# konrad-kaminski/ratelimit

Measured on AMD Instinct MI355X. Metric: rate-limit decisions/sec (whole node) at 10M/1B keys; p99 batch latency, higher is better.
Workload: dtype u32

## Files before the change

### ratelimit_amd/build.py

```python
import os
import subprocess
import sys

HERE = os.path.dirname(os.path.abspath(__file__))
ROOT = os.path.dirname(HERE)
CSRC = os.path.join(HERE, "csrc")
LIB = os.path.join(HERE, "libratelimit_hip.so")
TEAR_LIB = os.path.join(HERE, "libratelimit_hip_tear.so")
SOURCES = ["rl_kernels.hip", "rl_route.hip", "rl_match.hip", "rl_wire.hip", "rl_resp.hip", "rl_hot.hip", "rl_engine.hip", "rl_transport.hip",
           "rl_comm.hip",
           "rl_api.hip",
           "rl_pack.cpp"]
HEADERS = ["rl_device.h", "rl_kernels.h", "rl_slot_img.h", "rl_hot_select.h", "rl_match.h", "rl_wire_parse.h", "rl_resp_emit.h", "rl_engine.h",
           "rl_comm.h", "rl_transport.h",
           os.path.join("..", "..", "include", "ratelimit_hip.h")]
HIPCC = os.environ.get("HIPCC", "/opt/rocm/bin/hipcc")
ARCH = os.environ.get("RL_OFFLOAD_ARCH", "gfx950")
FLAGS = ["-O3", "-std=c++17", "-fPIC", "--offload-arch=" + ARCH, "-ffp-contract=off",
         "-Wall", "-Wno-unused-function", "-I" + os.path.join(ROOT, "include")]


def _stale():
    if not os.path.exists(LIB) or not os.path.exists(TEAR_LIB):
        return True
    t = min(os.path.getmtime(LIB), os.path.getmtime(TEAR_LIB))
    deps = [os.path.join(CSRC, s) for s in SOURCES + HEADERS] + [os.path.abspath(__file__)]
    return any(os.path.getmtime(d) > t for d in deps if os.path.exists(d))


def build(force=False, verbose=False, out=None, defines=()):
    lib = out or LIB
    if out is None and not force and not _stale():
        return LIB
    objs, procs = [], []
    tag = "" if out is None else "_%x" % (hash(lib) & 0xFFFFFF)

    def compile_(s, o, extra=()):
        cmd = [HIPCC] + FLAGS + ["-D" + d for d in tuple(defines) + tuple(extra)] + ["-c", os.path.join(CSRC, s),
                                                                                     "-o", o]
        if verbose:
            print(" ".join(cmd))
        procs.append((subprocess.Popen(cmd), cmd))

    for s in SOURCES:
        o = os.path.join(CSRC, os.path.splitext(s)[0] + tag + ".o")
        compile_(s, o)
        objs.append(o)
    tear_obj = None
    if out is None:
        tear_obj = os.path.join(CSRC, "rl_kernels_tear.o")
        compile_("rl_kernels.hip", tear_obj, ["RL_LOG_TEAR=1"])
    for p, cmd in procs:
        if p.wait() != 0:
            raise subprocess.CalledProcessError(p.returncode, cmd)

    def link(path, objects):
        cmd = [HIPCC, "-shared", "-fPIC", "--offload-arch=" + ARCH, "-o", path] + objects + ["-ldl"]
        if verbose:
            print(" ".join(cmd))
        subprocess.check_call(cmd)

    link(lib, objs)
    if tear_obj:
        link(TEAR_LIB, [tear_obj] + objs[1:])
        os.remove(tear_obj)
    for o in objs:
        os.remove(o)
    return lib


if __name__ == "__main__":
    print(build(force="--force" in sys.argv, verbose=True))
```

### ratelimit_amd/csrc/rl_engine.hip

```cpp
#include <hip/hip_runtime.h>
#include <hip/hip_ext.h>

#include <algorithm>
#include <chrono>
#include <cstdio>
#include <cstdlib>
#include <random>
#include <cstring>
#include <string>
#include <vector>

#include "../../include/ratelimit_hip.h"
#include "rl_device.h"
#include "rl_kernels.h"
#include "rl_match.h"
#include "rl_engine.h"

using namespace rl;



namespace {

thread_local std::string g_err;

int set_err(Engine* c, int code, const std::string& msg);

void prof_fold(Engine* c, uint32_t k) {
  if (!c->prof_pending[k]) return;
  c->prof_pending[k] = false;
  if (hipEventSynchronize(c->ev[k][RL_NUM_STAGES]) != hipSuccess) return;
  for (int i = 0; i < RL_NUM_STAGES; i++) {
    float ms = 0;
    if (hipEventElapsedTime(&ms, c->ev[k][i], c->ev[k][i + 1]) == hipSuccess) c->stage_ms[i] += ms;
  }
  c->prof_batches++;
}

void prof_fold_all(Engine* c) {
  for (uint32_t k = 0; k < PROF_RING; k++) prof_fold(c, (c->prof_next + k) % PROF_RING);
}

hipEvent_t* prof_events(Engine* c) {
  if (!c->prof) return nullptr;
  if (c->prof_skip) {
    c->prof_skip--;
    return nullptr;
  }
  c->prof_skip = c->prof_every - 1;
  const uint32_t k = c->prof_next;
  c->prof_next = (k + 1) % PROF_RING;
  prof_fold(c, k);
  c->prof_pending[k] = true;
  return c->ev[k];
}

int set_err(Engine* c, int code, const std::string& msg) {
  if (c) c->last_error = msg;
  else g_err = msg;
  return code;
}

#define HIPCHK(c, expr)                                                                        \
  do {                                                                                         \
    hipError_t _e = (expr);                                                                    \
    if (_e != hipSuccess)                                                                      \
      return set_err((c), RL_E_HIP, std::string("gpu: ") + #expr + ": " + hipGetErrorString(_e)); \
  } while (0)

#define RQ_SETTLE(c)                                               \
  do {                                                             \
    if ((c)->rq_n) {                                               \
      const int _rc = rl::eng_requests_advance((c), (c)->rq_n);    \
      if (_rc) return _rc;                                         \
    }                                                              \
  } while (0)

template <typename T>
hipError_t dalloc(T** p, size_t count) {
  return hipMalloc((void**)p, std::max<size_t>(count, 1) * sizeof(T));
}

inline double wall_s() {
  return std::chrono::duration<double>(std::chrono::steady_clock::now().time_since_epoch()).count();
}

int map_err(Engine* c, uint32_t e) {
  if (!e) return RL_OK;
  if (e & ERR_TIME) return set_err(c, RL_E_TIME, "gpu: now outside [0, 2^32-172800] or before the last sweep");
  if (e & ERR_HISTORY)
    return set_err(c, RL_E_TIME,
                   "gpu: a request's window is older than its key's history holds (more than 8 windows and "
                   "div + expiration_jitter_max_seconds behind the key's newest, or the history log overwrote it: "
                   "raise history_entries)");
  if (e & ERR_INVALID) return set_err(c, RL_E_INVALID, "gpu: malformed batch (unit, rule id, request index or stem offsets)");
  if (e & ERR_TABLE_FULL) return set_err(c, RL_E_TABLE_FULL, "gpu: counter table full (raise table_slots or sweep)");
  if (e & ERR_ARENA_FULL) return set_err(c, RL_E_ARENA_FULL, "gpu: long-stem arena full (raise arena_bytes)");
  return set_err(c, RL_E_INTERNAL, "gpu: unknown device error");
}

hipError_t after_batches(Engine* c, hipStream_t st) {
  for (uint32_t k = 0; k < NBUF; k++) {
    const hipError_t e = hipStreamWaitEvent(st, c->b_done[k], 0);
    if (e != hipSuccess) return e;
  }
  return hipSuccess;
}

int collect(Engine* c, hipStream_t st = nullptr) {
  if (!st) st = c->stream;
  HIPCHK(c, hipMemcpyAsync(c->h_err, c->errw, ERRW_WORDS * sizeof(uint32_t), hipMemcpyDeviceToHost, st));
  HIPCHK(c, hipStreamSynchronize(st));
  uint32_t e = c->h_err[NBUF + 2];
  for (uint32_t j = 0; j < NBUF; j++) e |= c->h_err[j];
  for (uint32_t j = 0; j < ERRB_RING; j++) e |= c->h_err[ERRW_B0 + j];
  if (e || c->h_err[NBUF + 1]) {
    HIPCHK(c, hipMemsetAsync(c->errw, 0, ERRW_WORDS * sizeof(uint32_t), st));
    HIPCHK(c, hipStreamSynchronize(st));
  }
  return map_err(c, e);
}

TableDev table_view(Engine* c);
Params params(Engine* c, int isolate = 0);

uint32_t enqueue(Engine* c, const BatchDev& b_in, const OutDev& o, int restore, hipStream_t st, bool pipelined) {
  const uint32_t k = c->next;
  const BatchDev& b = b_in;
  c->next = (k + 1) % NBUF;
  TableDev t = table_view(c);
  t.log_epoch = c->s[k].log_epoch;
  const int isolate = (!restore && o.status) ? 1 : 0;
  const Params P = params(c, isolate);
  const uint32_t* errb_prev = c->s[c->last].errb;
  c->s[k].errb = c->errw + ERRW_B0 + (c->errb_seq++ % ERRB_RING);
  const bool early = c->b_early;
  bool lng = c->long_mode == 2;
  if (c->long_mode == 1) {
    for (uint32_t j = 0; j < NBUF; j++)
      if (__atomic_load_n(&c->h_long[j], __ATOMIC_RELAXED)) {
        __atomic_store_n(&c->h_long[j], 0u, __ATOMIC_RELAXED);
        c->long_recent = 4 * NBUF;
      }
    lng = c->long_recent > 0;
    if (c->long_recent) c->long_recent--;
  }
  uint32_t* hint = c->long_mode ? c->h_long + k : nullptr;
  bool big_full = c->big_mode == 0;
  if (c->big_mode == 1) {
    for (uint32_t j = 0; j < NBUF; j++)
      if (__atomic_load_n(&c->h_big[j], __ATOMIC_RELAXED)) {
        __atomic_store_n(&c->h_big[j], 0u, __ATOMIC_RELAXED);
        c->big_recent = 4 * NBUF;
      }
    big_full = c->big_recent > 0;
    if (c->big_recent) c->big_recent--;
  }
  uint32_t* bhint = c->big_mode == 1 ? c->h_big + k : nullptr;
  bool late_full = c->late_mode == 0;
  if (c->late_mode == 1) {
    for (uint32_t j = 0; j < NBUF; j++)
      if (__atomic_load_n(&c->h_late[j], __ATOMIC_RELAXED)) {
        __atomic_store_n(&c->h_late[j], 0u, __ATOMIC_RELAXED);
        c->late_recent = 4 * NBUF;
      }
    late_full = c->late_recent > 0;
    if (c->late_recent) c->late_recent--;
  }
  uint32_t* lhint = c->late_mode == 1 ? c->h_late + k : nullptr;
  bool list_on = c->list_mode == 0;
  if (c->list_mode == 1) {
    for (uint32_t j = 0; j < NBUF; j++)
      if (__atomic_load_n(&c->h_list[j], __ATOMIC_RELAXED)) {
        __atomic_store_n(&c->h_list[j], 0u, __ATOMIC_RELAXED);
        c->list_recent = 4 * NBUF;
      }
    list_on = c->list_recent > 0;
    if (c->list_recent) c->list_recent--;
  }
  uint32_t* uhint = c->list_mode == 1 ? c->h_list + k : nullptr;
  if (pipelined) {
    hipStream_t a = c->pipe[k];
    hipEvent_t* ev = prof_events(c);
    (void)hipStreamWaitEvent(a, c->b_done[k], 0);
    (void)hipStreamWaitEvent(a, c->consumed[k], 0);
    launch_stage_a(b, c->s[k], isolate, P.per_second, a, ev, hint, lng, bhint, big_full, uhint, list_on);
    if (early) launch_b_begin_early(b, o, c->s[k], restore, a, c->log_ctr);
    (void)hipStreamWaitEvent(a, c->b_table[c->last], 0);
    launch_stage_b(b, o, t, P, c->s[k], restore, a, ev, errb_prev, c->b_table[k], ev ? c->d_kt_acc : nullptr,
                   early, lhint, late_full, list_on);
    (void)hipEventRecord(c->b_done[k], a);
  } else {
    if (!st) st = c->stream;
    (void)after_batches(c, st);
    hipEvent_t* ev = prof_events(c);
    launch_stage_a(b, c->s[k], isolate, P.per_second, st, ev, hint, lng, bhint, big_full, uhint, list_on);
    if (early) launch_b_begin_early(b, o, c->s[k], restore, st, c->log_ctr);
    launch_stage_b(b, o, t, P, c->s[k], restore, st, ev, errb_prev, c->b_table[k], ev ? c->d_kt_acc : nullptr,
                   early, lhint, late_full, list_on);
    (void)hipEventRecord(c->b_done[k], st);
  }
  c->last = k;
  return k;
}

hipError_t track(Engine* c, hipStream_t st) {
  if (c->seq_sub - c->seq_done >= PROGRESS_RING) {
    const hipError_t e = hipEventSynchronize(c->done_ring[c->seq_done % PROGRESS_RING]);
    if (e != hipSuccess) return e;
    c->seq_done++;
  }
  const hipError_t e = hipEventRecord(c->done_ring[c->seq_sub % PROGRESS_RING], st);
  c->seq_sub++;
  return e;
}

int check_sizes(Engine* c, const rl_batch* in, uint64_t stem_bytes) {
  if (!in) return set_err(c, RL_E_INVALID, "gpu: null batch");
  if (in->n > c->cfg.max_batch || in->n_requests > c->cfg.max_requests || in->n_rules > c->cfg.max_rules ||
      stem_bytes > c->cfg.max_stem_bytes)
    return set_err(c, RL_E_CAPACITY, "gpu: batch exceeds configured max_batch/max_requests/max_rules/max_stem_bytes");
  if (in->n && in->n_requests == 0) return set_err(c, RL_E_INVALID, "gpu: descriptors without requests");
  return RL_OK;
}

BatchDev dev_view(const Engine* c, const rl_batch* in, uint32_t stem_cap) {
  BatchDev b{};
  b.hk = c->hk;
  b.n = in->n;
  b.n_req = in->n_requests;
  b.n_rules = in->n_rules;
  b.stem_cap = stem_cap;
  b.stem_total = stem_cap;
  b.now_desc = 0;
  b.stem = in->stem_bytes;
  b.off = in->stem_off;
  b.now = in->now;
  b.req = in->req_idx;
  b.unit = in->unit;
  b.flags = in->flags;
  b.limit = in->limit;
  b.hits = in->hits;
  b.rule = in->rule_id;
  return b;
}

hipError_t log_ctr_get(Engine* c, std::vector<unsigned long long>& ctr, unsigned long long* lost,
                       unsigned long long* refused = nullptr) {
  std::vector<unsigned long long> h((size_t)(LOG_PARTS + 1) * LOG_CTR_STRIDE);
  hipError_t e = hipMemcpyAsync(h.data(), c->log_ctr, h.size() * 8, hipMemcpyDeviceToHost, c->stream);
  if (e == hipSuccess) e = hipStreamSynchronize(c->stream);
  if (e != hipSuccess) return e;
  ctr.resize(LOG_PARTS);
  for (uint32_t k = 0; k < LOG_PARTS; k++) ctr[k] = h[(size_t)k * LOG_CTR_STRIDE];
  if (lost) *lost = h[(size_t)LOG_PARTS * LOG_CTR_STRIDE];
  if (refused) *refused = h[(size_t)LOG_PARTS * LOG_CTR_STRIDE + 1];
  return hipSuccess;
}

TableDev table_view(Engine* c) {
  TableDev t;
  t.slots = c->slots;
  t.log = c->log;
  t.log_ctr = c->log_ctr;
  t.log_cap = c->log_cap;
  t.horizon = c->horizon;
  t.hist_lost = c->log_ctr + (size_t)LOG_PARTS * LOG_CTR_STRIDE;
  t.tear = c->tear;
  t.log_epoch = nullptr;
  t.mask = c->nslots - 1;
  t.arena = c->arena;
  t.arena_used16 = c->s[0].counters + 4;
  t.arena_cap16 = c->arena_cap16;
  t.max_probe = (uint32_t)std::min<uint64_t>(c->nslots, 1u << 16);
  t.shift = 64u - (uint32_t)__builtin_ctzll(c->nslots);
  return t;
}

Params params(Engine* c, int isolate) {
  Params P;
  P.ratio = c->cfg.near_limit_ratio;
  P.lc_en = c->cfg.local_cache_enabled != 0;
  P.per_second = c->cfg.per_second_split != 0;
  P.isolate = isolate;
  return P;
}

bool alloc_buffer(Scratch& s, uint32_t n) {
  const size_t items = (size_t)n / (64 * 4 * 8) + 1 + PART_DIGITS;
  bool ok = dalloc(&s.big_meta, PART_DIGITS) == hipSuccess && dalloc(&s.big_n, 1) == hipSuccess &&
            dalloc(&s.big_work, items) == hipSuccess && dalloc(&s.work_n, 1) == hipSuccess &&
            dalloc(&s.sorted_n, 1) == hipSuccess &&
            dalloc(&s.big_cnt, items * (1 + 2 * BIG_HEAVY)) == hipSuccess;
  ok = ok && dalloc(&s.rec, n) == hipSuccess && dalloc(&s.res, n) == hipSuccess;
  for (int i = 0; i < 2; i++) ok = ok && dalloc(&s.keys[i], n) == hipSuccess && dalloc(&s.vals[i], n) == hipSuccess;
  ok = ok && dalloc(&s.grp, n) == hipSuccess && dalloc(&s.lead, n) == hipSuccess && dalloc(&s.gmask, n) == hipSuccess &&
       dalloc(&s.defer, n) == hipSuccess &&
       dalloc(&s.defer_n, 1) == hipSuccess && dalloc(&s.defer2, n) == hipSuccess &&
       dalloc(&s.defer1, n) == hipSuccess && dalloc(&s.defer1_n, 1) == hipSuccess &&
       dalloc(&s.defer2_n, 1) == hipSuccess && dalloc(&s.fast_blk, (size_t)n / (256 * 32) + 1) == hipSuccess &&
       dalloc(&s.log_epoch, LOG_PARTS) == hipSuccess &&
       dalloc(&s.uniq, n) == hipSuccess && dalloc(&s.uniq_n, 1) == hipSuccess &&
       dalloc(&s.long_runs, (size_t)n / 1024 + 2) == hipSuccess &&
       dalloc(&s.kt_blk, 2 * ((size_t)n / 2 + BIG_HEAVY * PART_DIGITS + 2 * (size_t)n + 512) / 256) == hipSuccess;
  ok = ok && dalloc(&s.hits_s, n) == hipSuccess && dalloc(&s.segsum, n) == hipSuccess &&
       dalloc(&s.rid, n) == hipSuccess && dalloc(&s.run_start, (size_t)n + 1) == hipSuccess &&
       dalloc(&s.run_flags, n) == hipSuccess && dalloc(&s.run_state, n) == hipSuccess && dalloc(&s.run_alias, n) == hipSuccess &&
       dalloc(&s.run_f, n) == hipSuccess &&
       dalloc(&s.runs64, 1) == hipSuccess && dalloc(&s.split, 2) == hipSuccess && dalloc(&s.drun, (size_t)n / 2 + BIG_HEAVY * PART_DIGITS) == hipSuccess;
  ok = ok && dalloc(&s.hit_a, n) == hipSuccess && dalloc(&s.tile, n) == hipSuccess &&
       dalloc(&s.hit_t, n) == hipSuccess;
  ok = ok && dalloc(&s.run_end, n) == hipSuccess &&
       dalloc(&s.part_info, (size_t)PART_DIGITS * std::max((n + PART_TILE - 1) / PART_TILE, 1u)) == hipSuccess;
  ok = ok && dalloc(&s.r_base, RL_MAX_SHARDS) == hipSuccess && dalloc(&s.woff, (size_t)n + 1) == hipSuccess &&
       dalloc(&s.wtsum, WIRE_SCAN_WORDS(n)) == hipSuccess;
  return ok;
}

void free_buffer(Scratch& s) {
  void* bufs[] = {s.rec, s.res, s.big_meta, s.big_n, s.big_work, s.work_n, s.sorted_n, s.big_cnt, s.keys[0], s.keys[1],
                  s.vals[0], s.vals[1], s.grp, s.lead, s.gmask, s.defer, s.defer_n, s.defer2, s.defer2_n, s.defer1,
                  s.defer1_n, s.fast_blk, s.hits_s, s.segsum, s.rid, s.run_start, s.run_flags, s.run_state, s.run_alias,
                  s.run_f, s.runs64, s.split, s.drun, s.run_end, s.part_info, s.hit_a, s.tile, s.hit_t, s.r_base,
                  s.uniq, s.uniq_n, s.long_runs, s.kt_blk, s.log_epoch, s.woff, s.wtsum};
  for (void* p : bufs)
    if (p) (void)hipFree(p);
}

int stage(Engine* c, const rl_batch* in, BatchDev* out) {
  const uint32_t n = in->n, nq = in->n_requests;
  const uint64_t nb = n ? in->stem_off[n] : 0;
  int rc = check_sizes(c, in, nb);
  if (rc) return rc;
  hipStream_t st = c->stream;
  HIPCHK(c, after_batches(c, st));
  if (nb) HIPCHK(c, hipMemcpyAsync(c->d_stem, in->stem_bytes, nb, hipMemcpyHostToDevice, st));
  HIPCHK(c, hipMemcpyAsync(c->d_off, in->stem_off, (n + 1) * sizeof(uint32_t), hipMemcpyHostToDevice, st));
  if (nq) HIPCHK(c, hipMemcpyAsync(c->d_now, in->now, nq * sizeof(int64_t), hipMemcpyHostToDevice, st));
  if (n) {
    HIPCHK(c, hipMemcpyAsync(c->d_req, in->req_idx, n * 4, hipMemcpyHostToDevice, st));
    HIPCHK(c, hipMemcpyAsync(c->d_unit, in->unit, n, hipMemcpyHostToDevice, st));
    HIPCHK(c, hipMemcpyAsync(c->d_flags, in->flags, n, hipMemcpyHostToDevice, st));
    HIPCHK(c, hipMemcpyAsync(c->d_limit, in->limit, n * 4, hipMemcpyHostToDevice, st));
    HIPCHK(c, hipMemcpyAsync(c->d_hits, in->hits, n * 4, hipMemcpyHostToDevice, st));
    HIPCHK(c, hipMemcpyAsync(c->d_rule, in->rule_id, n * 4, hipMemcpyHostToDevice, st));
  }
  rl_batch d = *in;
  d.stem_bytes = c->d_stem;
  d.stem_off = c->d_off;
  d.now = c->d_now;
  d.req_idx = c->d_req;
  d.unit = c->d_unit;
  d.flags = c->d_flags;
  d.limit = c->d_limit;
  d.hits = c->d_hits;
  d.rule_id = c->d_rule;
  *out = dev_view(c, &d, c->cfg.max_stem_bytes);
  return RL_OK;
}

}

namespace rl {

const char* eng_last_error(const Engine* c) { return c ? c->last_error.c_str() : g_err.c_str(); }

hipError_t rl_stream_create(hipStream_t* st, uint32_t role) {
  static const uint32_t dedicated =
      getenv("RL_DEDICATED_QUEUES") ? (uint32_t)strtoul(getenv("RL_DEDICATED_QUEUES"), nullptr, 0) : 0u;
  if (!(dedicated & role)) return hipStreamCreateWithFlags(st, hipStreamNonBlocking);
  int dev = 0, cus = 0;
  hipError_t e = hipGetDevice(&dev);
  if (e == hipSuccess) e = hipDeviceGetAttribute(&cus, hipDeviceAttributeMultiprocessorCount, dev);
  if (e != hipSuccess) return e;
  std::vector<uint32_t> mask(((uint32_t)cus + 31) / 32, 0xFFFFFFFFu);
  return hipExtStreamCreateWithCUMask(st, (uint32_t)mask.size(), mask.data());
}

Engine* eng_create(const rl_config* cfg_in, char* err, size_t errlen) {
  auto fail = [&](const std::string& m, Engine* c) -> Engine* {
    if (err && errlen) snprintf(err, errlen, "%s", m.c_str());
    g_err = m;
    if (c) eng_destroy(c);
    return nullptr;
  };
  if (!cfg_in) return fail("gpu: null config", nullptr);
  rl_config cfg = *cfg_in;
  if (!cfg.table_slots) cfg.table_slots = 1ull << 24;
  if (cfg.table_slots & (cfg.table_slots - 1)) return fail("gpu: table_slots must be a power of two", nullptr);
  if (!cfg.arena_bytes) cfg.arena_bytes = 64ull << 20;
  if (!cfg.history_entries) cfg.history_entries = cfg.table_slots;
  if (cfg.history_entries > (uint64_t)LOG_PARTS * LOG_PART_MAX)
    return fail("gpu: history_entries must be at most 2^31", nullptr);
  if (cfg.expiration_jitter_max_seconds < 0) return fail("gpu: expiration_jitter_max_seconds must be >= 0", nullptr);
  if (!cfg.max_batch) cfg.max_batch = 1u << 20;
  if (cfg.max_batch > MAX_PART_TILES * PART_TILE)
    return fail("gpu: max_batch must be at most 8388608 descriptors", nullptr);
  if (!cfg.max_requests) cfg.max_requests = cfg.max_batch;
  if (!cfg.max_rules) cfg.max_rules = 65536;
  if (!cfg.max_stem_bytes) cfg.max_stem_bytes = 128u * cfg.max_batch;
  if (hipSetDevice(cfg.device) != hipSuccess) return fail("gpu: hipSetDevice failed", nullptr);

  Engine* c = new Engine();
  c->cfg = cfg;
  c->hash_seed = cfg.hash_seed;
  while (!c->hash_seed) {
    std::random_device rd;
    c->hash_seed = ((uint64_t)rd() << 32) ^ rd();
  }
  c->cfg.hash_seed = c->hash_seed;
  c->hk = hash_key_of(c->hash_seed, cfg.debug_hash_bits);
  c->nslots = cfg.table_slots;
  {
    const uint64_t want = std::max<uint64_t>(cfg.history_entries / LOG_PARTS, std::max<uint64_t>(cfg.max_batch / 16, 1024));
    uint64_t cap = 1;
    while (cap * 2 <= want && cap * 2 <= LOG_PART_MAX) cap *= 2;
    if (cap < want && cap < LOG_PART_MAX) cap *= 2;
    c->log_cap = (uint32_t)cap;
    c->cfg.history_entries = (uint64_t)LOG_PARTS * cap;
    c->horizon = (uint32_t)std::min<int64_t>(cfg.expiration_jitter_max_seconds, 1ll << 30);
  }
  c->arena_cap16 = cfg.arena_bytes / 16;
  const uint32_t n = cfg.max_batch;
  bool ok = true;
  for (uint32_t k = 0; k < NBUF; k++) ok = ok && rl_stream_create(&c->pipe[k], SR_PIPE) == hipSuccess;
  if (const char* be = getenv("RL_B_BEGIN_EARLY")) c->b_early = atoi(be) != 0;
  c->stream = c->pipe[0];
  for (uint32_t k = 0; k < NBUF; k++)
    ok = ok && hipEventCreateWithFlags(&c->b_done[k], hipEventDisableTiming) == hipSuccess &&
         hipEventCreateWithFlags(&c->b_table[k], hipEventDisableTiming) == hipSuccess;
  for (uint32_t k = 0; k < PROGRESS_RING; k++)
    ok = ok && hipEventCreateWithFlags(&c->done_ring[k], hipEventDisableTiming) == hipSuccess;
  ok = ok && dalloc(&c->slots, c->nslots) == hipSuccess &&
       dalloc(&c->log, (size_t)LOG_PARTS * c->log_cap) == hipSuccess &&
       dalloc(&c->log_ctr, (size_t)(LOG_PARTS + 1) * LOG_CTR_STRIDE) == hipSuccess;
  ok = ok && dalloc(&c->arena, cfg.arena_bytes) == hipSuccess && dalloc(&c->arena2, cfg.arena_bytes) == hipSuccess;
  for (uint32_t k = 0; k < NBUF; k++) ok = ok && alloc_buffer(c->s[k], n);
  Scratch& s0 = c->s[0];
  ok = ok && dalloc(&c->errw, ERRW_WORDS) == hipSuccess;
  for (uint32_t k = 0; k < NBUF; k++)
    ok = ok && hipEventCreateWithFlags(&c->consumed[k], hipEventDisableTiming) == hipSuccess;
  ok = ok && hipEventCreateWithFlags(&c->route_ready, hipEventDisableTiming) == hipSuccess &&
       hipEventCreateWithFlags(&c->caller_ready, hipEventDisableTiming) == hipSuccess;
  c->serial_debug = getenv("RL_DEBUG_SERIAL") != nullptr;
  c->copy_time = getenv("RL_DEBUG_COPYTIME") != nullptr;
  c->host_time = getenv("RL_DEBUG_HOSTTIME") != nullptr;
  for (uint32_t k = 0; c->copy_time && k < 64; k++)
    ok = ok && hipEventCreate(&c->ct_ev[0][k]) == hipSuccess && hipEventCreate(&c->ct_ev[1][k]) == hipSuccess &&
         hipEventCreate(&c->ct_ev[2][k]) == hipSuccess;
  ok = ok && hipHostMalloc((void**)&c->h_base, (size_t)NBUF * RL_MAX_SHARDS * 8) == hipSuccess;
  for (uint32_t k = 0; k < NBUF; k++)
    ok = ok && dalloc(&c->s[k].stripes, (size_t)STAT_STRIPES * STAT_LDS_RULES * RL_NUM_STATS) == hipSuccess;
  ok = ok && dalloc(&s0.time_floor, 1) == hipSuccess;
  ok = ok && dalloc(&s0.counters, 8) == hipSuccess;
  for (uint32_t k = 0; k < NBUF; k++) {
    Scratch& sk = c->s[k];
    sk.err = c->errw ? c->errw + k : nullptr;
    sk.errb = c->errw ? c->errw + ERRW_B0 + k : nullptr;
    sk.errs = c->errw ? c->errw + NBUF + 1 : nullptr;
    sk.time_floor = s0.time_floor;
    sk.counters = s0.counters;
  }
  ok = ok && dalloc(&c->d_stem, (size_t)cfg.max_stem_bytes + 64) == hipSuccess;
  ok = ok && dalloc(&c->d_off, (size_t)n + 1) == hipSuccess;
  ok = ok && dalloc(&c->d_now, cfg.max_requests) == hipSuccess;
  ok = ok && dalloc(&c->d_req, n) == hipSuccess && dalloc(&c->d_unit, n) == hipSuccess &&
       dalloc(&c->d_flags, n) == hipSuccess && dalloc(&c->d_limit, n) == hipSuccess &&
       dalloc(&c->d_hits, n) == hipSuccess && dalloc(&c->d_rule, n) == hipSuccess;
  ok = ok && dalloc(&c->d_code, n) == hipSuccess && dalloc(&c->d_status, n) == hipSuccess &&
       dalloc(&c->d_rem, n) == hipSuccess &&
       dalloc(&c->d_reset, n) == hipSuccess;
  ok = ok && dalloc(&c->d_stats, (size_t)cfg.max_rules * RL_NUM_STATS) == hipSuccess;
  ok = ok && hipHostMalloc((void**)&c->h_err, ERRW_WORDS * sizeof(uint32_t)) == hipSuccess;
  ok = ok && hipHostMalloc((void**)&c->h_counters, 8 * sizeof(unsigned long long)) == hipSuccess;
  ok = ok && hipHostMalloc((void**)&c->h_long, NBUF * sizeof(uint32_t)) == hipSuccess;
  if (ok) memset(c->h_long, 0, NBUF * sizeof(uint32_t));
  if (const char* sl = getenv("RL_SPLIT_LONG")) c->long_mode = atoi(sl);
  ok = ok && hipHostMalloc((void**)&c->h_big, NBUF * sizeof(uint32_t)) == hipSuccess;
  if (ok) memset(c->h_big, 0, NBUF * sizeof(uint32_t));
  if (const char* bc = getenv("RL_BIG_CUE")) c->big_mode = atoi(bc);
  ok = ok && hipHostMalloc((void**)&c->h_late, NBUF * sizeof(uint32_t)) == hipSuccess;
  if (ok) memset(c->h_late, 0, NBUF * sizeof(uint32_t));
  if (const char* lc = getenv("RL_LATE_CUE")) c->late_mode = atoi(lc);
  ok = ok && hipHostMalloc((void**)&c->h_list, NBUF * sizeof(uint32_t)) == hipSuccess;
  if (ok) memset(c->h_list, 0, NBUF * sizeof(uint32_t));
  if (const char* uc = getenv("RL_LIST_CUE")) c->list_mode = atoi(uc);
  if (const char* hr = getenv("RL_HOT_RANGE"))
    c->hot_range = std::min<uint64_t>(std::max<uint64_t>(strtoull(hr, nullptr, 0), 64), 1ull << 22);
  if (!ok) return fail("gpu: device allocation failed (table_slots/arena/max_batch too large?)", c);
  ok = hipMemsetAsync(c->slots, 0, c->nslots * sizeof(Slot), c->stream) == hipSuccess &&
       hipMemsetAsync(c->log_ctr, 0, (size_t)(LOG_PARTS + 1) * LOG_CTR_STRIDE * 8, c->stream) == hipSuccess &&
       hipMemsetAsync(c->errw, 0, ERRW_WORDS * 4, c->stream) == hipSuccess &&
       hipMemsetAsync(s0.time_floor, 0, 8, c->stream) == hipSuccess &&
       hipMemsetAsync(s0.counters, 0, 64, c->stream) == hipSuccess &&
       hipMemsetAsync(c->s[0].stripes, 0, (size_t)STAT_STRIPES * STAT_LDS_RULES * RL_NUM_STATS * 8, c->stream) ==
           hipSuccess &&
       hipMemsetAsync(c->d_stem, 0, (size_t)cfg.max_stem_bytes + 64, c->stream) == hipSuccess &&
       hipStreamSynchronize(c->stream) == hipSuccess;
  for (uint32_t k = 0; k < NBUF; k++)
    ok = ok && hipEventRecord(c->b_done[k], c->stream) == hipSuccess &&
         hipEventRecord(c->b_table[k], c->stream) == hipSuccess &&
         (k == 0 || hipMemsetAsync(c->s[k].stripes, 0, (size_t)STAT_STRIPES * STAT_LDS_RULES * RL_NUM_STATS * 8,
                                   c->stream) == hipSuccess) &&
         hipEventRecord(c->consumed[k], c->stream) == hipSuccess;
  if (!ok) return fail("gpu: device initialisation failed", c);
  return c;
}

void free_host_slots(Engine* c) {
  for (HostSlot& h : c->hs) {
    void* bufs[] = {h.stem, h.off, h.req, h.limit, h.hits, h.rule, h.now, h.unit, h.flags, h.code, h.status, h.rem,
                    h.reset, h.stats, h.cbuf};
    for (void* p : bufs)
      if (p) (void)hipFree(p);
    if (h.in_done) (void)hipEventDestroy(h.in_done);
    if (h.out_done) (void)hipEventDestroy(h.out_done);
    h = HostSlot{};
  }
  for (hipStream_t st : {c->h2d, c->d2h})
    if (st) (void)hipStreamDestroy(st);
  c->h2d = c->d2h = nullptr;
  c->hs_ready = false;
}

void copy_time_fold(Engine* c, bool all);
namespace {
void free_request_slots(Engine* c);
}

void eng_destroy(Engine* c) {
  if (!c) return;
  (void)hipSetDevice(c->cfg.device);
  if (c->host_time && c->ht_n)
    fprintf(stderr, "RL_DEBUG_HOSTTIME: %llu batches, ms each: check %.4f copy %.4f unpack %.4f enqueue %.4f to_host %.4f "
            "track %.4f\n", (unsigned long long)c->ht_n, c->ht[0] / c->ht_n * 1e3, c->ht[1] / c->ht_n * 1e3,
            c->ht[2] / c->ht_n * 1e3, c->ht[3] / c->ht_n * 1e3, c->ht[4] / c->ht_n * 1e3, c->ht[5] / c->ht_n * 1e3);
  if (c->copy_time) {
    (void)hipDeviceSynchronize();
    copy_time_fold(c, true);
    if (c->ct_count)
      fprintf(stderr, "RL_DEBUG_COPYTIME: %llu input copies, %.4f ms each, slot wait %.4f ms, gap after the previous "
              "copy %.4f ms\n", (unsigned long long)c->ct_count, c->ct_ms / c->ct_count, c->ct_wait_ms / c->ct_count,
              c->ct_gap_ms / c->ct_count);
    for (uint32_t k = 0; k < 64; k++)
      for (int j = 0; j < 3; j++)
        if (c->ct_ev[j][k]) (void)hipEventDestroy(c->ct_ev[j][k]);
  }
  if (c->hs_ready) {
    (void)hipDeviceSynchronize();
    free_host_slots(c);
  }
  if (c->rq) {
    (void)hipDeviceSynchronize();
    free_request_slots(c);
  }
  for (uint32_t k = 0; k < NBUF; k++)
    if (c->pipe[k]) (void)hipStreamSynchronize(c->pipe[k]);
  for (uint32_t k = 0; k < PROF_RING; k++)
    for (int i = 0; i <= RL_NUM_STAGES; i++)
      if (c->ev[k][i]) (void)hipEventDestroy(c->ev[k][i]);
  if (c->d_kt_acc) (void)hipFree(c->d_kt_acc);
  for (uint32_t k = 0; k < NBUF; k++) {
    free_buffer(c->s[k]);
    if (c->b_done[k]) (void)hipEventDestroy(c->b_done[k]);
    if (c->b_table[k]) (void)hipEventDestroy(c->b_table[k]);
    if (c->consumed[k]) (void)hipEventDestroy(c->consumed[k]);
  }
  for (uint32_t k = 0; k < PROGRESS_RING; k++)
    if (c->done_ring[k]) (void)hipEventDestroy(c->done_ring[k]);
  if (c->rs_ready) {
    c->rs.err = nullptr;
    scratch_free(c->rs);
  }
  if (c->route_ready) (void)hipEventDestroy(c->route_ready);
  if (c->caller_ready) (void)hipEventDestroy(c->caller_ready);
  if (c->ov_order) (void)hipEventDestroy(c->ov_order);
  for (void* p : {(void*)c->ov.slots, (void*)c->ov.koff, (void*)c->ov.klen, (void*)c->ov.arena, (void*)c->ov.ctr})
    if (p) (void)hipFree(p);
  if (c->h_base) (void)hipHostFree(c->h_base);
  const Scratch& s0 = c->s[0];
  void* bufs[] = {c->slots, c->log, c->log_ctr, c->tear, c->arena, c->arena2, c->errw, s0.stripes, s0.time_floor, s0.counters, c->d_stem, c->d_off,
                  c->d_now, c->d_req, c->d_unit, c->d_flags, c->d_limit, c->d_hits, c->d_rule, c->d_code, c->d_status,
                  c->d_rem,
                  c->d_reset, c->d_stats};
  for (void* p : bufs)
    if (p) (void)hipFree(p);
  for (uint32_t k = 1; k < NBUF; k++)
    if (c->s[k].stripes) (void)hipFree(c->s[k].stripes);
  if (c->h_err) (void)hipHostFree(c->h_err);
  if (c->h_counters) (void)hipHostFree(c->h_counters);
  if (c->h_long) (void)hipHostFree(c->h_long);
// ... 2525 lines not shown
```

### ratelimit_amd/csrc/rl_kernels.h

```cpp
#pragma once

#include <hip/hip_runtime.h>
#include <stdint.h>

#include "rl_device.h"
#include "rl_hot_select.h"

namespace rl {

#ifndef RL_PART_ITEMS
#define RL_PART_ITEMS 16
#endif
constexpr uint32_t PART_ITEMS = RL_PART_ITEMS, PART_TILE = 256 * PART_ITEMS;
constexpr uint32_t PART_BITS = 10, PART_DIGITS = 1u << PART_BITS;
#ifndef RL_BIG_BLOCKS
#define RL_BIG_BLOCKS 64
#endif
constexpr uint32_t BIG_BLOCKS = RL_BIG_BLOCKS;
constexpr uint32_t BIG_ITEM_BLOCKS = 256;
constexpr uint32_t BIG_HEAVY = 4;

struct BigMeta {
  uint32_t d, S, base, nchunks, item0, r, rb_heavy, db_heavy;
  uint32_t heavy[BIG_HEAVY];
};
constexpr uint32_t MAX_PART_TILES = 2048 * 16 / PART_ITEMS;
constexpr uint32_t LONG_RUN = 32;
constexpr uint32_t RUN_SLOW = 1, RUN_FAST = 2, RUN_MULTI = 4;
constexpr uint32_t RUN_NOWVAR = 8;
constexpr uint32_t RUN_ALIAS = 16;
constexpr uint32_t RUN_AHEAD = 32;
constexpr uint32_t RUN_MERGE = 64;
constexpr uint32_t RUN_G_SHIFT = 8, RUN_UMASK_SHIFT = 16;
constexpr uint32_t RUN_UNITS = 128, RUN_STEMS = 1u << 24;
#ifndef RL_KEY_HEAD
#define RL_KEY_HEAD 64
#endif
constexpr uint32_t KEY_HEAD = RL_KEY_HEAD;
constexpr uint32_t KEY_HV = KEY_HEAD / 16;
static_assert(KEY_HEAD % 16 == 0 && KEY_HEAD >= 48 && KEY_HEAD <= 64, "key head: 48 or 64 bytes (>= KEY_IN)");
constexpr uint32_t STAT_STRIPES = 64;
constexpr uint32_t STAT_LDS_RULES = 512;
constexpr uint32_t RUNS_GENERAL_LATE_BLOCKS = 8;

struct Wire;
struct OwnChunk {
  uint32_t lo, n, rank, stem_total;
  uint32_t src_n;
  uint32_t n_rules;
  const uint32_t* idx;
  const unsigned long long* hash;
  const uint8_t* stem;
  const uint32_t* off;
  const int64_t* now;
  const uint32_t* req;
  const uint8_t* unit;
  const uint8_t* flags;
  const uint32_t* limit;
  const uint32_t* hits;
  const uint32_t* rule;
  uint8_t* code;
  uint32_t* rem;
  uint32_t* reset;
  uint8_t* status;
  uint32_t* src_err;
};
struct BatchDev {
  uint32_t n, n_req, n_rules, stem_cap;
  uint32_t stem_total;
  uint32_t now_desc;
  HashKey hk;
  const uint8_t* stem;
  const uint32_t* off;
  const int64_t* now;
  const uint32_t* req;
  const uint8_t* unit;
  const uint8_t* flags;
  const uint32_t* limit;
  const uint32_t* hits;
  const uint32_t* rule;
  const Wire* wire;
  const uint32_t* woff;
  const unsigned long long* wbad;
  const unsigned long long* wbase;
  uint32_t n_src, rule_stride;
  OwnChunk own;
};

struct __attribute__((aligned(16))) Rec {
  uint32_t hlo;
  uint32_t off;
  uint32_t lu;
  uint32_t rule;
  uint32_t req;
  uint32_t now;
  uint32_t hits;
  uint32_t limit;
};
static_assert(sizeof(Rec) == 32, "Rec is two dwordx4");

struct SRec {
  const Rec* rec;
  const uint32_t* sv;
  __device__ inline Rec operator[](uint32_t q) const { return rec[sv[q]]; }
};

__host__ __device__ inline uint32_t rec_len(const Rec& r) { return r.lu & 0xFFFFu; }
__host__ __device__ inline uint32_t rec_unit(const Rec& r) { return (r.lu >> 16) & 0xFFu; }
__host__ __device__ inline uint32_t rec_flags(const Rec& r) { return r.lu >> 24; }

constexpr uint32_t ROUTE_REQ_BITS = 24;
constexpr uint32_t ROUTE_MAX_REQ = 1u << ROUTE_REQ_BITS;
constexpr uint32_t ROUTE_TILE = 512;
struct __attribute__((aligned(8))) Wire {
  uint32_t label;
  uint32_t lu;
  uint32_t limit;
  uint32_t hits;
  uint32_t rule;
  uint32_t now;
  unsigned long long hash;
};
constexpr uint32_t WIRE_NOW_BAD = 0xFFFFFFFFu;
static_assert(sizeof(Wire) == RL_WIRE_BYTES, "wire record size is part of the ABI");

struct OutDev {
  uint8_t* code;
  uint32_t* rem;
  uint32_t* reset;
  unsigned long long* stats;
  uint8_t* status;
};

struct TableDev {
  Slot* slots;
  LogEnt* log;
  unsigned long long* log_ctr;
  uint32_t log_cap;
  uint32_t horizon;
  unsigned long long* hist_lost;
  const unsigned long long* log_epoch;
  uint32_t* tear;
  uint64_t mask;
  uint8_t* arena;
  unsigned long long* arena_used16;
  uint64_t arena_cap16;
  uint32_t max_probe;
  uint32_t shift;
};

struct Params {
  float ratio;
  int lc_en;
  int per_second;
  int isolate;
};

struct Scratch {
  Rec* rec;
  unsigned long long* res;
  uint32_t* keys[2];
  uint32_t* vals[2];
  BigMeta* big_meta;
  uint32_t* big_n;
  uint32_t* big_work;
  uint32_t* work_n;
  uint32_t* sorted_n;
  uint32_t* big_cnt;
  uint32_t* grp;
  uint32_t* lead;
  uint8_t* gmask;
  uint32_t* defer;
  uint32_t* defer_n;
  uint32_t* defer2;
  uint32_t* defer2_n;
  uint32_t* defer1;
  uint32_t* defer1_n;
  uint32_t* fast_blk;
  unsigned long long* log_epoch;
  uint2* uniq;
  uint32_t* uniq_n;
  uint32_t* long_runs;
  unsigned long long* kt_blk;
  unsigned long long* stripes;
  uint32_t* hits_s;
  uint32_t* hit_a;
  uint4* tile;
  uint32_t* hit_t;
  uint32_t* segsum;
  uint32_t* rid;
  uint32_t* run_start;
  uint32_t* run_end;
  uint32_t* part_info;
  uint32_t* run_flags;
  uint4* run_state;
  uint4* run_alias;
  uint32_t* run_f;
  unsigned long long* runs64;
  unsigned long long* split;
  uint32_t* drun;
  uint32_t* err;
  uint32_t* errb;
  uint32_t* errs;
  int64_t* time_floor;
  unsigned long long* counters;
  uint32_t* route_start;
  uint8_t* route_dest;
  unsigned long long* route_hash;
  uint32_t* route_hist;
  unsigned long long* r_base;
  uint32_t* woff;
  unsigned long long* wtsum;
};

void launch_stage_a(const BatchDev& b, const Scratch& s, int isolate, int per_second, hipStream_t st,
                    hipEvent_t* ev = nullptr, uint32_t* long_hint = nullptr, bool long_kernel = false,
                    uint32_t* big_hint = nullptr, bool big_full = true, uint32_t* list_hint = nullptr,
                    bool list_on = true);
void launch_stage_b(const BatchDev& b, const OutDev& o, const TableDev& t, const Params& P, const Scratch& s,
                    int restore, hipStream_t st, hipEvent_t* ev, const uint32_t* errb_prev, hipEvent_t table_done,
                    unsigned long long* kt_acc = nullptr, bool early = false, uint32_t* late_hint = nullptr,
                    bool late_full = true, bool list_on = true);
void launch_b_begin_early(const BatchDev& b, const OutDev& o, const Scratch& s, int restore, hipStream_t st,
                          const unsigned long long* log_ctr);
void launch_unpack(const rl_batch_compact& cb, const uint8_t* buf, uint32_t* req, uint8_t* unit, uint8_t* flags,
                   uint32_t* limit, uint32_t* hits, uint32_t* rule, int64_t* now, uint32_t* err, hipStream_t st);
void launch_unpack_range(const rl_batch_compact& cb, const uint8_t* buf, uint32_t d0, uint32_t d1, uint32_t q0,
                         uint32_t q1, uint32_t* req, uint8_t* unit, uint8_t* flags, uint32_t* limit, uint32_t* hits,
                         uint32_t* rule, int64_t* now, uint32_t* err, hipStream_t st);
constexpr uint32_t TO_HOST_MAX = 6;
struct ToHost {
  const uint8_t* src[TO_HOST_MAX];
  uint8_t* dst[TO_HOST_MAX];
  uint64_t bytes[TO_HOST_MAX];
  uint32_t n;
};
void launch_to_host(const ToHost& c, hipStream_t st);
hipError_t copy_to_host(ToHost c, hipStream_t st);

void launch_unpack_prefixed(const rl_batch_prefixed& pb, const uint8_t* buf, uint32_t t0, uint32_t t1, uint8_t* stem,
                            uint32_t* off, uint32_t* req, uint8_t* unit, uint8_t* flags, uint32_t* limit,
                            uint32_t* hits, uint32_t* rule, int64_t* now, uint32_t* err, hipStream_t st);
constexpr uint32_t ROUTE_OWN_NONE = 0xFFFFFFFFu;
constexpr uint32_t WIRE_SCAN_TILE = 2048;
inline uint32_t WIRE_SCAN_TILES(uint64_t n) { return (uint32_t)((n + WIRE_SCAN_TILE) / WIRE_SCAN_TILE); }
inline uint32_t WIRE_SCAN_WORDS(uint64_t n) { return WIRE_SCAN_TILES(n) + 1; }
void launch_wire_offsets(const Wire* w, uint32_t n, uint32_t olo, uint32_t ohi, const unsigned long long* wbase,
                         uint32_t n_src, unsigned long long stem_total, uint32_t* woff, unsigned long long* tsum,
                         hipStream_t st);
void launch_route_pack(const BatchDev& b, uint32_t n_shards, uint32_t src_rank, Wire* out, uint8_t* out_stem,
                       uint32_t* perm, unsigned long long* counts, const Scratch& s, hipStream_t st,
                       uint32_t cstride = 2, unsigned long long meta0 = 0, unsigned long long meta1 = 0,
                       uint32_t own_rank = ROUTE_OWN_NONE, unsigned long long* hash_out = nullptr,
                       unsigned long long* counts_host = nullptr);
void launch_cnt_fill(unsigned long long* cnt, uint32_t n_peers, uint32_t cstride, unsigned long long meta0,
                     unsigned long long meta1, hipStream_t st, unsigned long long* cnt_host = nullptr);
void launch_route_fail(unsigned long long* ret, uint32_t n, uint32_t status, hipStream_t st);
void launch_route_scatter(const uint32_t* perm, const unsigned long long* ret, uint32_t n, const OutDev& o,
                          hipStream_t st, uint32_t* src_err = nullptr, const uint32_t* errb = nullptr,
                          uint32_t own_lo = 0, uint32_t own_hi = 0);
void launch_route_ret(const unsigned long long* res, uint32_t n, const uint32_t* errb, unsigned long long* ret,
                      hipStream_t st);
void launch_stats_sum(const unsigned long long* stage, uint32_t n_blocks, uint32_t m, unsigned long long* out,
                      hipStream_t st, uint32_t stride = 0);
void launch_sweep(const TableDev& t, uint64_t nslots, uint32_t now, unsigned long long* evicted, hipStream_t st);
void launch_arena_compact(Slot* slots, uint64_t nslots, const uint8_t* from, uint8_t* to, unsigned long long* used16,
                          hipStream_t st);
void launch_reclaim(const TableDev& t, const HashKey& hk, uint64_t nslots, uint32_t* need, unsigned long long* ctr,
                    hipStream_t st);
void launch_lc_count(const TableDev& t, uint64_t nslots, uint32_t now, unsigned long long* out, hipStream_t st);
void launch_table_info(const Slot* slots, uint64_t nslots, unsigned long long* out, hipStream_t st);
constexpr uint32_t RESIZE_CTR_WORDS = 6;
void launch_resize_place(const TableDev& t, const HashKey& hk, uint64_t nslots, Slot* to, uint64_t to_nslots,
                         uint32_t* map, unsigned long long* ctr, hipStream_t st);
void launch_resize_relink(const TableDev& t, uint64_t nslots, const uint32_t* map, unsigned long long* ctr,
                          hipStream_t st);
struct ExportDev {
  uint8_t* stem;
  uint32_t* off;
  uint8_t* unit;
  uint8_t* flags;
  uint32_t *ws, *count, *expire, *lc;
};
void launch_export_count(const TableDev& t, uint64_t s0, uint64_t s1, uint32_t* cnt, unsigned long long* tot,
                         hipStream_t st);
void launch_export_write(const TableDev& t, uint64_t s0, uint64_t s1, const uint32_t* cnt, unsigned long long* cursor,
                         const ExportDev& o, hipStream_t st);
struct __attribute__((aligned(16))) ImportRec {
  uint32_t off;
  uint32_t lu;
  uint32_t ws, count, expire, lc;
  uint32_t pad[2];
};
static_assert(sizeof(ImportRec) == 32, "ImportRec is two dwordx4");
void launch_import(const TableDev& t, const HashKey& hk, const uint8_t* stem, uint32_t stem_total, const ImportRec* rec,
                   const uint32_t* gstart, const unsigned long long* ghash, uint32_t ng, unsigned long long* epoch,
                   uint32_t* err, hipStream_t st);
constexpr uint32_t LOOKUP_NOW_BAD = 0xFFFFFFFFu;
struct LookupDev {
  uint32_t n;
  const uint32_t* off;
  const uint8_t* unit;
  const uint32_t* now;
  uint8_t *status, *found;
  uint32_t *count, *expire, *lc;
};
void launch_lookup(const TableDev& t, const HashKey& hk, const Params& P, const int64_t* time_floor,
                   const uint8_t* stem, uint32_t stem_total, const LookupDev& q, hipStream_t st);
struct HotState {
  unsigned long long matched, hits;
  unsigned long long stem_bytes;
  unsigned long long cursor;
  uint32_t pool_n;
  uint32_t thr, full;
  uint32_t err;
};
struct HotOutDev {
  uint8_t* stem;
  uint64_t stem_cap;
  uint32_t *off, *len;
  uint8_t* unit;
  uint32_t *ws, *count, *expire, *lc;
};
void launch_hot_scan(const TableDev& t, uint64_t s0, uint64_t s1, const rlhot::Query& q, uint32_t k, HotState* st,
                     unsigned long long* pool, uint32_t pool_cap, hipStream_t stream);
void launch_hot_select(HotState* st, unsigned long long* pool, uint32_t pool_cap, uint32_t k, uint32_t limit,
                       hipStream_t stream);
void launch_hot_size(const TableDev& t, HotState* st, const unsigned long long* pool, uint32_t pool_cap, uint32_t k,
                     hipStream_t stream);
void launch_hot_gather(const TableDev& t, HotState* st, const unsigned long long* pool, uint32_t n, const HotOutDev& o,
                       hipStream_t stream);
bool log_tear_hook();
void launch_debug_keys(const BatchDev& b, uint8_t* out, uint32_t* klen, hipStream_t st);
void launch_debug_decide(uint32_t n, const uint32_t* before, const uint32_t* after, const uint8_t* lc_hit,
                         const uint32_t* hits, const uint32_t* limit, const uint8_t* unit, const uint8_t* flags,
                         const int64_t* now, float ratio, int lc_en, uint8_t* code, uint32_t* rem, uint32_t* reset,
                         unsigned long long* deltas, uint8_t* lc_set, hipStream_t st);

}
```

### ratelimit_amd/csrc/rl_kernels.hip

```cpp
#include <hip/hip_runtime.h>
#include <stdint.h>
#include <cstdlib>

#include "rl_device.h"
#include "rl_kernels.h"
#include "rl_slot_img.h"

#ifndef RL_ABL
#define RL_ABL 0
#endif

namespace rl {

constexpr uint32_t HASH_LDS_BYTES = 16384;

__global__ __launch_bounds__(256) void k_prepare(BatchDev b, Rec* __restrict__ rec, uint32_t* __restrict__ keys,
                                                 uint32_t* err, uint32_t* errs, int isolate,
                                                 const int64_t* time_floor, uint32_t* defer_n,
                                                 uint32_t* big_n, uint32_t* work_n, uint32_t* __restrict__ run_flags,
                                                 unsigned long long* num_runs, uint32_t* __restrict__ hit_a,
                                                 unsigned long long* __restrict__ res, uint32_t* sorted_n,
                                                 uint32_t* uniq_n) {
  __shared__ uint32_t lds[HASH_LDS_BYTES / 4 + 4];
  const uint32_t tid = threadIdx.x;
// ... 982 lines not shown
  uint32_t pend_w, pend_e;
  __device__ inline void apply_pending() {
    if (pend) {
      if (cur.ws == pend_w) {
        cur.lc = pend_e;
        cur_dirty = true;
      } else if (old.ws == pend_w) {
        old.lc = pend_e;
        old_dirty = true;
      }
      pend = false;
    }
  }
};

__device__ __attribute__((always_inline)) inline void simple_put(const TableDev& t, SimpleState& S) {
  S.chain = log_append(t, S.si, S.tag, S.chain, S.cur.ws, S.old);
  S.chain_dirty = true;
  S.old_dirty = false;
}

__device__ __attribute__((always_inline)) inline int simple_pick(const TableDev& t, SimpleState& S, uint32_t w, uint32_t d,
                                                                 uint32_t now) {
  if (S.cur.ws == w) return 0;
  if (S.cur.ws == WS_INVALID || w > S.cur.ws) {
    if (S.cur.ws != WS_INVALID) {
      if (S.old_dirty) simple_put(t, S);
      if (hist_keep(t, S.cur, w, d)) {
        S.old = S.cur;
        S.old_dirty = true;
      }
    }
    S.cur = Win{w, 0, 0, 0};
    return 0;
  }
  if (S.old.ws != w) {
    if (S.old_dirty) simple_put(t, S);
    Win r;
    const int f = S.chain == LOG_NONE ? 0 : log_find(t, S.chain, S.si, S.tag, S.cur.ws, w, &r);
    if (f < 0 ? !hist_dead(now, w, d) : (f == 0 && !hist_absent_ok(t, now, w, S.cur.ws, d))) return -1;
    S.old = f > 0 ? r : Win{w, 0, 0, 0};
    S.old_dirty = false;
  }
  return 1;
}

__device__ __attribute__((always_inline)) inline void simple_step(const TableDev& t, const Params& P, unsigned long long* res,
                                                                  LaneStats& L, StatAcc& acc, SimpleState& S,
                                                                  const Elem& x, bool restore, uint32_t* err) {
  if (x.req != S.cur_req) {
    S.apply_pending();
    S.cur_req = x.req;
  }
  const int which = simple_pick(t, S, x.w, x.d, x.now);
  if (which < 0) {
    if (P.isolate) res[x.e] = pack_fail(RL_E_TIME);
    if (!(RL_ABL & 1)) atomicOr(err, ERR_HISTORY);
    return;
  }
  Win R = which ? S.old : S.cur;
  uint32_t after = 0;
  bool lc_hit = false;
  if (restore) {
    R.count = x.h;
    R.expire = x.now + x.d;
    if (x.flags) R.lc = x.now + x.d;
  } else {
    lc_hit = P.lc_en && x.now < R.lc;
    if (!lc_hit) {
      const uint32_t v = x.now <= R.expire ? R.count : 0u;
      R.count = v + x.h;
      R.expire = x.now + x.d;
      after = R.count;
    }
  }
  if (which) {
    S.old = R;
    S.old_dirty = true;
  } else {
    S.cur = R;
    S.cur_dirty = true;
  }
  if (restore) return;
  const Decision r = decide(after - x.h, after, lc_hit && !x.shadow, x.h, x.thr, P.ratio, x.shadow, P.lc_en);
  if (r.set_lc) {
    S.pend = true;
    S.pend_w = x.w;
    S.pend_e = x.now + x.d;
  }
  emit(res, L, acc, x, r, lc_hit);
}

struct GeneralState {
  int64_t sidx[4];
  Win cur[4];
  Win old[4];
  Win vic[4];
  uint32_t tag[4];
  uint32_t chain[4];
  uint32_t odirty;
  uint32_t vdirty;
  uint32_t cdirty;
  uint32_t present;
  uint32_t cur_req;
  uint32_t npend;
  uint32_t pend_w[4], pend_e[4];
};

__device__ inline bool ps_class(const Params& P, uint32_t k) { return P.per_second && k == 0; }

__device__ inline void gen_put(const TableDev& t, GeneralState& G, uint32_t k, bool vic = false) {
  G.chain[k] = log_append(t, (uint32_t)G.sidx[k], G.tag[k], G.chain[k], G.cur[k].ws, vic ? G.vic[k] : G.old[k]);
  G.cdirty |= 1u << k;
  if (vic) G.vdirty &= ~(1u << k);
  else G.odirty &= ~(1u << k);
}

__device__ inline void gen_set_old(const TableDev& t, GeneralState& G, uint32_t k, const Win& r, bool dirty) {
  if ((G.vdirty >> k) & 1) gen_put(t, G, k, true);
  G.vic[k] = G.old[k];
  G.vdirty = (G.vdirty & ~(1u << k)) | (G.odirty & (1u << k));
  G.old[k] = r;
  G.odirty = (G.odirty & ~(1u << k)) | (dirty ? 1u << k : 0u);
}

__device__ inline Win* gen_rec(const TableDev& t, GeneralState& G, uint32_t k, uint32_t w, uint32_t now, bool* lost) {
  const uint32_t d = div_of(k + 1);
  Win& c = G.cur[k];
  if (c.ws == w) return &c;
  if (c.ws == WS_INVALID || w > c.ws || w % d) return nullptr;
  if (G.old[k].ws == w) return &G.old[k];
  if (G.vic[k].ws == w) {
    const Win v = G.vic[k];
    G.vic[k] = G.old[k];
    G.old[k] = v;
    const uint32_t b = 1u << k, od = G.odirty & b;
    G.odirty = (G.odirty & ~b) | (G.vdirty & b);
    G.vdirty = (G.vdirty & ~b) | od;
    return &G.old[k];
  }
  Win r;
  const int f = G.chain[k] == LOG_NONE ? 0 : log_find(t, G.chain[k], (uint32_t)G.sidx[k], G.tag[k], c.ws, w, &r);
  if (f > 0) {
    gen_set_old(t, G, k, r, false);
    return &G.old[k];
  }
  if (lost && (f < 0 ? !hist_dead(now, w, d) : !hist_absent_ok(t, now, w, c.ws, d))) *lost = true;
  return nullptr;
}

__device__ inline void gen_touch(GeneralState& G, uint32_t k, const Win* R) {
  if (R == &G.old[k]) G.odirty |= 1u << k;
}

__device__ inline void general_apply_pending(const TableDev& t, GeneralState& G) {
  for (uint32_t j = 0; j < G.npend; j++) {
    for (uint32_t k = 0; k < 4; k++) {
      if (!(G.present >> k & 1)) continue;
      Win* R = gen_rec(t, G, k, G.pend_w[j], 0u, nullptr);
      if (R) {
        R->lc = G.pend_e[j];
        gen_touch(G, k, R);
      }
    }
  }
  G.npend = 0;
}

__device__ inline void general_step(const TableDev& t, const Params& P, unsigned long long* res, LaneStats& L,
                                    StatAcc& acc, GeneralState& G, const Elem& x, bool restore, uint32_t* err) {
  if (x.req != G.cur_req) {
    general_apply_pending(t, G);
    G.cur_req = x.req;
  }
  const uint32_t ui = x.unit - 1;
  const bool ps_e = ps_class(P, ui);
  bool lc_hit = false, lost = false;
  uint32_t v = 0, lcw = 0;
  bool vfound = false;
  for (uint32_t k = 0; k < 4; k++) {
    if (!(G.present >> k & 1)) continue;
    const Win* R = gen_rec(t, G, k, x.w, x.now, &lost);
    if (!R) continue;
    if (x.now < R->lc) lc_hit = true;
    lcw = R->lc > lcw ? R->lc : lcw;
    if (ps_class(P, k) == ps_e && !vfound && x.now <= R->expire) {
      v = R->count;
      vfound = true;
    }
  }
  if (lost) {
    if (P.isolate) res[x.e] = pack_fail(RL_E_TIME);
    atomicOr(err, ERR_HISTORY);
    return;
  }
  lc_hit = lc_hit && P.lc_en && !restore;
  uint32_t after = 0;
  if (!lc_hit) {
    const uint32_t nv = restore ? x.h : v + x.h;
    const uint32_t ex = x.now + x.d;
    Win& c = G.cur[ui];
    if (c.ws != x.w) {
      if (c.ws == WS_INVALID || x.w > c.ws) {
        if (c.ws != WS_INVALID && hist_keep(t, c, x.w, x.d)) gen_set_old(t, G, ui, c, true);
        c = Win{x.w, 0, 0, lcw};
      } else if (G.old[ui].ws != x.w) {
        gen_set_old(t, G, ui, Win{x.w, 0, 0, lcw}, true);
      }
    }
    for (uint32_t k = 0; k < 4; k++) {
      if (!(G.present >> k & 1) || ps_class(P, k) != ps_e) continue;
      Win* R = gen_rec(t, G, k, x.w, x.now, nullptr);
      if (R) {
        R->count = nv;
        R->expire = ex;
        gen_touch(G, k, R);
      }
    }
    after = nv;
  }
  if (restore) {
    if (x.flags) {
      for (uint32_t k = 0; k < 4; k++) {
        if (!(G.present >> k & 1)) continue;
        Win* R = gen_rec(t, G, k, x.w, x.now, nullptr);
        if (R) {
          R->lc = x.now + x.d;
          gen_touch(G, k, R);
        }
      }
    }
    return;
  }
  const Decision r = decide(after - x.h, after, lc_hit && !x.shadow, x.h, x.thr, P.ratio, x.shadow, P.lc_en);
  if (r.set_lc) {
    uint32_t j = 0;
    while (j < G.npend && G.pend_w[j] != x.w) j++;
    if (j == G.npend) G.npend++;
    G.pend_w[j] = x.w;
    G.pend_e[j] = x.now + x.d;
  }
  emit(res, L, acc, x, r, lc_hit);
}

__device__ __attribute__((always_inline)) inline void replay_simple(SRec rec_s, const uint32_t* svals,
                                                                    unsigned long long* res, const TableDev& t,
                                                                    const Params& P, const uint32_t* grp,
                                                                    uint32_t p, uint32_t end, uint32_t k, int64_t s0,
                                                                    Win cur0, uint32_t ring0, uint32_t tag0,
                                                                    const Rec& x0, uint32_t e0, LaneStats& L,
                                                                    StatAcc& acc, uint32_t* err, bool restore) {
  Slot* s = &t.slots[s0];
  SimpleState S;
  S.cur = cur0;
  S.old = Win{WS_INVALID, 0, 0, 0};
  S.si = (uint32_t)s0;
  S.tag = tag0;
  S.chain = ring0;
  S.cur_dirty = S.old_dirty = S.chain_dirty = false;
  S.cur_req = 0xFFFFFFFFu;
  S.pend = false;
  simple_step(t, P, res, L, acc, S, load_elem(x0, e0, restore), restore, err);
  for (uint32_t q = p + 1; q < end; q++) {
    if (grp && grp[q] != k) continue;
    simple_step(t, P, res, L, acc, S, load_elem(rec_s[q], svals[q], restore), restore, err);
  }
  S.apply_pending();
  if (S.old_dirty) simple_put(t, S);
  if (S.cur_dirty) s->cur = S.cur;
  if (S.chain_dirty) s->ring = S.chain;
}

__device__ __attribute__((always_inline)) inline uint32_t wave_incl_add(uint32_t x);
struct SegPair {
  uint32_t f, s;
};
__device__ inline SegPair seg_op(SegPair a, SegPair b) { return SegPair{a.f | b.f, b.f ? b.s : a.s + b.s}; }

struct SegChunk {
  uint64_t heads;
  uint32_t h;
};

__device__ inline SegPair seg_chunk_scan(const SegChunk& c, uint32_t lane) {
  const uint32_t P = wave_incl_add(c.h);
  const uint64_t le = c.heads & (lane == 63 ? ~0ull : ((2ull << lane) - 1));
  const uint32_t lh = le ? 63u - (uint32_t)__clzll((long long)le) : 0u;
  const uint32_t Plh = __shfl(P, lh, 64), hlh = __shfl(c.h, lh, 64);
  return le ? SegPair{1u, P - (Plh - hlh)} : SegPair{0u, P};
}

constexpr uint32_t BK_HEAVY = BIG_HEAVY;
constexpr uint32_t BK_HEAVY_MIN = 3;

template <uint32_t W, uint32_t IT>
struct BkShape {
  static constexpr uint32_t WAVES = W, ITEMS = IT, THREADS = 64 * W, CAP = 64 * W * IT, STRIP = 64 * IT;
};
using BkSmall = BkShape<4, 8>;
using BkBig = BkShape<8, 8>;

#ifdef RL_BK_PROF
__device__ unsigned long long g_bk_prof[PART_DIGITS * 16];
__device__ uint32_t g_bk_peel[PART_DIGITS * 16];
#define BK_STAMP(d, k) \
  if (threadIdx.x == 0) g_bk_prof[(d) * 16 + (k)] = wall_clock64()
#else
#define BK_STAMP(d, k)
#endif

template <uint32_t IT, uint32_t BITS>
__device__ inline void wave_multisplit(const uint32_t (&kk)[IT], uint32_t nvalid_base, uint32_t limit, uint32_t shift,
                                       uint32_t* row, uint32_t (&pos)[IT]) {
  const uint32_t lane = threadIdx.x & 63;
  const uint64_t lt_mask = (1ull << lane) - 1;
  uint32_t leader[IT];
#pragma unroll
  for (uint32_t i = 0; i < IT; i++) {
    leader[i] = lane;
    pos[i] = 0;
    if (nvalid_base + i * 64 >= limit) continue;
    const bool valid = nvalid_base + i * 64 + lane < limit;
    const uint32_t d = (kk[i] >> shift) & ((1u << BITS) - 1u);
    uint64_t peers = __ballot(valid);
#pragma unroll
    for (uint32_t bit = 0; bit < BITS; bit++) {
      const bool sb = (d >> bit) & 1u;
      const uint64_t bal = __ballot(sb);
      peers &= sb ? bal : ~bal;
    }
    const uint32_t rank = __popcll(peers & lt_mask);
    leader[i] = valid ? (uint32_t)(__ffsll((unsigned long long)peers) - 1) : lane;
    pos[i] = (valid && rank == 0) ? atomicAdd(&row[d], (uint32_t)__popcll(peers)) : 0u;
    pos[i] |= rank << 16;
  }
#pragma unroll
  for (uint32_t i = 0; i < IT; i++) pos[i] = __shfl(pos[i] & 0xFFFFu, leader[i]) + (pos[i] >> 16);
}

__device__ inline uint32_t scan256(uint32_t v, uint32_t* wsum4, uint32_t* total) {
  const uint32_t lane = threadIdx.x & 63, wave = threadIdx.x >> 6;
  uint32_t inc = v;
#pragma unroll
  for (uint32_t off = 1; off < 64; off <<= 1) {
    const uint32_t y = __shfl_up(inc, off, 64);
    if (lane >= off) inc += y;
  }
  if (wave < 4 && lane == 63) wsum4[wave] = inc;
  __syncthreads();
  uint32_t pre = 0;
#pragma unroll
  for (uint32_t w = 0; w < 4; w++) pre += w < wave ? wsum4[w] : 0u;
  if (total) *total = wsum4[0] + wsum4[1] + wsum4[2] + wsum4[3];
  __syncthreads();
  return pre + inc - v;
}

__global__ __launch_bounds__(256) void k_part(const uint32_t* __restrict__ kin, const uint32_t* __restrict__ hin,
                                              uint4* __restrict__ out, uint32_t n, uint32_t ntiles,
                                              uint32_t* __restrict__ info, const uint32_t* err) {
  constexpr uint32_t DPT = PART_DIGITS / 256;
  __shared__ uint32_t wcnt[4][PART_DIGITS];
  __shared__ uint32_t wsum[4];
  __shared__ uint32_t sk[PART_TILE], sv[PART_TILE], sh[PART_TILE];
  if (*err) return;
  const uint32_t tid = threadIdx.x, lane = tid & 63, wave = tid >> 6, tile = blockIdx.x;
  for (uint32_t j = tid; j < 4 * PART_DIGITS; j += 256) (&wcnt[0][0])[j] = 0;
  __syncthreads();
  const uint32_t wbase = tile * PART_TILE + wave * 64 * PART_ITEMS;
  uint32_t kk[PART_ITEMS], vv[PART_ITEMS], hh[PART_ITEMS], pos[PART_ITEMS];
#pragma unroll
  for (uint32_t i = 0; i < PART_ITEMS; i++) {
    const uint32_t j = min(wbase + i * 64 + lane, n - 1);
    kk[i] = kin[j];
    vv[i] = j;
    hh[i] = hin[j];
  }
  wave_multisplit<PART_ITEMS, PART_BITS>(kk, wbase, n, 32 - PART_BITS, wcnt[wave], pos);
  __syncthreads();
  uint32_t c[DPT], tsum = 0;
#pragma unroll
  for (uint32_t j = 0; j < DPT; j++) {
    const uint32_t d = tid * DPT + j;
    uint32_t acc = 0;
#pragma unroll
    for (uint32_t w = 0; w < 4; w++) {
      const uint32_t t = wcnt[w][d];
      wcnt[w][d] = acc;
      acc += t;
    }
    c[j] = acc;
    tsum += acc;
  }
  uint32_t excl = scan256(tsum, wsum, nullptr);
#pragma unroll
  for (uint32_t j = 0; j < DPT; j++) {
    const uint32_t d = tid * DPT + j;
    info[(size_t)d * ntiles + tile] = (excl << 16) | c[j];
#pragma unroll
    for (uint32_t w = 0; w < 4; w++) wcnt[w][d] += excl;
    excl += c[j];
  }
  __syncthreads();
#pragma unroll
  for (uint32_t i = 0; i < PART_ITEMS; i++) {
    if (wbase + i * 64 + lane < n) {
      const uint32_t d = kk[i] >> (32 - PART_BITS);
      const uint32_t q = wcnt[wave][d] + pos[i];
      sk[q] = kk[i];
      sv[q] = vv[i];
      sh[q] = hh[i];
    }
  }
  __syncthreads();
  const uint32_t cnt = min(PART_TILE, n - tile * PART_TILE);
  uint4* o = out + (size_t)tile * PART_TILE;
#pragma unroll
  for (uint32_t i = 0; i < PART_ITEMS; i++) {
    const uint32_t q = i * 256 + tid;
    if (q < cnt) o[q] = make_uint4(sk[q], sv[q], sh[q], 0u);
  }
}

template <typename B>
struct BucketLds {
  uint32_t k[B::CAP], v[B::CAP], h[B::CAP];
  uint32_t wcnt[B::WAVES][256];
  uint32_t gsum[B::WAVES / 4][256];
  uint32_t base[256];
  uint32_t roff[3][256];
  uint32_t dtot[256];
  uint32_t wsum[B::WAVES];
  SegPair sp[B::WAVES];
  uint32_t sh[B::WAVES];
  SegPair carry;
  uint32_t hcarry, rb, nruns, S, base_pos, db, dcnt;
  uint32_t heavy[BK_HEAVY];
  uint32_t hcnt[BK_HEAVY];
  uint32_t hstart[BK_HEAVY];
  uint32_t hrun[BK_HEAVY];
  uint32_t hw[B::WAVES][BK_HEAVY];
  uint32_t hsw[B::WAVES][BK_HEAVY];
  uint32_t acc[1 + 2 * BK_HEAVY];
  uint32_t lw[B::WAVES];
  uint32_t nheavy, nlight;
  uint32_t ub;
};

extern __shared__ uint32_t bk_seg[];

template <uint32_t IT>
__device__ inline void bucket_src(uint32_t ntiles, const uint32_t (&p)[IT], uint32_t (&j)[IT]) {
  const uint32_t* seg = bk_seg;
  const uint32_t* src = bk_seg + ntiles + 1;
  uint32_t lo[IT];
#pragma unroll
  for (uint32_t i = 0; i < IT; i++) lo[i] = 0;
#pragma unroll
  for (uint32_t step = MAX_PART_TILES / 2; step; step >>= 1) {
    if (step >= ntiles) continue;
#pragma unroll
    for (uint32_t i = 0; i < IT; i++) {
      const uint32_t m = lo[i] + step;
      if (m < ntiles && seg[m] <= p[i]) lo[i] = m;
    }
  }
#pragma unroll
  for (uint32_t i = 0; i < IT; i++) j[i] = src[lo[i]] + p[i];
}

template <typename B>
__device__ inline uint32_t block_sum(BucketLds<B>& L, uint32_t v) {
  const uint32_t lane = threadIdx.x & 63, wave = threadIdx.x >> 6;
#pragma unroll
  for (uint32_t off = 32; off; off >>= 1) v += __shfl_xor(v, off, 64);
  if (lane == 0) L.wsum[wave] = v;
  __syncthreads();
  uint32_t s = 0;
#pragma unroll
  for (uint32_t w = 0; w < B::WAVES; w++) s += L.wsum[w];
  __syncthreads();
  return s;
}

template <typename B>
__device__ inline void bucket_setup(BucketLds<B>& L, const uint32_t* __restrict__ info, uint32_t ntiles, uint32_t d) {
  const uint32_t tid = threadIdx.x, lane = tid & 63, wave = tid >> 6;
  uint32_t* seg = bk_seg;
  uint32_t* src = bk_seg + ntiles + 1;
  uint32_t carry = 0, offs = 0;
  for (uint32_t t0 = 0; t0 < ntiles; t0 += B::THREADS) {
    const uint32_t t = t0 + tid;
    const uint32_t e = t < ntiles ? info[(size_t)d * ntiles + t] : 0u;
    const uint32_t cnt = e & 0xFFFFu;
    offs += e >> 16;
    uint32_t inc = cnt;
#pragma unroll
    for (uint32_t off = 1; off < 64; off <<= 1) {
      const uint32_t y = __shfl_up(inc, off, 64);
      if (lane >= off) inc += y;
    }
    if (lane == 63) L.wsum[wave] = inc;
    __syncthreads();
    uint32_t pre = carry, all = carry;
    for (uint32_t w = 0; w < B::WAVES; w++) {
      pre += w < wave ? L.wsum[w] : 0u;
      all += L.wsum[w];
    }
    if (t < ntiles) {
      const uint32_t st = pre + inc - cnt;
      seg[t] = st;
      src[t] = t * PART_TILE + (e >> 16) - st;
    }
    carry = all;
    __syncthreads();
  }
  const uint32_t bp = block_sum(L, offs);
  if (tid == 0) {
    seg[ntiles] = carry;
    L.S = carry;
    L.base_pos = bp;
  }
  __syncthreads();
}

template <typename B, uint32_t BITS>
__device__ inline void bucket_rank(BucketLds<B>& L, const uint32_t (&kk)[B::ITEMS], uint32_t strip0, uint32_t limit,
                                   uint32_t shift, bool chunk_scan, uint32_t (&pos)[B::ITEMS]) {
  const uint32_t tid = threadIdx.x, wave = tid >> 6;
  for (uint32_t j = tid; j < B::WAVES * 256; j += B::THREADS) (&L.wcnt[0][0])[j] = 0;
  __syncthreads();
  uint32_t local[B::ITEMS];
  wave_multisplit<B::ITEMS, BITS>(kk, strip0, limit, shift, L.wcnt[wave], local);
  __syncthreads();
  constexpr uint32_t NG = B::WAVES / 4;
  const uint32_t dg = tid & 255u, g = tid >> 8;
  uint32_t r[4], c = 0;
#pragma unroll
  for (uint32_t w = 0; w < 4; w++) r[w] = L.wcnt[g * 4 + w][dg];
#pragma unroll
  for (uint32_t w = 0; w < 4; w++) {
    const uint32_t t = r[w];
    r[w] = c;
    c += t;
  }
  L.gsum[g][dg] = c;
  __syncthreads();
  uint32_t pre = 0, all = 0;
#pragma unroll
  for (uint32_t q = 0; q < NG; q++) {
    const uint32_t t = L.gsum[q][dg];
    pre += q < g ? t : 0u;
    all += t;
  }
#pragma unroll
  for (uint32_t w = 0; w < 4; w++) L.wcnt[g * 4 + w][dg] = r[w] + pre;
  if (tid < 256) L.dtot[tid] = all;
  const uint32_t excl = scan256(tid < 256 ? all : 0u, L.wsum, nullptr);
  if (chunk_scan && tid < 256) L.base[tid] = excl;
  __syncthreads();
#pragma unroll
  for (uint32_t i = 0; i < B::ITEMS; i++) {
    const uint32_t d = (kk[i] >> shift) & ((1u << BITS) - 1u);
    pos[i] = L.base[d] + L.wcnt[wave][d] + local[i];
  }
  __syncthreads();
}

template <typename B>
__device__ inline void lds_sort3(BucketLds<B>& L, uint32_t (&kk)[B::ITEMS], uint32_t (&vv)[B::ITEMS],
                                 uint32_t (&hh)[B::ITEMS], uint32_t n) {
  static_assert(32 - PART_BITS == 22, "passes of 8 + 8 + 6 bits");
  const uint32_t lane = threadIdx.x & 63, strip0 = (threadIdx.x >> 6) * B::STRIP;
  uint32_t pos[B::ITEMS];
#pragma unroll 1
  for (uint32_t pass = 0; pass < 3; pass++) {
    if (pass < 2) bucket_rank<B, 8>(L, kk, strip0, n, 8 * pass, true, pos);
    else bucket_rank<B, 6>(L, kk, strip0, n, 16, true, pos);
#pragma unroll
    for (uint32_t i = 0; i < B::ITEMS; i++) {
      if (strip0 + i * 64 + lane < n) {
        L.k[pos[i]] = kk[i];
        L.v[pos[i]] = vv[i];
        L.h[pos[i]] = hh[i];
      }
    }
    __syncthreads();
#pragma unroll
    for (uint32_t i = 0; i < B::ITEMS; i++) {
      const uint32_t p = strip0 + i * 64 + lane;
      if (p < n) {
        kk[i] = L.k[p];
        vv[i] = L.v[p];
        hh[i] = L.h[p];
      }
    }
  }
}

template <typename B, bool FROM_LDS, bool PRE = false>
__device__ inline void bucket_segment(BucketLds<B>& L, uint32_t d, uint32_t S, uint32_t base,
                                      const uint32_t* __restrict__ sk, const uint32_t* __restrict__ sh,
                                      uint32_t* __restrict__ segsum, uint32_t* __restrict__ rid,
                                      uint32_t* __restrict__ run_start, uint32_t* __restrict__ run_end,
                                      unsigned long long* num_runs, uint32_t* __restrict__ drun) {
  constexpr uint32_t IT = B::ITEMS;
  const uint32_t tid = threadIdx.x, lane = tid & 63, wave = tid >> 6;
  auto key = [&](uint32_t p) -> uint32_t { return FROM_LDS ? L.k[p] : sk[base + p]; };
  auto hit = [&](uint32_t p) -> uint32_t { return FROM_LDS ? L.h[p] : sh[base + p]; };
  uint32_t nh = 0, nd = 0;
  for (uint32_t c0 = 0; !PRE && c0 < S; c0 += B::CAP) {
    uint32_t a[IT], b[IT], c[IT];
#pragma unroll
    for (uint32_t i = 0; i < IT; i++) {
      const uint32_t p = min(c0 + i * B::THREADS + tid, S - 1);
      a[i] = key(p ? p - 1 : 0);
      b[i] = key(p);
      c[i] = key(p > 1 ? p - 2 : 0);
    }
#pragma unroll
    for (uint32_t i = 0; i < IT; i++) {
      const uint32_t p = c0 + i * B::THREADS + tid;
      nh += (p < S && (p == 0 || a[i] != b[i])) ? 1u : 0u;
      nd += (p < S && p >= 1 && a[i] == b[i] && (p == 1 || c[i] != a[i])) ? 1u : 0u;
    }
  }
  if constexpr (!PRE) {
    nh = block_sum(L, nh);
    nd = block_sum(L, nd);
    BK_STAMP(d, 4);
    if (tid == 0) {
      const unsigned long long old = atomicAdd(num_runs, ((unsigned long long)nd << 32) | nh);
      L.rb = (uint32_t)old;
      L.db = (uint32_t)(old >> 32);
      L.dcnt = 0;
      L.nruns = nh;
      L.carry = SegPair{0, 0};
      L.hcarry = 0;
    }
    __syncthreads();
  }
  const uint32_t rb = L.rb;
  for (uint32_t c0 = 0; c0 < S; c0 += B::CAP) {
    const uint32_t s0 = c0 + wave * B::STRIP;
    const uint32_t ni = s0 >= S ? 0u : min(IT, (S - s0 + 63) / 64);
    SegChunk ch[IT];
    SegPair agg{0, 0};
    uint32_t hc = 0;
    uint32_t kp[IT], kq[IT], hq[IT], kpp[IT];
#pragma unroll
    for (uint32_t j = 0; j < IT; j++) {
      const uint32_t q = min(s0 + 64 * j + lane, S - 1);
      kp[j] = key(q ? q - 1 : 0);
      kq[j] = key(q);
      hq[j] = hit(q);
      kpp[j] = key(q > 1 ? q - 2 : 0);
    }
    uint32_t hd = 0, sd = 0;
#pragma unroll
    for (uint32_t j = 0; j < IT; j++) {
      const uint32_t q = s0 + 64 * j + lane;
      hd |= (q < S && (q == 0 || kp[j] != kq[j])) ? 1u << j : 0u;
      sd |= (q < S && q >= 1 && kp[j] == kq[j] && (q == 1 || kpp[j] != kp[j])) ? 1u << j : 0u;
    }
#pragma unroll
    for (uint32_t j = 0; j < IT; j++) {
      ch[j] = SegChunk{0, 0};
      if (j >= ni) continue;
      const uint32_t hv = s0 + 64 * j + lane < S ? (hq[j] > 1 ? hq[j] : 1u) : 0u;
      ch[j] = SegChunk{(uint64_t)__ballot((hd >> j) & 1u), hv};
      uint32_t t = hv;
      const uint32_t lh = ch[j].heads ? 63u - (uint32_t)__clzll((long long)ch[j].heads) : 0u;
      if (ch[j].heads && lane < lh) t = 0;
#pragma unroll
      for (uint32_t off = 32; off; off >>= 1) t += __shfl_xor(t, off, 64);
      agg = seg_op(agg, SegPair{ch[j].heads ? 1u : 0u, t});
      hc += (uint32_t)__popcll(ch[j].heads);
    }
    if (lane == 0) {
      L.sp[wave] = agg;
      L.sh[wave] = hc;
    }
    __syncthreads();
    SegPair run = L.carry;
    uint32_t hrun = L.hcarry;
    SegPair tot = run;
    uint32_t htot = hrun;
    for (uint32_t w = 0; w < B::WAVES; w++) {
      if (w == wave) {
        run = tot;
        hrun = htot;
      }
      tot = seg_op(tot, L.sp[w]);
      htot += L.sh[w];
    }
    __syncthreads();
    if (tid == 0) {
      L.carry = tot;
      L.hcarry = htot;
    }
#pragma unroll
    for (uint32_t j = 0; j < IT; j++) {
      if (j >= ni) continue;
      const uint32_t q = s0 + 64 * j + lane;
      const SegPair v = seg_chunk_scan(ch[j], lane);
      const SegPair in = seg_op(run, v);
      const uint64_t heads = ch[j].heads;
      const uint32_t r = hrun + (uint32_t)__popcll(heads & (lane == 63 ? ~0ull : ((2ull << lane) - 1))) - 1;
      if (q < S) {
        segsum[base + q] = in.s;
        rid[base + q] = rb + r;
        if ((heads >> lane) & 1) {
          run_start[rb + r] = base + q;
          if (r) run_end[rb + r - 1] = base + q;
        }
        if ((sd >> j) & 1) drun[L.db + atomicAdd(&L.dcnt, 1u)] = rb + r;
      }
      run = seg_op(run, SegPair{__shfl(v.f, 63, 64), __shfl(v.s, 63, 64)});
      hrun += (uint32_t)__popcll(heads);
    }
    __syncthreads();
  }
  if (tid == 0 && S) run_end[rb + L.nruns - 1] = base + S;
}

constexpr uint32_t BIG_CHUNK = BkSmall::CAP;
constexpr uint32_t BIG_LIGHT_CAP = BkBig::CAP;
constexpr uint32_t BIG_CNT = 1 + 2 * BK_HEAVY;

constexpr uint32_t BK_SAMPLES_PER_LANE = 4;
template <typename B>
__device__ inline void sample_heavy(BucketLds<B>& L, uint32_t S, uint32_t ntiles, const uint4* __restrict__ pt) {
  constexpr uint32_t R = BK_SAMPLES_PER_LANE, NS = 64 * R;
  const uint32_t lane = threadIdx.x & 63;
  if ((threadIdx.x >> 6) == 0) {
    uint32_t p[R], j[R], ks[R], cnt[R];
    bool first[R];
#pragma unroll
    for (uint32_t i = 0; i < R; i++) p[i] = (uint32_t)(((uint64_t)(2 * (lane * R + i) + 1) * S) / (2 * NS));
    bucket_src(ntiles, p, j);
#pragma unroll
    for (uint32_t i = 0; i < R; i++) {
      ks[i] = pt[j[i]].x;
      cnt[i] = 0;
      first[i] = true;
    }
    for (uint32_t q = 0; q < 64; q++) {
#pragma unroll
      for (uint32_t r = 0; r < R; r++) {
        const uint32_t kq = __shfl(ks[r], q, 64), g = q * R + r;
#pragma unroll
        for (uint32_t i = 0; i < R; i++) {
          cnt[i] += kq == ks[i] ? 1u : 0u;
          if (g < lane * R + i && kq == ks[i]) first[i] = false;
        }
      }
    }
    uint32_t nc = 0;
#pragma unroll
    for (uint32_t i = 0; i < R; i++) nc += (first[i] && cnt[i] >= BK_HEAVY_MIN) ? 1u : 0u;
    uint32_t incl = nc;
#pragma unroll
    for (uint32_t o = 1; o < 64; o <<= 1) {
      const uint32_t y = __shfl_up(incl, o, 64);
      if (lane >= o) incl += y;
    }
    uint32_t rank = incl - nc;
#pragma unroll
    for (uint32_t i = 0; i < R; i++)
      if (first[i] && cnt[i] >= BK_HEAVY_MIN) {
        if (rank < BK_HEAVY) L.heavy[rank] = ks[i];
        rank++;
      }
    if (lane == 63) L.nheavy = min(incl, BK_HEAVY);
  }
  __syncthreads();
}

#ifndef RL_BK_EARLY
#define RL_BK_EARLY 1
#endif
template <bool LIST>
__global__ __launch_bounds__(BkSmall::THREADS, 4) void k_bucket(
    const uint4* __restrict__ pt,
    const uint32_t* __restrict__ info, uint32_t ntiles, uint32_t* __restrict__ sk, uint32_t* __restrict__ sv,
    uint32_t* __restrict__ sh, uint32_t* __restrict__ segsum, uint32_t* __restrict__ rid,
    uint32_t* __restrict__ run_start, uint32_t* __restrict__ run_end, unsigned long long* num_runs,
    uint32_t* __restrict__ drun, BigMeta* __restrict__ meta, uint32_t* big_n, uint32_t* __restrict__ work,
    uint32_t* work_n, uint32_t* sorted_n, uint2* __restrict__ uniq, uint32_t* uniq_n, const uint32_t* err,
    uint32_t* big_hint) {
  using B = BkSmall;
  __shared__ BucketLds<B> L;
  if (*err) return;
  const uint32_t tid = threadIdx.x, lane = tid & 63, wave = tid >> 6, d = blockIdx.x;
  BK_STAMP(d, 0);
  bucket_setup(L, info, ntiles, d);
  const uint32_t S = L.S;
  if (!S) return;
  if (S > B::CAP) {
    sample_heavy(L, S, ntiles, pt);
    if (tid == 0) {
      BigMeta M;
      M.d = d;
      M.S = S;
      M.base = atomicAdd(sorted_n, S);
      M.r = L.nheavy;
      M.nchunks = M.r ? (S + BIG_CHUNK - 1) / BIG_CHUNK : 0u;
      M.item0 = M.nchunks ? atomicAdd(work_n, M.nchunks) : 0u;
      const unsigned long long old =
          M.r ? atomicAdd(num_runs, ((unsigned long long)M.r << 32) | M.r) : 0ull;
      M.rb_heavy = (uint32_t)old;
      M.db_heavy = (uint32_t)(old >> 32);
      for (uint32_t c = 0; c < BK_HEAVY; c++) M.heavy[c] = c < M.r ? L.heavy[c] : 0u;
      const uint32_t b = atomicAdd(big_n, 1u);
      meta[b] = M;
      if (big_hint) *big_hint = 1u;
      L.rb = b;
      L.nruns = M.item0;
      L.hcarry = M.nchunks;
    }
    __syncthreads();
    for (uint32_t t = tid; t < L.hcarry; t += B::THREADS) work[L.nruns + t] = (L.rb << 16) | t;
    return;
  }
  BK_STAMP(d, 1);
  uint32_t kk[B::ITEMS], vv[B::ITEMS], hh[B::ITEMS];
  const uint32_t strip0 = wave * B::STRIP;
  uint32_t pp[B::ITEMS], jj[B::ITEMS];
#pragma unroll
  for (uint32_t i = 0; i < B::ITEMS; i++) pp[i] = min(strip0 + i * 64 + lane, S - 1);
  bucket_src(ntiles, pp, jj);
#pragma unroll
  for (uint32_t i = 0; i < B::ITEMS; i++) {
    const uint4 e = pt[jj[i]];
    kk[i] = e.x;
    vv[i] = e.y;
    hh[i] = e.z;
  }
  BK_STAMP(d, 2);
  uint32_t* ht = L.v;
  uint8_t* df = reinterpret_cast<uint8_t*>(&L.wcnt[0][0]);
  static_assert(sizeof(L.wcnt) >= B::CAP, "dup flags fit the multisplit rows");
  constexpr uint32_t HT = 2 * B::CAP, HT_SHIFT = 32 - 12;
  static_assert(HT == 1u << 12, "hash index bits");
#pragma unroll
  for (uint32_t i = 0; i < B::ITEMS; i++) {
    const uint32_t p = strip0 + i * 64 + lane;
    if (p < S) L.k[p] = kk[i];
  }
  for (uint32_t j = tid; j < HT; j += B::THREADS) ht[j] = 0xFFFFFFFFu;
  for (uint32_t j = tid; j < B::CAP / 4; j += B::THREADS) reinterpret_cast<uint32_t*>(df)[j] = 0u;
  __syncthreads();
  uint32_t win = 0;
#pragma unroll
  for (uint32_t i = 0; i < B::ITEMS; i++) {
    const uint32_t p = strip0 + i * 64 + lane;
    if (p >= S) continue;
    uint32_t h = (kk[i] * 0x9E3779B1u) >> HT_SHIFT;
    for (;;) {
      const uint32_t o = atomicCAS(&ht[h], 0xFFFFFFFFu, p);
      if (o == 0xFFFFFFFFu) {
        win |= 1u << i;
        break;
      }
      if (L.k[o] == kk[i]) {
        df[p] = 1;
        df[o] = 1;
        break;
      }
      h = (h + 1) & (HT - 1);
    }
  }
  __syncthreads();
  const uint64_t lt = (1ull << lane) - 1;
  uint32_t cidx[B::ITEMS], sidx[LIST ? B::ITEMS : 1], wc = 0, ws = 0, wr = 0, dmask = 0, smask = 0;
#pragma unroll
  for (uint32_t i = 0; i < B::ITEMS; i++) {
    const uint32_t p = strip0 + i * 64 + lane;
    const bool dup = p < S && df[p];
    const uint64_t bl = __ballot(dup);
    cidx[i] = wc + (uint32_t)__popcll(bl & lt);
    wc += (uint32_t)__popcll(bl);
    dmask |= dup ? 1u << i : 0u;
    if (RL_BK_EARLY) wr += (uint32_t)__popcll(__ballot(dup && ((win >> i) & 1u)));
    if constexpr (LIST) {
      const bool one = p < S && !df[p];
      const uint64_t bs = __ballot(one);
      sidx[i] = ws + (uint32_t)__popcll(bs & lt);
      ws += (uint32_t)__popcll(bs);
      smask |= one ? 1u << i : 0u;
    }
  }
  if (lane == 0) {
    L.wsum[wave] = wc;
    L.sh[wave] = wr;
    if (LIST) L.lw[wave] = ws;
  }
  __syncthreads();
  uint32_t wpre = 0, M = 0, spre = 0, nh = 0;
#pragma unroll
  for (uint32_t w = 0; w < B::WAVES; w++) {
    wpre += w < wave ? L.wsum[w] : 0u;
    if (LIST) spre += w < wave ? L.lw[w] : 0u;
    M += L.wsum[w];
    nh += L.sh[w];
  }
#pragma unroll
  for (uint32_t i = 0; i < B::ITEMS; i++) {
    if (!((dmask >> i) & 1u)) continue;
    const uint32_t c = wpre + cidx[i];
    L.k[c] = kk[i];
    L.v[c] = vv[i];
    L.h[c] = hh[i];
  }
  uint32_t r_base = 0;
  unsigned long long r_runs = 0;
  if (tid == 0) {
    if (M) {
      r_base = atomicAdd(sorted_n, M);
      if (RL_BK_EARLY) r_runs = atomicAdd(num_runs, ((unsigned long long)nh << 32) | nh);
    }
    if constexpr (LIST) L.ub = M < S ? atomicAdd(uniq_n, S - M) : 0u;
  }
  __syncthreads();
  if constexpr (LIST) {
    const uint32_t ub = L.ub + spre;
#pragma unroll
    for (uint32_t i = 0; i < B::ITEMS; i++)
      if ((smask >> i) & 1u) uniq[ub + sidx[i]] = make_uint2(vv[i], kk[i]);
  }
  if (!M) return;
  if (M <= 64) {
    if (wave == 0) {
      const bool v = lane < M;
      const uint32_t k = v ? L.k[lane] : 0xFFFFFFFFu, x = v ? L.v[lane] : 0u, y = v ? L.h[lane] : 0u;
      uint32_t r = 0;
      for (uint32_t j = 0; j < M; j++) {
        const uint32_t kj = __shfl(k, j, 64);
        r += (kj < k || (kj == k && j < lane)) ? 1u : 0u;
      }
      if (v) {
        L.k[r] = k;
        L.v[r] = x;
        L.h[r] = y;
      }
    }
  } else {
#pragma unroll
    for (uint32_t i = 0; i < B::ITEMS; i++) {
      const uint32_t p = strip0 + i * 64 + lane;
      kk[i] = p < M ? L.k[p] : 0xFFFFFFFFu;
      vv[i] = p < M ? L.v[p] : 0u;
      hh[i] = p < M ? L.h[p] : 0u;
    }
    __syncthreads();
    lds_sort3(L, kk, vv, hh, M);
  }
  if (tid == 0) {
    L.base_pos = r_base;
    if (RL_BK_EARLY) {
      L.rb = (uint32_t)r_runs;
      L.db = (uint32_t)(r_runs >> 32);
      L.dcnt = 0;
      L.nruns = nh;
      L.carry = SegPair{0, 0};
      L.hcarry = 0;
    }
  }
  __syncthreads();
  const uint32_t base = L.base_pos;
  for (uint32_t p = tid; p < M; p += B::THREADS) {
    sk[base + p] = L.k[p];
    sv[base + p] = L.v[p];
  }
  BK_STAMP(d, 3);
  [[clang::always_inline]] bucket_segment<B, true, RL_BK_EARLY != 0>(L, d, M, base, sk, sh, segsum, rid, run_start,
                                                                     run_end, num_runs, drun);
  BK_STAMP(d, 5);
}

template <typename B>
__device__ inline bool bucket_peel(BucketLds<B>& L, uint32_t d, uint32_t S, uint32_t base, uint32_t ntiles,
                                   const uint4* __restrict__ pt,
                                   uint32_t* __restrict__ sk,
                                   uint32_t* __restrict__ sv, uint32_t* __restrict__ sh) {
  constexpr uint32_t IT = B::ITEMS;
  const uint32_t tid = threadIdx.x, lane = tid & 63, wave = tid >> 6;
  const uint64_t lt_mask = (1ull << lane) - 1;
  if (wave == 0) {
    uint32_t p[1] = {(uint32_t)(((uint64_t)(2 * lane + 1) * S) >> 7)}, j[1];
    bucket_src(ntiles, p, j);
    const uint32_t ks = pt[j[0]].x;
    uint32_t cnt = 0;
    bool first = true;
    for (uint32_t q = 0; q < 64; q++) {
      const uint32_t kq = __shfl(ks, q, 64);
      cnt += kq == ks ? 1u : 0u;
      if (q < lane && kq == ks) first = false;
    }
    const bool cand = first && cnt >= BK_HEAVY_MIN;
    const uint64_t b = __ballot(cand);
    const uint32_t rank = __popcll(b & lt_mask);
    if (cand && rank < BK_HEAVY) L.heavy[rank] = ks;
    if (lane < BK_HEAVY) {
      L.hcnt[lane] = 0;
      L.hrun[lane] = 0;
    }
    if (lane == 0) {
      L.nheavy = min((uint32_t)__popcll(b), BK_HEAVY);
      L.nlight = 0;
    }
  }
  __syncthreads();
  const uint32_t r = L.nheavy;
  if (!r) return false;
  uint32_t hk[BK_HEAVY];
#pragma unroll
  for (uint32_t c = 0; c < BK_HEAVY; c++) hk[c] = __builtin_amdgcn_readfirstlane(c < r ? L.heavy[c] : 0u);
  uint32_t kk[IT], vv[IT], hh[IT], cls[IT];
  for (uint32_t c0 = 0; c0 < S; c0 += B::CAP) {
    const uint32_t strip0 = c0 + wave * B::STRIP;
    uint32_t pp[IT], jj[IT];
#pragma unroll
    for (uint32_t i = 0; i < IT; i++) pp[i] = min(strip0 + i * 64 + lane, S - 1);
    bucket_src(ntiles, pp, jj);
#pragma unroll
    for (uint32_t i = 0; i < IT; i++) {
      const uint4 e = pt[jj[i]];
      kk[i] = e.x;
      vv[i] = e.y;
      hh[i] = e.z;
    }
    uint32_t wl = 0, lr[IT];
    uint32_t wc[BK_HEAVY];
#pragma unroll
    for (uint32_t c = 0; c < BK_HEAVY; c++) wc[c] = 0;
#pragma unroll
    for (uint32_t i = 0; i < IT; i++) {
      const bool in = strip0 + i * 64 + lane < S;
      cls[i] = in ? r : 0xFFu;
#pragma unroll
      for (uint32_t c = 0; c < BK_HEAVY; c++)
        if (in && c < r && kk[i] == hk[c]) cls[i] = c;
      const uint64_t bl = __ballot(cls[i] == r);
      lr[i] = wl + __popcll(bl & lt_mask);
      wl += __popcll(bl);
#pragma unroll
      for (uint32_t c = 0; c < BK_HEAVY; c++) wc[c] += c < r ? __popcll(__ballot(cls[i] == c)) : 0u;
    }
    if (lane == 0) {
      L.lw[wave] = wl;
#pragma unroll
      for (uint32_t c = 0; c < BK_HEAVY; c++) L.hw[wave][c] = wc[c];
    }
    __syncthreads();
    uint32_t pre = L.nlight, tl = 0;
    for (uint32_t w = 0; w < B::WAVES; w++) {
      pre += w < wave ? L.lw[w] : 0u;
      tl += L.lw[w];
    }
#pragma unroll
    for (uint32_t i = 0; i < IT; i++) {
      const uint32_t at = pre + lr[i];
      if (cls[i] == r && at < B::CAP) {
        L.k[at] = kk[i];
        L.v[at] = vv[i];
        L.h[at] = hh[i];
      }
    }
    __syncthreads();
    if (tid < BK_HEAVY) {
      uint32_t t = 0;
      for (uint32_t w = 0; w < B::WAVES; w++) t += L.hw[w][tid];
      L.hcnt[tid] += t;
    }
    if (tid == 0) L.nlight += tl;
    __syncthreads();
  }
  const uint32_t nl = L.nlight;
  if (nl > B::CAP) return false;
  BK_STAMP(d, 13);
  const uint32_t strip0 = wave * B::STRIP;
#pragma unroll
  for (uint32_t i = 0; i < IT; i++) {
    const uint32_t p = strip0 + i * 64 + lane;
    kk[i] = p < nl ? L.k[p] : 0xFFFFFFFFu;
    vv[i] = p < nl ? L.v[p] : 0u;
    hh[i] = p < nl ? L.h[p] : 0u;
  }
  if (nl) lds_sort3(L, kk, vv, hh, nl);
  if (tid < r) {
    const uint32_t K = hk[tid];
    uint32_t lo = 0, hi = nl;
    while (lo < hi) {
      const uint32_t mid = (lo + hi) >> 1;
      if (L.k[mid] < K) lo = mid + 1;
      else hi = mid;
    }
    uint32_t st = lo;
    for (uint32_t c = 0; c < r; c++) st += hk[c] < K ? L.hcnt[c] : 0u;
    L.hstart[tid] = st;
  }
#ifdef RL_BK_PROF
  __syncthreads();
  if (tid == 0) {
    uint32_t* g = g_bk_peel + d * 16;
    g[0] = r;
    g[1] = nl;
    for (uint32_t c = 0; c < BK_HEAVY; c++) {
      g[2 + c] = hk[c];
      g[6 + c] = L.hcnt[c];
      g[10 + c] = L.hstart[c];
    }
    g[14] = S;
  }
#endif
#pragma unroll
  for (uint32_t i = 0; i < IT; i++) {
    const uint32_t p = strip0 + i * 64 + lane;
    if (p < nl) {
      uint32_t at = p;
#pragma unroll
      for (uint32_t c = 0; c < BK_HEAVY; c++) at += (c < r && hk[c] < kk[i]) ? L.hcnt[c] : 0u;
      sk[base + at] = kk[i];
      sv[base + at] = vv[i];
      sh[base + at] = hh[i];
    }
  }
  __syncthreads();
  BK_STAMP(d, 14);
  for (uint32_t c0 = 0; c0 < S; c0 += B::CAP) {
    const uint32_t s0 = c0 + wave * B::STRIP;
    uint32_t pp[IT], jj[IT];
#pragma unroll
    for (uint32_t i = 0; i < IT; i++) pp[i] = min(s0 + i * 64 + lane, S - 1);
    bucket_src(ntiles, pp, jj);
#pragma unroll
    for (uint32_t i = 0; i < IT; i++) {
      const uint4 e = pt[jj[i]];
      kk[i] = e.x;
      vv[i] = e.y;
      hh[i] = e.z;
    }
    uint32_t hr[IT], wc[BK_HEAVY];
#pragma unroll
    for (uint32_t c = 0; c < BK_HEAVY; c++) wc[c] = 0;
#pragma unroll
    for (uint32_t i = 0; i < IT; i++) {
      const bool in = s0 + i * 64 + lane < S;
      cls[i] = BK_HEAVY;
#pragma unroll
      for (uint32_t c = 0; c < BK_HEAVY; c++)
        if (in && c < r && kk[i] == hk[c]) cls[i] = c;
      hr[i] = 0;
#pragma unroll
      for (uint32_t c = 0; c < BK_HEAVY; c++) {
        if (c >= r) continue;
        const uint64_t b = __ballot(cls[i] == c);
        if (cls[i] == c) hr[i] = wc[c] + __popcll(b & lt_mask);
        wc[c] += __popcll(b);
      }
    }
    if (lane == 0) {
#pragma unroll
      for (uint32_t c = 0; c < BK_HEAVY; c++) L.hw[wave][c] = wc[c];
    }
    __syncthreads();
#pragma unroll
    for (uint32_t i = 0; i < IT; i++) {
      const uint32_t c = cls[i];
      if (c < BK_HEAVY) {
        uint32_t at = L.hstart[c] + L.hrun[c] + hr[i];
        for (uint32_t w = 0; w < wave; w++) at += L.hw[w][c];
        sk[base + at] = kk[i];
        sv[base + at] = vv[i];
        sh[base + at] = hh[i];
      }
    }
    __syncthreads();
    if (tid < r) {
      uint32_t t = 0;
      for (uint32_t w = 0; w < B::WAVES; w++) t += L.hw[w][tid];
      L.hrun[tid] += t;
    }
    __syncthreads();
  }
  __threadfence_block();
  __syncthreads();
  BK_STAMP(d, 15);
  return true;
}

template <typename B>
__device__ inline void bucket_lsd(BucketLds<B>& L, uint32_t S, uint32_t base, uint32_t ntiles,
                                  const uint4* __restrict__ pt,
                                  uint32_t* __restrict__ sk,
                                  uint32_t* __restrict__ sv, uint32_t* __restrict__ sh, uint32_t* __restrict__ ht,
                                  uint32_t* __restrict__ segsum, uint32_t* __restrict__ rid) {
  constexpr uint32_t IT = B::ITEMS;
  const uint32_t tid = threadIdx.x, lane = tid & 63, wave = tid >> 6;
  uint32_t kk[IT], vv[IT], hh[IT], pos[IT];
  for (uint32_t j = tid; j < 3 * 256; j += B::THREADS) (&L.roff[0][0])[j] = 0;
  __syncthreads();
  for (uint32_t c0 = 0; c0 < S; c0 += B::CAP) {
    uint32_t pp[IT], jj[IT];
#pragma unroll
    for (uint32_t i = 0; i < IT; i++) pp[i] = min(c0 + i * B::THREADS + tid, S - 1);
    bucket_src(ntiles, pp, jj);
#pragma unroll
    for (uint32_t i = 0; i < IT; i++) kk[i] = pt[jj[i]].x;
#pragma unroll
    for (uint32_t i = 0; i < IT; i++) {
      if (c0 + i * B::THREADS + tid < S) {
        atomicAdd(&L.roff[0][kk[i] & 255u], 1u);
        atomicAdd(&L.roff[1][(kk[i] >> 8) & 255u], 1u);
        atomicAdd(&L.roff[2][(kk[i] >> 16) & 63u], 1u);
      }
    }
  }
  __syncthreads();
  for (uint32_t pass = 0; pass < 3; pass++) {
    const uint32_t v = tid < 256 ? L.roff[pass][tid] : 0u;
    const uint32_t excl = scan256(v, L.wsum, nullptr);
    if (tid < 256) L.roff[pass][tid] = excl;
  }
  __syncthreads();
  for (uint32_t pass = 0; pass < 3; pass++) {
    const uint32_t* ik = pass == 1 ? sk + base : rid + base;
    const uint32_t* iv = pass == 1 ? sv + base : segsum + base;
    const uint32_t* ih = pass == 1 ? sh + base : ht + base;
    uint32_t* ok = pass == 1 ? rid + base : sk + base;
    uint32_t* ov = pass == 1 ? segsum + base : sv + base;
    uint32_t* oh = pass == 1 ? ht + base : sh + base;
    for (uint32_t c0 = 0; c0 < S; c0 += B::CAP) {
      const uint32_t strip0 = c0 + wave * B::STRIP;
      uint32_t pp[IT], jj[IT];
#pragma unroll
      for (uint32_t i = 0; i < IT; i++) pp[i] = min(strip0 + i * 64 + lane, S - 1);
      if (pass == 0) {
        bucket_src(ntiles, pp, jj);
      } else {
#pragma unroll
        for (uint32_t i = 0; i < IT; i++) jj[i] = pp[i];
      }
      if (pass == 0) {
#pragma unroll
        for (uint32_t i = 0; i < IT; i++) {
          const uint4 e = pt[jj[i]];
          kk[i] = e.x;
          vv[i] = e.y;
          hh[i] = e.z;
        }
      } else {
#pragma unroll
        for (uint32_t i = 0; i < IT; i++) {
          kk[i] = ik[jj[i]];
          vv[i] = iv[jj[i]];
          hh[i] = ih[jj[i]];
        }
      }
#pragma unroll
      for (uint32_t i = 0; i < IT; i++)
        if (strip0 + i * 64 + lane >= S) kk[i] = 0xFFFFFFFFu;
      if (tid < 256) L.base[tid] = L.roff[pass][tid];
      if (pass < 2) bucket_rank<B, 8>(L, kk, strip0, S, 8 * pass, false, pos);
      else bucket_rank<B, 6>(L, kk, strip0, S, 16, false, pos);
      if (tid < 256) L.roff[pass][tid] += L.dtot[tid];
#pragma unroll
      for (uint32_t i = 0; i < IT; i++) {
        if (strip0 + i * 64 + lane < S) {
          ok[pos[i]] = kk[i];
          ov[pos[i]] = vv[i];
          oh[pos[i]] = hh[i];
        }
      }
    }
    __threadfence_block();
    __syncthreads();
  }
}

__device__ inline uint32_t wave_sum32(uint32_t x) {
#pragma unroll
  for (uint32_t m = 32; m >= 1; m >>= 1) x += __shfl_xor(x, m, 64);
  return x;
}

#ifndef RL_DPP_SCAN
#define RL_DPP_SCAN 1
#endif
__device__ __attribute__((always_inline)) inline uint32_t wave_incl_add(uint32_t x) {
#if RL_DPP_SCAN
  x += (uint32_t)__builtin_amdgcn_update_dpp(0, (int)x, 0x111, 0xf, 0xf, false);
  x += (uint32_t)__builtin_amdgcn_update_dpp(0, (int)x, 0x112, 0xf, 0xf, false);
  x += (uint32_t)__builtin_amdgcn_update_dpp(0, (int)x, 0x114, 0xf, 0xf, false);
  x += (uint32_t)__builtin_amdgcn_update_dpp(0, (int)x, 0x118, 0xf, 0xf, false);
  x += (uint32_t)__builtin_amdgcn_update_dpp(0, (int)x, 0x142, 0xa, 0xf, false);
  x += (uint32_t)__builtin_amdgcn_update_dpp(0, (int)x, 0x143, 0xc, 0xf, false);
#else
  const uint32_t lane = __lane_id();
#pragma unroll
  for (uint32_t off = 1; off < 64; off <<= 1) {
    const uint32_t y = __shfl_up(x, off, 64);
    if (lane >= off) x += y;
  }
#endif
  return x;
}

__device__ inline void big_chunk_load(const BigMeta& M, uint32_t j, uint32_t ntiles, const uint4* __restrict__ pt,
                                      uint32_t (&kk)[BkSmall::ITEMS], uint32_t (&vv)[BkSmall::ITEMS],
                                      uint32_t (&hh)[BkSmall::ITEMS], uint32_t (&cls)[BkSmall::ITEMS], bool values) {
  using B = BkSmall;
  const uint32_t lane = threadIdx.x & 63, s0 = j * BIG_CHUNK + (threadIdx.x >> 6) * B::STRIP;
  uint32_t pp[B::ITEMS], jj[B::ITEMS];
#pragma unroll
  for (uint32_t i = 0; i < B::ITEMS; i++) pp[i] = min(s0 + i * 64 + lane, M.S - 1);
  bucket_src(ntiles, pp, jj);
#pragma unroll
  for (uint32_t i = 0; i < B::ITEMS; i++) {
    const uint4 e = pt[jj[i]];
    kk[i] = e.x;
    hh[i] = e.z;
    vv[i] = values ? e.y : 0u;
  }
#pragma unroll
  for (uint32_t i = 0; i < B::ITEMS; i++) {
    cls[i] = s0 + i * 64 + lane < M.S ? M.r : 0xFFu;
#pragma unroll
    for (uint32_t c = 0; c < BK_HEAVY; c++)
      if (cls[i] != 0xFFu && c < M.r && kk[i] == M.heavy[c]) cls[i] = c;
  }
}

__global__ __launch_bounds__(BkSmall::THREADS) void k_big_count(const uint4* __restrict__ pt,
                                                                const uint32_t* __restrict__ info, uint32_t ntiles,
                                                                const BigMeta* __restrict__ meta,
                                                                const uint32_t* __restrict__ work,
                                                                const uint32_t* work_n, uint32_t* __restrict__ cnt,
                                                                const uint32_t* err) {
  using B = BkSmall;
  __shared__ BucketLds<B> L;
  if (*err) return;
  const uint32_t tid = threadIdx.x, lane = tid & 63, wave = tid >> 6, nw = *work_n;
  for (uint32_t it = blockIdx.x; it < nw; it += gridDim.x) {
    const uint32_t w = work[it];
    const BigMeta M = meta[w >> 16];
    bucket_setup(L, info, ntiles, M.d);
    uint32_t kk[B::ITEMS], vv[B::ITEMS], hh[B::ITEMS], cls[B::ITEMS];
    big_chunk_load(M, w & 0xFFFFu, ntiles, pt, kk, vv, hh, cls, false);
    uint32_t nl = 0, nc[BK_HEAVY], hs[BK_HEAVY];
#pragma unroll
    for (uint32_t c = 0; c < BK_HEAVY; c++) nc[c] = hs[c] = 0;
#pragma unroll
    for (uint32_t i = 0; i < B::ITEMS; i++) {
      const uint32_t hv = hh[i] > 1 ? hh[i] : 1u;
      nl += cls[i] == M.r ? 1u : 0u;
#pragma unroll
      for (uint32_t c = 0; c < BK_HEAVY; c++) {
        nc[c] += cls[i] == c ? 1u : 0u;
        hs[c] += cls[i] == c ? hv : 0u;
      }
    }
    nl = wave_sum32(nl);
#pragma unroll
    for (uint32_t c = 0; c < BK_HEAVY; c++) {
      nc[c] = wave_sum32(nc[c]);
      hs[c] = wave_sum32(hs[c]);
    }
    if (lane == 0) {
      L.lw[wave] = nl;
#pragma unroll
      for (uint32_t c = 0; c < BK_HEAVY; c++) {
        L.hw[wave][c] = nc[c];
        L.hsw[wave][c] = hs[c];
      }
    }
    __syncthreads();
    if (tid < BIG_CNT) {
      uint32_t t = 0;
      for (uint32_t v = 0; v < B::WAVES; v++)
        t += tid == 0 ? L.lw[v] : tid <= BK_HEAVY ? L.hw[v][tid - 1] : L.hsw[v][tid - 1 - BK_HEAVY];
      cnt[(size_t)it * BIG_CNT + tid] = t;
    }
    __syncthreads();
  }
}

__global__ __launch_bounds__(BkSmall::THREADS) void k_big_place(
    const uint4* __restrict__ pt,
    const uint32_t* __restrict__ info, uint32_t ntiles, const BigMeta* __restrict__ meta,
    const uint32_t* __restrict__ work, const uint32_t* work_n, const uint32_t* __restrict__ cnt,
    uint32_t* __restrict__ sk, uint32_t* __restrict__ sv, uint32_t* __restrict__ sh, uint32_t* __restrict__ segsum,
    uint32_t* __restrict__ rid, uint32_t* __restrict__ run_start, uint32_t* __restrict__ run_end,
    uint32_t* __restrict__ drun, const uint32_t* err) {
  using B = BkSmall;
  __shared__ BucketLds<B> L;
  if (*err) return;
  const uint32_t tid = threadIdx.x, lane = tid & 63, wave = tid >> 6, nw = *work_n;
  const uint64_t lt_mask = (1ull << lane) - 1;
  for (uint32_t it = blockIdx.x; it < nw; it += gridDim.x) {
    const uint32_t w = work[it], j = w & 0xFFFFu;
    const BigMeta M = meta[w >> 16];
    if (tid < BIG_CNT) L.acc[tid] = 0;
    uint32_t tot[BIG_CNT];
#pragma unroll
    for (uint32_t k = 0; k < BIG_CNT; k++) tot[k] = 0;
    __syncthreads();
    for (uint32_t t = tid; t < M.nchunks; t += B::THREADS) {
      const uint32_t* ct = cnt + (size_t)(M.item0 + t) * BIG_CNT;
#pragma unroll
      for (uint32_t k = 0; k < BIG_CNT; k++) {
        const uint32_t v = ct[k];
        tot[k] += v;
        if (t < j) atomicAdd(&L.acc[k], v);
      }
    }
#pragma unroll
    for (uint32_t k = 0; k < 1 + BK_HEAVY; k++) tot[k] = block_sum(L, tot[k]);
    bucket_setup(L, info, ntiles, M.d);
    const uint32_t NL = tot[0];
    if (NL > BIG_LIGHT_CAP) continue;
    uint32_t hstart[BK_HEAVY];
    uint32_t st = NL;
#pragma unroll
    for (uint32_t c = 0; c < BK_HEAVY; c++) {
      hstart[c] = st;
      st += c < M.r ? tot[1 + c] : 0u;
    }
    if (j == 0 && tid < M.r) {
      run_start[M.rb_heavy + tid] = M.base + hstart[tid];
      run_end[M.rb_heavy + tid] = M.base + hstart[tid] + tot[1 + tid];
      drun[M.db_heavy + tid] = M.rb_heavy + tid;
    }
    uint32_t kk[B::ITEMS], vv[B::ITEMS], hh[B::ITEMS], cls[B::ITEMS];
    big_chunk_load(M, j, ntiles, pt, kk, vv, hh, cls, true);
    uint32_t rk[B::ITEMS], hp[B::ITEMS], wl = 0, wc[BK_HEAVY], wh[BK_HEAVY];
#pragma unroll
    for (uint32_t c = 0; c < BK_HEAVY; c++) wc[c] = wh[c] = 0;
#pragma unroll
    for (uint32_t i = 0; i < B::ITEMS; i++) {
      const uint64_t bl = __ballot(cls[i] == M.r);
      rk[i] = wl + __popcll(bl & lt_mask);
      wl += __popcll(bl);
      hp[i] = 0;
      const uint32_t hv = hh[i] > 1 ? hh[i] : 1u;
#pragma unroll
      for (uint32_t c = 0; c < BK_HEAVY; c++) {
        if (c >= M.r) continue;
        const bool mine = cls[i] == c;
        const uint64_t b = __ballot(mine);
        const uint32_t x = wave_incl_add(mine ? hv : 0u);
        if (mine) {
          rk[i] = wc[c] + __popcll(b & lt_mask);
          hp[i] = wh[c] + x;
        }
        wc[c] += __popcll(b);
        wh[c] += (uint32_t)__builtin_amdgcn_readlane((int)x, 63);
      }
    }
    if (lane == 0) {
      L.lw[wave] = wl;
#pragma unroll
      for (uint32_t c = 0; c < BK_HEAVY; c++) {
        L.hw[wave][c] = wc[c];
        L.hsw[wave][c] = wh[c];
      }
    }
    __syncthreads();
    uint32_t lpre = L.acc[0], cpre[BK_HEAVY], hpre[BK_HEAVY];
#pragma unroll
    for (uint32_t c = 0; c < BK_HEAVY; c++) {
      cpre[c] = L.acc[1 + c];
      hpre[c] = L.acc[1 + BK_HEAVY + c];
    }
    for (uint32_t v = 0; v < wave; v++) {
      lpre += L.lw[v];
#pragma unroll
      for (uint32_t c = 0; c < BK_HEAVY; c++) {
        cpre[c] += L.hw[v][c];
        hpre[c] += L.hsw[v][c];
      }
    }
#pragma unroll
    for (uint32_t i = 0; i < B::ITEMS; i++) {
      const uint32_t c = cls[i];
      if (c == M.r) {
        const uint32_t at = M.base + lpre + rk[i];
        sk[at] = kk[i];
        sv[at] = vv[i];
        sh[at] = hh[i];
      } else if (c < BK_HEAVY) {
        uint32_t cp = 0, hq = 0, hs0 = 0;
#pragma unroll
        for (uint32_t q = 0; q < BK_HEAVY; q++)
          if (q == c) {
            cp = cpre[q];
            hq = hpre[q];
            hs0 = hstart[q];
          }
        const uint32_t at = M.base + hs0 + cp + rk[i];
        sk[at] = kk[i];
        sv[at] = vv[i];
        segsum[at] = hq + hp[i];
        rid[at] = M.rb_heavy + c;
      }
    }
    __syncthreads();
  }
}

__global__ __launch_bounds__(BkBig::THREADS) void k_bucket_big(
    const uint4* __restrict__ pt,
    const uint32_t* __restrict__ info, uint32_t ntiles, uint32_t* __restrict__ sk, uint32_t* __restrict__ sv,
    uint32_t* __restrict__ sh, uint32_t* __restrict__ ht, uint32_t* __restrict__ segsum, uint32_t* __restrict__ rid,
    uint32_t* __restrict__ run_start, uint32_t* __restrict__ run_end, unsigned long long* num_runs,
    uint32_t* __restrict__ drun, const BigMeta* __restrict__ meta, const uint32_t* big_n,
    const uint32_t* __restrict__ cnt, const uint32_t* err) {
  using B = BkBig;
  __shared__ BucketLds<B> L;
  if (*err) return;
  const uint32_t tid = threadIdx.x, lane = tid & 63, wave = tid >> 6, nb = *big_n;
  for (uint32_t bi = blockIdx.x; bi < nb; bi += gridDim.x) {
    const BigMeta M = meta[bi];
    const uint32_t d = M.d, S = M.S, base = M.base;
    BK_STAMP(d, 0);
    uint32_t nl = 0;
    for (uint32_t t = tid; t < M.nchunks; t += B::THREADS) nl += cnt[(size_t)(M.item0 + t) * BIG_CNT];
    nl = block_sum(L, nl);
    if (M.r && nl <= BIG_LIGHT_CAP) {
      uint32_t kk[B::ITEMS], vv[B::ITEMS], hh[B::ITEMS];
      const uint32_t strip0 = wave * B::STRIP;
#pragma unroll
      for (uint32_t i = 0; i < B::ITEMS; i++) {
        const uint32_t p = min(strip0 + i * 64 + lane, nl ? nl - 1 : 0u);
        kk[i] = sk[base + p];
        vv[i] = sv[base + p];
        hh[i] = sh[base + p];
      }
#pragma unroll
      for (uint32_t i = 0; i < B::ITEMS; i++)
        if (strip0 + i * 64 + lane >= nl) kk[i] = 0xFFFFFFFFu;
      if (nl) {
        lds_sort3(L, kk, vv, hh, nl);
#pragma unroll
        for (uint32_t i = 0; i < B::ITEMS; i++) {
          const uint32_t p = strip0 + i * 64 + lane;
          if (p < nl) {
            sk[base + p] = kk[i];
            sv[base + p] = vv[i];
          }
        }
        __syncthreads();
        bucket_segment<B, true>(L, d, nl, base, sk, sh, segsum, rid, run_start, run_end, num_runs, drun);
      }
    } else {
      if (tid < M.r) run_start[M.rb_heavy + tid] = run_end[M.rb_heavy + tid] = 0;
      bucket_setup(L, info, ntiles, d);
      BK_STAMP(d, 1);
      if (!bucket_peel(L, d, S, base, ntiles, pt, sk, sv, sh))
        bucket_lsd(L, S, base, ntiles, pt, sk, sv, sh, ht, segsum, rid);
      bucket_segment<B, false>(L, d, S, base, sk, sh, segsum, rid, run_start, run_end, num_runs, drun);
    }
    BK_STAMP(d, 7);
    __syncthreads();
  }
}

#ifndef RL_RC_CHUNK
#define RL_RC_CHUNK 256
#endif
constexpr uint32_t RC_CHUNK = RL_RC_CHUNK;

#ifndef RL_UNIQ_DENSE
#define RL_UNIQ_DENSE 3
#endif

template <typename Pred>
__device__ __attribute__((always_inline)) inline uint32_t block_compact(uint32_t lo, uint32_t hi, uint32_t* list,
                                                                        uint32_t* count, Pred pred) {
  const uint32_t lane = threadIdx.x & 63;
  if (threadIdx.x == 0) *count = 0;
  __syncthreads();
  for (uint32_t i0 = lo; i0 < hi; i0 += blockDim.x) {
    const uint32_t i = i0 + threadIdx.x;
    const bool take = i < hi && pred(i);
    const uint64_t m = __ballot(take);
    uint32_t base = 0;
    if (lane == 0 && m) base = atomicAdd(count, (uint32_t)__popcll(m));
    base = __shfl(base, 0);
    if (take) list[base + __popcll(m & ((1ull << lane) - 1))] = i;
  }
  __syncthreads();
  return *count;
}

constexpr uint32_t SPLIT_POS_OTHER = 0xFFu, SPLIT_POS_SKIP = 0xFEu, SPLIT_POS_NOWVAR = 1u << 16;
constexpr uint32_t SPLIT_ULIST = 1024;

__global__ __launch_bounds__(256) void k_run_check(BatchDev b, SRec rec_s,
                                                   const uint32_t* __restrict__ skeys,
                                                   const uint32_t* __restrict__ rid,
                                                   const uint32_t* __restrict__ run_start,
                                                   uint32_t* __restrict__ run_end,
                                                   uint32_t* __restrict__ run_flags, uint32_t* __restrict__ defer,
                                                   uint32_t* defer_n, const uint32_t* err,
                                                   const unsigned long long* num_runs, unsigned long long* split,
                                                   const uint32_t* sorted_n, uint32_t* __restrict__ pos_unit,
                                                   uint32_t* __restrict__ pos_hits, uint2* __restrict__ uniq,
                                                   uint32_t* uniq_n, uint32_t* long_runs, uint32_t* __restrict__ keys0,
                                                   int list_on, uint32_t* list_hint) {
  __shared__ uint32_t s_list[RC_CHUNK], s_cnt;
  if (blockIdx.x == 0 && threadIdx.x == 0) {
    split[0] = 0;
    split[1] = *num_runs;
    long_runs[0] = 0;
  }
  if (*err) return;
  const uint32_t sn = *sorted_n;
  if (list_hint && blockIdx.x == 0 && threadIdx.x == 0 && (uint64_t)(b.n - min(sn, b.n)) * 4 < (uint64_t)b.n * RL_UNIQ_DENSE)
    *list_hint = 1u;
  for (uint32_t q0 = blockIdx.x * RC_CHUNK; list_on && q0 < min(blockIdx.x * RC_CHUNK + RC_CHUNK, sn); q0 += blockDim.x) {
    const uint32_t q = q0 + threadIdx.x;
    const uint32_t k = q < sn ? skeys[q] : 0u;
    const bool one = q < sn && (q == 0 || skeys[q - 1] != k) && (q + 1 >= sn || skeys[q + 1] != k);
    const uint64_t m = __ballot(one);
    if (!m) continue;
    const uint32_t lane = threadIdx.x & 63, leader = (uint32_t)__ffsll((unsigned long long)m) - 1;
    uint32_t at = 0;
    if (lane == leader) at = atomicAdd(uniq_n, (uint32_t)__popcll(m));
    at = __shfl(at, leader, 64) + (uint32_t)__popcll(m & ((1ull << lane) - 1));
    if (one) uniq[at] = make_uint2(rec_s.sv[q], k);
  }
  const uint32_t lo = max(blockIdx.x * RC_CHUNK, 1u), hi = min(blockIdx.x * RC_CHUNK + RC_CHUNK, sn);
  if (lo >= hi) return;
  const uint32_t cnt = block_compact(lo, hi, s_list, &s_cnt, [&](uint32_t q) { return skeys[q - 1] == skeys[q]; });
  refine_totals(b);
  Rec* rec = const_cast<Rec*>(rec_s.rec);
#pragma unroll 1
  for (uint32_t j = threadIdx.x; j < cnt; j += blockDim.x) {
    const uint32_t q = s_list[j];
    const uint32_t r = rid[q];
    const uint32_t p = run_start[r];
    const uint32_t eq = rec_s.sv[q], ep = rec_s.sv[p];
    const Rec x = rec[eq], y = rec[ep];
    const bool skip = (rec_flags(x) | rec_flags(y)) & FLAG_SKIP;
    const bool same_stem = !skip && x.hlo == y.hlo && (x.lu & 0xFFFFu) == (y.lu & 0xFFFFu) &&
                           key_equal(key_of(b, x), key_of(b, y));
    if (!same_stem && !skip && q == p + 1 && run_end[r] == q + 1) {
      run_end[r] = p;
      if (list_on) {
        const uint32_t at = atomicAdd(uniq_n, 2u);
        uniq[at] = make_uint2(ep, skeys[q]);
        uniq[at + 1] = make_uint2(eq, skeys[q]);
      }
      continue;
    }
    keys0[eq] = KEY_DUP;
    if (q == p + 1) keys0[ep] = KEY_DUP;
    const bool same = same_stem && rec_unit(x) == rec_unit(y);
    pos_unit[q] = (rec_unit(x) << 8) | (skip ? SPLIT_POS_SKIP : !same_stem ? SPLIT_POS_OTHER : 0u) |
                  (x.now != y.now ? SPLIT_POS_NOWVAR : 0u);
    pos_hits[q] = x.hits > 1 ? x.hits : 1u;
    uint32_t f = 0;
    if (!same)
      f = RUN_MULTI | (same_stem ? RUN_UNITS | ((1u << (rec_unit(x) - 1)) << RUN_UMASK_SHIFT) : RUN_STEMS);
    if (x.now != y.now) {
      const uint32_t d = div_of(rec_unit(x));
      f |= (same && x.now / d != y.now / d) ? RUN_SLOW | RUN_NOWVAR : RUN_NOWVAR;
    }
    uint64_t pend = __ballot(f != 0);
    while (pend) {
      const uint32_t leader = (uint32_t)(__ffsll((unsigned long long)pend) - 1);
      const uint32_t rr = __shfl(r, leader, 64);
      const bool mine = f != 0 && r == rr;
      const uint64_t mm = __ballot(mine);
      constexpr uint32_t kBits[] = {RUN_MULTI, RUN_UNITS, RUN_STEMS, RUN_SLOW, RUN_NOWVAR,
                                    1u << RUN_UMASK_SHIFT, 2u << RUN_UMASK_SHIFT, 4u << RUN_UMASK_SHIFT,
                                    8u << RUN_UMASK_SHIFT};
      uint32_t fo = 0;
#pragma unroll
      for (uint32_t bi = 0; bi < sizeof(kBits) / sizeof(kBits[0]); bi++)
        if (__ballot(mine && (f & kBits[bi]))) fo |= kBits[bi];
      if ((threadIdx.x & 63u) == leader &&
          (__hip_atomic_load(&run_flags[rr], __ATOMIC_RELAXED, __HIP_MEMORY_SCOPE_AGENT) & fo) != fo) {
        const uint32_t old = atomicOr(&run_flags[rr], fo);
        if ((fo & RUN_MULTI) && !(old & RUN_MULTI)) defer[atomicAdd(defer_n, 1u)] = rr;
      }
      pend &= ~mm;
    }
  }
}

#ifndef RL_SPLIT_BLOCKS
#define RL_SPLIT_BLOCKS 128
#endif
constexpr uint32_t SPLIT_CAP = 1024, SPLIT_MAXG = 8, SPLIT_BLOCKS = RL_SPLIT_BLOCKS;
constexpr uint32_t DEFER_DONE = 0xFFFFFFFFu;
constexpr uint32_t SPLIT_BAD = 0xFFu;

struct SplitPlan {
  uint8_t ug[SPLIT_MAXG][4];
  uint8_t head[SPLIT_MAXG];
  uint8_t ng[SPLIT_MAXG];
  uint8_t fam[SPLIT_MAXG];
  uint8_t alias[SPLIT_MAXG];
  uint8_t gmask[SPLIT_MAXG];
  uint32_t G, any_alias;
};

__device__ inline uint32_t split_plan(SplitPlan& S, uint32_t NF, const uint32_t* fmask, const uint32_t* fnow,
                                      const uint32_t* fnv, int per_second) {
  uint32_t G = 0;
  S.any_alias = 0;
  for (uint32_t f = 0; f < NF; f++) {
    const uint32_t m = fmask[f];
    S.head[f] = (uint8_t)G;
    if (__popc(m) == 1) {
      if (G >= SPLIT_MAXG) return SPLIT_BAD;
      for (uint32_t u = 0; u < 4; u++) S.ug[f][u] = (uint8_t)G;
      S.fam[G] = (uint8_t)f;
      S.alias[G] = 0;
      S.gmask[G] = (uint8_t)m;
      S.ng[f] = 1;
      G++;
      continue;
    }
    if (fnv[f]) return SPLIT_BAD;
    const uint32_t now = fnow[f], first = G;
    uint32_t w[4];
    for (uint32_t u = 0; u < 4; u++) {
      S.ug[f][u] = SPLIT_BAD;
      if (!((m >> u) & 1)) continue;
      w[u] = now - now % div_of(u + 1);
      const bool cls = per_second && u == 0;
      uint32_t g = SPLIT_BAD;
      for (uint32_t v = 0; v < u; v++) {
        if (!((m >> v) & 1) || w[v] != w[u]) continue;
        if ((per_second && v == 0) != cls) return SPLIT_BAD;
        g = S.ug[f][v];
      }
      if (g == SPLIT_BAD) {
        if (G >= SPLIT_MAXG) return SPLIT_BAD;
        g = G++;
        S.fam[g] = (uint8_t)f;
        S.alias[g] = 1;
        S.gmask[g] = 0;
      }
      S.ug[f][u] = (uint8_t)g;
      S.gmask[g] |= (uint8_t)(1u << u);
    }
    S.ng[f] = (uint8_t)(G - first);
    S.any_alias = 1;
  }
  S.G = G;
  return G;
}

__device__ inline uint32_t split_group_flags(const SplitPlan& S, uint32_t g, uint32_t fl) {
  if (!S.alias[g]) return fl;
  const uint32_t f = S.fam[g];
  uint32_t x = RUN_ALIAS | ((uint32_t)S.gmask[g] << RUN_UMASK_SHIFT);
  if (S.head[f] == g) x |= RUN_AHEAD | ((uint32_t)S.ng[f] << RUN_G_SHIFT);
  return x;
}

constexpr uint32_t SPLIT_UNROLL = 8;
#ifndef RL_SPLIT_ST
#define RL_SPLIT_ST 16
#endif
constexpr uint32_t SPLIT_ST = RL_SPLIT_ST;
#ifndef RL_SPLIT_LONG_THREADS
#define RL_SPLIT_LONG_THREADS 1024
#endif
#ifndef RL_SPLIT_LONG_ST
#define RL_SPLIT_LONG_ST 8
#endif
#ifndef RL_SPLIT_LONG_OCC
#define RL_SPLIT_LONG_OCC 4
#endif
#ifndef RL_SPLIT_LONG_BLOCKS
#define RL_SPLIT_LONG_BLOCKS 8
#endif
#ifndef RL_SPLIT_THREADS
#define RL_SPLIT_THREADS 256
#endif
constexpr uint32_t SPLIT_THREADS = RL_SPLIT_THREADS;

struct UniqList {
  uint2* list;
  uint32_t* n;
  const uint32_t* skeys;
  uint32_t* keys0;
  __device__ inline void single(uint32_t e, uint32_t p) const {
    const uint32_t k = skeys[p];
    keys0[e] = k;
    if (list) list[atomicAdd(n, 1u)] = make_uint2(e, k);
  }
};

template <uint32_t NT, uint32_t ST>
__device__ __attribute__((always_inline)) inline void split_long_body(uint32_t j, uint32_t r, uint32_t p, uint32_t L, BatchDev b,
                                                          SRec rec_s, uint32_t* svals, uint32_t* segsum,
                                                          uint32_t* __restrict__ rid, uint32_t* __restrict__ run_start,
                                                          uint32_t* __restrict__ run_end,
                                                          uint32_t* __restrict__ run_flags, uint32_t* __restrict__ defer,
                                                          unsigned long long* num_runs, unsigned long long* split,
                                                          uint32_t* __restrict__ drun, uint32_t drun_cap, uint32_t* grp,
                                                          uint32_t* rank, uint32_t* __restrict__ pos_hits,
                                                          uint32_t* __restrict__ hnew, int per_second, uint32_t rfl,
                                                          const UniqList& uq) {
  constexpr uint32_t NW = NT / 64;
  __shared__ uint32_t s_wc[NW][SPLIT_MAXG], s_wh[NW][SPLIT_MAXG], s_wp[NW][SPLIT_MAXG], s_ws[NW];
  __shared__ uint32_t s_cnt[SPLIT_MAXG], s_base[SPLIT_MAXG], s_id[SPLIT_MAXG], s_fl[SPLIT_MAXG], s_off[SPLIT_MAXG];
  __shared__ uint32_t s_lnow[SPLIT_MAXG], s_lunit[SPLIT_MAXG], s_fmask[SPLIT_MAXG], s_fnv[SPLIT_MAXG];
  __shared__ uint32_t s_bad, s_lead, s_nu, s_ul[SPLIT_ULIST];
  __shared__ SplitPlan s_plan;
  const uint32_t tid = threadIdx.x, lane = tid & 63, wv = tid >> 6;
  const uint64_t lt = lane ? (~0ull >> (64 - lane)) : 0ull;
  Rec* rec = const_cast<Rec*>(rec_s.rec);
  const uint32_t* sv = rec_s.sv;
  {
#ifdef RL_SPLIT_PROF
    uint64_t ts[8];
    ts[0] = wall_clock64();
#define SPLIT_STAMP(i) ts[i] = wall_clock64()
#else
#define SPLIT_STAMP(i)
#endif
    __syncthreads();
    if (tid == 0) {
      s_bad = 0;
      s_nu = 0;
    }
    if (tid < SPLIT_MAXG) {
      s_fmask[tid] = 0;
      s_fnv[tid] = 0;
    }
    __syncthreads();
    uint32_t NF = 0;
    if (tid == 0) {
      const Rec y = rec[sv[p]];
      pos_hits[p] = y.hits > 1 ? y.hits : 1u;
      if ((rfl & (RUN_UNITS | RUN_STEMS)) == RUN_UNITS) {
        grp[p] = rec_unit(y) << 8;
        s_lnow[0] = y.now;
        s_lunit[0] = rec_unit(y);
        s_fnv[0] = (rfl & RUN_NOWVAR) ? 1u : 0u;
        s_fmask[0] = ((rfl >> RUN_UMASK_SHIFT) & 0xFu) | (1u << (rec_unit(y) - 1));
      }
    }
    if ((rfl & (RUN_UNITS | RUN_STEMS)) == RUN_UNITS) {
      NF = 1;
    } else {
      uint32_t fm0 = 0, nv0 = 0;
      for (uint32_t k = tid + 1; k < L; k += NT) {
        const uint32_t v = grp[p + k], lo = v & 0xFFu;
        if (lo == SPLIT_POS_SKIP) {
          s_bad = 1;
        } else if (lo == 0) {
          fm0 |= 1u << (((v >> 8) & 0xFFu) - 1);
          nv0 |= (v & SPLIT_POS_NOWVAR) ? 1u : 0u;
        } else {
          const uint32_t j = atomicAdd(&s_nu, 1u);
// ... 1799 lines not shown
__global__ __launch_bounds__(EXPORT_WRITE_THREADS) void k_export_write(const TableDev t, uint64_t s0, uint64_t s1,
                                                                       const uint32_t* __restrict__ cnt,
                                                                       unsigned long long* cursor, const ExportDev o) {
  const uint64_t i = s0 + (uint64_t)blockIdx.x * EXPORT_WRITE_THREADS + threadIdx.x;
  const uint32_t lane = threadIdx.x & 63u, wave = threadIdx.x >> 6;
  const uint32_t c = i < s1 ? cnt[i - s0] : 0u, r = c & ~EXPORT_LOST;
  SlotImg im;
  uint32_t len = 0;
  if (r) {
    load_img_lo(&t.slots[i], im);
    len = im.key_len();
  }
  const unsigned long long mine = ((unsigned long long)r << 32) | ((unsigned long long)r * len);
  unsigned long long x = mine;
#pragma unroll
  for (uint32_t d = 1; d < 64; d <<= 1) {
    const unsigned long long y = __shfl_up(x, d);
    if (lane >= d) x += y;
  }
  __shared__ unsigned long long wtot[EXPORT_WRITE_THREADS / 64];
  if (lane == 63) wtot[wave] = x;
  __syncthreads();
  if (threadIdx.x == 0) {
    unsigned long long run = 0;
    for (uint32_t k = 0; k < EXPORT_WRITE_THREADS / 64; k++) {
      const unsigned long long w = wtot[k];
      wtot[k] = run;
      run += w;
    }
    const unsigned long long at0 = run ? atomicAdd(cursor, run) : 0ull;
    for (uint32_t k = 0; k < EXPORT_WRITE_THREADS / 64; k++) wtot[k] += at0;
  }
  __syncthreads();
  const unsigned long long base = wtot[wave];
  if (!r) return;
  const unsigned long long at = base + x - mine;
  uint32_t R = (uint32_t)(at >> 32), B = (uint32_t)at;
  const Slot* s = &t.slots[i];
  const uint8_t unit = (uint8_t)im.unit();
  auto put = [&](const Win& w, uint32_t j) {
    o.off[R] = B;
    o.unit[R] = unit;
    o.flags[R] = (uint8_t)((c & EXPORT_LOST) && j == 0 ? RL_REC_CHAIN_LOST : 0u);
    o.ws[R] = w.ws;
    o.count[R] = w.count;
    o.expire[R] = w.expire;
    o.lc[R] = w.lc;
    export_stem(t, s, len, o.stem + B);
    R++;
    B += len;
  };
  const bool has_cur = im.cur().ws != WS_INVALID;
  const uint32_t logged = r - (has_cur ? 1u : 0u);
  Win w{WS_INVALID, 0, 0, 0};
  bool brk;
  uint32_t j = 0;
  for (; j < logged && export_next(t, (uint32_t)i, im, j == 0, w.ws, &w, &brk); j++) put(w, j);
  if (has_cur && j == logged) put(im.cur(), j);
}

__global__ __launch_bounds__(256) void k_log_epoch(const unsigned long long* log_ctr,
                                                   unsigned long long* __restrict__ epoch) {
  if (threadIdx.x < LOG_PARTS)
    epoch[threadIdx.x] =
        __hip_atomic_load(log_ctr + (size_t)threadIdx.x * LOG_CTR_STRIDE, __ATOMIC_RELAXED, __HIP_MEMORY_SCOPE_AGENT);
}

constexpr int64_t SLOT_UNKNOWN = -9;
__device__ inline uint32_t import_append(const TableDev& t, uint32_t p, uint32_t si, uint32_t tag, uint32_t prev,
                                         uint32_t t_app, const Win& r) {
  const unsigned long long k = atomicAdd(&t.log_ctr[(size_t)p * LOG_CTR_STRIDE], 1ull);
  if (k - t.log_epoch[p] >= t.log_cap) {
    atomicAdd(t.hist_lost + 1, 1ull);
    return LOG_LOST;
  }
  const uint32_t pos = (uint32_t)k & (t.log_cap - 1u);
  uint4* e = reinterpret_cast<uint4*>(&t.log[(size_t)p * t.log_cap + pos]);
  const uint4 h = make_uint4(si, tag, prev, t_app), rv = make_uint4(r.ws, r.count, r.expire, r.lc);
#pragma unroll
  for (uint32_t s = 0; s < LOG_WRITE_STEPS; s++) log_write_step(e, s, h, rv, !RL_LOG_BUSY);
  return (p << LOG_POS_BITS) | pos;
}

__global__ __launch_bounds__(256) void k_import(const TableDev t, const BatchDev b, const ImportRec* __restrict__ rec,
                                                const uint32_t* __restrict__ gstart,
                                                const unsigned long long* __restrict__ ghash, uint32_t ng,
                                                uint32_t* err) {
  const uint32_t g = blockIdx.x * 256 + threadIdx.x;
  if (g >= ng) return;
  const uint64_t hs = ghash[g];
  const uint32_t p0 = gstart[g], p1 = gstart[g + 1];
  Rec r0{};
  r0.off = rec[p0].off;
  r0.lu = rec[p0].lu & 0xFFFFu;
  const Key key = key_of(b, r0);
  int64_t sidx[4] = {SLOT_UNKNOWN, SLOT_UNKNOWN, SLOT_UNKNOWN, SLOT_UNKNOWN};
  bool ins;
  for (uint32_t p = p0; p < p1; p++) {
    const ImportRec x = rec[p];
    const uint32_t u = (x.lu >> 16) & 0xFFu, d = div_of(u), tag = slot_tag(hs, u);
    const uint32_t part = p & (LOG_PARTS - 1u);
    bool fresh = false;
    if (sidx[u - 1] == SLOT_UNKNOWN) {
      sidx[u - 1] = find_slot(t, hs, tag, key, u, true, &ins, err);
      fresh = ins;
    }
    if (sidx[u - 1] < 0) continue;
    const uint32_t si = (uint32_t)sidx[u - 1];
    Slot* s = &t.slots[si];
    const Win cur = s->cur, nr{x.ws, x.count, x.expire, x.lc};
    uint32_t chain = s->ring;
    if (fresh && ((x.lu >> 24) & RL_REC_CHAIN_LOST)) {
      chain = LOG_LOST;
      s->ring = chain;
    }
    if (cur.ws == WS_INVALID || cur.ws == x.ws) {
      s->cur = nr;
    } else if (x.ws > cur.ws) {
      if (hist_keep(t, cur, x.ws, d)) s->ring = import_append(t, part, si, tag, chain, x.ws, cur);
      s->cur = nr;
    } else {
      s->ring = import_append(t, part, si, tag, chain, cur.ws, nr);
    }
  }
  uint32_t present = 0;
  for (uint32_t u = 1; u <= 4; u++) {
    if (sidx[u - 1] == SLOT_UNKNOWN) sidx[u - 1] = find_slot(t, hs, slot_tag(hs, u), key, u, false, &ins, err);
    if (sidx[u - 1] >= 0) present |= 1u << (u - 1);
  }
  if (__popc(present) >= 2)
    for (uint32_t u = 0; u < 4; u++)
      if ((present >> u) & 1) t.slots[sidx[u]].flags |= SLOT_EXACT;
}

__device__ inline int lookup_find(const TableDev& t, uint32_t head, uint32_t si, uint32_t tag, uint32_t cur_ws,
                                  uint32_t w, Win* out) {
  uint32_t ptr = head, tprev = cur_ws, saved = LOG_NONE, power = 1, lam = 0;
  for (uint32_t hops = 0; ptr != LOG_NONE; hops++) {
    const uint32_t pos = ptr & LOG_POS_MASK;
    if (hops == LOG_MAX_HOPS || pos >= t.log_cap || ptr == saved) return -1;
    if (++lam == power) {
      saved = ptr;
      power <<= 1;
      lam = 0;
    }
    const uint4* e = reinterpret_cast<const uint4*>(&t.log[(size_t)(ptr >> LOG_POS_BITS) * t.log_cap + pos]);
    const uint4 a = e[0], b = e[1];
    if (a.x != si || a.y != tag || a.w > tprev) return -1;
    if (b.x == w) {
      *out = Win{b.x, b.y, b.z, b.w};
      return 1;
    }
    if (a.w <= w) return 0;
    tprev = a.w;
    ptr = a.z;
  }
  return 0;
}

__device__ inline uint64_t hash_key(const HashKey& hk, const Key& key) {
  const uint32_t len = key.len;
  StemHasher hs(hk, len);
  uint64_t tail = 0;
#pragma unroll
  for (uint32_t k = 0; k < KEY_HEAD / 8; k++) {
    const uint64_t m = (uint64_t)key_dw(key, 2 * k) | ((uint64_t)key_dw(key, 2 * k + 1) << 32);
    if (8 * k + 8 <= len) hs.word(m);
    else if (8 * k < len) tail = m;
  }
  if (len > KEY_HEAD) {
    uint32_t i = KEY_HEAD;
    for (; i + 8 <= len; i += 8) hs.word((uint64_t)key.st.word(i >> 2) | ((uint64_t)key.st.word((i >> 2) + 1) << 32));
    if (i < len)
      tail = ((uint64_t)key.st.word(i >> 2) | ((uint64_t)key.st.word((i >> 2) + 1) << 32)) &
             ((1ull << ((len - i) * 8)) - 1);
  }
  return hs.finish(tail, hk.hi_bits);
}

__global__ __launch_bounds__(256) void k_lookup(const TableDev t, const BatchDev b, const Params P,
                                                const int64_t* __restrict__ time_floor, const LookupDev q) {
  const uint32_t i = blockIdx.x * 256 + threadIdx.x;
  if (i >= q.n) return;
  const uint32_t s0 = q.off[i], s1 = q.off[i + 1], u = q.unit[i], now = q.now[i];
  uint32_t status = RL_OK, found = 0, count = 0, expire = 0, lc = 0;
  if (s1 <= s0 || s1 - s0 > 65535u || s1 > b.stem_total || u < 1 || u > 4) {
    status = RL_E_INVALID;
  } else if (now > NOW_MAX || (int64_t)now < *time_floor) {
    status = RL_E_TIME;
  } else {
    Rec r0{};
    r0.off = s0;
    r0.lu = s1 - s0;
    const Key key = key_of(b, r0);
    uint64_t hs = hash_key(b.hk, key);
    if ((uint32_t)(hs >> 32) == KEY_DUP) hs = ((uint64_t)(KEY_DUP - 1u) << 32) | (uint32_t)hs;
    const uint32_t tag = slot_tag(hs, u);
    SlotImg im;
    uint64_t j = hs >> t.shift;
    bool hit = false;
    for (uint32_t p = 0; p < t.max_probe; p++, j = (j + 1) & t.mask) {
      load_img_lo(&t.slots[j], im);
      const uint32_t tg = im.tag();
      if (tg == TAG_EMPTY) break;
      if (tg == tag && im.unit() == u && img_key_equal(im, key, t.arena)) {
        hit = true;
        break;
      }
    }
    int64_t sidx[4];
    Win c[4];
    uint32_t chain[4], present;
    if (hit && !(im.flags() & SLOT_EXACT)) {
      present = 1u << (u - 1);
#pragma unroll
      for (uint32_t k = 0; k < 4; k++) {
        sidx[k] = (int64_t)j;
        c[k] = im.cur();
        chain[k] = im.ring();
      }
    } else {
      present = find_unit_slots(t, hs, key, sidx, c, chain) & 0xFu;
    }
    const uint32_t w = now - now % div_of(u);
    const bool cls = P.per_second && u == RL_UNIT_SECOND;
    bool lost = false, vf = false;
    uint32_t lcw = 0;
#pragma unroll
    for (uint32_t k = 0; k < 4; k++) {
      if (!((present >> k) & 1)) continue;
      const uint32_t d = div_of(k + 1);
      Win R = c[k];
      if (R.ws != w) {
        if (R.ws == WS_INVALID || w > R.ws || w % d) continue;
        const int f =
            chain[k] == LOG_NONE ? 0 : lookup_find(t, chain[k], (uint32_t)sidx[k], slot_tag(hs, k + 1), c[k].ws, w, &R);
        if (f <= 0) {
          if (f < 0 ? !hist_dead(now, w, d) : !hist_absent_ok(t, now, w, c[k].ws, d)) lost = true;
          continue;
        }
      }
      lcw = R.lc > lcw ? R.lc : lcw;
      if ((P.per_second && k == 0) == cls && !vf && now <= R.expire) {
        vf = true;
        count = R.count;
        expire = R.expire;
      }
    }
    if (lost) {
      status = RL_E_TIME;
      count = expire = 0;
    } else {
      found = vf ? 1u : 0u;
      lc = (P.lc_en && now < lcw) ? lcw : 0u;
    }
  }
  q.status[i] = (uint8_t)status;
  q.found[i] = (uint8_t)found;
  q.count[i] = count;
  q.expire[i] = expire;
  q.lc[i] = lc;
}

__global__ __launch_bounds__(256) void k_debug_keys(BatchDev b, uint8_t* out, uint32_t* klen) {
  const uint32_t i = blockIdx.x * 256 + threadIdx.x;
  if (i >= b.n) return;
  const uint32_t s0 = b.off[i], len = b.off[i + 1] - s0;
  uint8_t* dst = out + s0 + 24ull * i;
  for (uint32_t j = 0; j < len; j++) dst[j] = b.stem[s0 + j];
  const uint32_t now = (uint32_t)b.now[b.req[i]];
  const uint32_t d = div_of(b.unit[i]);
  uint32_t ws = now / d * d;
  uint8_t tmp[12];
  uint32_t nd = 0;
  do { tmp[nd++] = (uint8_t)('0' + ws % 10); ws /= 10; } while (ws);
  for (uint32_t j = 0; j < nd; j++) dst[len + j] = tmp[nd - 1 - j];
  klen[i] = len + nd;
}

__global__ __launch_bounds__(256) void k_debug_decide(uint32_t n, const uint32_t* before, const uint32_t* after,
                                                      const uint8_t* lc_hit, const uint32_t* hits,
                                                      const uint32_t* limit, const uint8_t* unit,
                                                      const uint8_t* flags, const int64_t* now, float ratio,
                                                      int lc_en, uint8_t* code, uint32_t* rem, uint32_t* reset,
                                                      unsigned long long* deltas, uint8_t* lc_set) {
  const uint32_t i = blockIdx.x * 256 + threadIdx.x;
  if (i >= n) return;
  const bool shadow = flags[i] & RL_FLAG_SHADOW;
  const Decision r = decide(before[i], after[i], lc_hit[i] != 0, hits[i], limit[i], ratio, shadow, lc_en != 0);
  code[i] = r.code;
  rem[i] = r.remaining;
  const uint32_t d = div_of(unit[i]);
  reset[i] = d - (uint32_t)(now[i] % d);
  unsigned long long* s = deltas + (size_t)i * RL_NUM_STATS;
  s[RL_STAT_TOTAL_HITS] = 0;
  s[RL_STAT_OVER_LIMIT] = r.d_over;
  s[RL_STAT_NEAR_LIMIT] = r.d_near;
  s[RL_STAT_OVER_LIMIT_WITH_LOCAL_CACHE] = r.d_lc;
  s[RL_STAT_WITHIN_LIMIT] = r.d_within;
  s[RL_STAT_SHADOW_MODE] = r.d_shadow;
  lc_set[i] = r.set_lc;
}

static inline uint32_t cdiv(uint64_t a, uint64_t b) { return (uint32_t)((a + b - 1) / b); }

void launch_stage_a(const BatchDev& b, const Scratch& s, int isolate, int per_second, hipStream_t st,
                    hipEvent_t* ev, uint32_t* long_hint, bool long_kernel, uint32_t* big_hint, bool big_full,
                    uint32_t* list_hint, bool list_on) {
  const uint32_t g0 = cdiv(b.n > b.n_req ? b.n : b.n_req, 256);
  if (ev) (void)hipEventRecord(ev[0], st);
  if (g0)
    k_prepare<<<g0, 256, 0, st>>>(b, s.rec, s.keys[0], s.err, s.errs, isolate, s.time_floor, s.defer_n, s.big_n,
                                  s.work_n, s.run_flags, s.runs64, s.hit_a, s.res, s.sorted_n, s.uniq_n);
  if (ev) (void)hipEventRecord(ev[1], st);
  const uint32_t ptiles = cdiv(b.n, PART_TILE);
  if (b.n)
    k_part<<<ptiles, 256, 0, st>>>(s.keys[0], b.wire ? s.hit_a : b.hits, s.tile, b.n, ptiles, s.part_info, s.err);
  if (ev) (void)hipEventRecord(ev[2], st);
  if (b.n) {
    const size_t seg_lds = (2ull * ptiles + 1) * 4;
    (list_on ? k_bucket<true> : k_bucket<false>)<<<PART_DIGITS, BkSmall::THREADS, seg_lds, st>>>(
        s.tile, s.part_info, ptiles, s.keys[1], s.vals[0], s.hits_s, s.segsum, s.rid, s.run_start, s.run_end,
        s.runs64, s.drun, s.big_meta, s.big_n, s.big_work, s.work_n, s.sorted_n, s.uniq, s.uniq_n, s.err, big_hint);
#ifndef RL_EXP_NO_BIG
    const uint32_t gi = big_full ? BIG_ITEM_BLOCKS : 1u, gb = big_full ? BIG_BLOCKS : 1u;
    k_big_count<<<gi, BkSmall::THREADS, seg_lds, st>>>(s.tile, s.part_info, ptiles,
                                                                    s.big_meta, s.big_work, s.work_n, s.big_cnt,
                                                                    s.err);
    k_big_place<<<gi, BkSmall::THREADS, seg_lds, st>>>(
        s.tile, s.part_info, ptiles, s.big_meta, s.big_work, s.work_n, s.big_cnt, s.keys[1],
        s.vals[0], s.hits_s, s.segsum, s.rid, s.run_start, s.run_end, s.drun, s.err);
    k_bucket_big<<<gb, BkBig::THREADS, seg_lds, st>>>(s.tile, s.part_info, ptiles,
                                                              s.keys[1], s.vals[0], s.hits_s, s.hit_t, s.segsum,
                                                              s.rid, s.run_start, s.run_end, s.runs64, s.drun, s.big_meta,
                                                              s.big_n, s.big_cnt, s.err);
#endif
    k_run_check<<<cdiv(b.n, RC_CHUNK), 256, 0, st>>>(b, SRec{s.rec, s.vals[0]}, s.keys[1], s.rid, s.run_start,
                                                s.run_end, s.run_flags, s.defer, s.defer_n, s.err, s.runs64, s.split,
                                                s.sorted_n, s.grp, s.hit_t, s.uniq, s.uniq_n, s.long_runs, s.keys[0],
                                                list_on ? 1 : 0, list_hint);
#ifndef RL_EXP_NO_SPLIT
    k_split<<<SPLIT_BLOCKS, SPLIT_THREADS, 0, st>>>(b, SRec{s.rec, s.vals[0]}, s.vals[0], s.segsum, s.rid, s.run_start,
                                          s.run_end, s.run_flags, s.defer, s.defer_n, s.runs64, s.split, s.drun,
                                          b.n / 2 + BIG_HEAVY * PART_DIGITS, s.grp, s.lead, s.hit_t, s.vals[1], s.err,
                                          per_second, UniqList{list_on ? s.uniq : nullptr, s.uniq_n, s.keys[1], s.keys[0]}, s.long_runs, long_hint,
                                          long_kernel ? 1 : 0);
#endif
#if RL_SPLIT_LONG_THREADS
    if (long_kernel)
      k_split_long<<<RL_SPLIT_LONG_BLOCKS, RL_SPLIT_LONG_THREADS, 0, st>>>(
          b, SRec{s.rec, s.vals[0]}, s.vals[0], s.segsum, s.rid, s.run_start, s.run_end, s.run_flags, s.defer,
          s.runs64, s.split, s.drun, b.n / 2 + BIG_HEAVY * PART_DIGITS, s.grp, s.lead, s.hit_t, s.vals[1], s.err,
          per_second, UniqList{list_on ? s.uniq : nullptr, s.uniq_n, s.keys[1], s.keys[0]}, s.long_runs);
#endif
  }
}

#ifndef RL_LATE_FAST_BLOCKS
#define RL_LATE_FAST_BLOCKS 0
#endif
constexpr uint32_t LATE_SCAN_BLOCKS = 4;
void launch_b_begin_early(const BatchDev& b, const OutDev& o, const Scratch& s, int restore, hipStream_t st,
                          const unsigned long long* log_ctr) {
  const uint32_t m = restore ? 0u : b.n_rules * RL_NUM_STATS;
  const uint32_t gb = m ? (cdiv(m, 256) < 64 ? cdiv(m, 256) : 64) : 1;
  k_b_begin<<<gb, 256, 0, st>>>(s.err, s.errb, nullptr, s.defer2_n, s.defer1_n, o.stats, m, s.fast_blk,
                                cdiv(b.n, 256 * 32), log_ctr, s.log_epoch);
}

void launch_stage_b(const BatchDev& b, const OutDev& o, const TableDev& t, const Params& P, const Scratch& s,
                    int restore, hipStream_t st, hipEvent_t* ev, const uint32_t* errb_prev, hipEvent_t table_done,
                    unsigned long long* kt_acc, bool early, uint32_t* late_hint, bool late_full, bool list_on) {
  const uint32_t m = restore ? 0u : b.n_rules * RL_NUM_STATS;
  const uint32_t gb = m ? (cdiv(m, 256) < 64 ? cdiv(m, 256) : 64) : 1;
  if (!early)
    k_b_begin<<<gb, 256, 0, st>>>(s.err, s.errb, errb_prev, s.defer2_n, s.defer1_n, o.stats, m, s.fast_blk,
                                  cdiv(b.n, 256 * 32), t.log_ctr, s.log_epoch);
  else if (!b.n)
    k_b_begin<<<1, 256, 0, st>>>(s.errb, s.errb, errb_prev, s.defer2_n, s.defer1_n, o.stats, 0, s.fast_blk, 0,
                                 nullptr, nullptr);
  if (b.n) {
    const uint32_t g = cdiv(b.n, 256);
    const size_t lds = (!restore && b.n_rules <= LDS_RULES) ? (size_t)b.n_rules * RL_NUM_STATS * 8 : 0;
    const SRec rs{s.rec, s.vals[0]};
    if (ev) (void)hipEventRecord(ev[3], st);
    const uint32_t g_runs = cdiv(b.n / 2 + BIG_HEAVY * PART_DIGITS, 256);
    k_table<<<g_runs + g, 256, lds, st>>>(g_runs, b, t, P, rs, s.keys[1], s.vals[0], s.res, s.run_start, s.run_end,
                                         s.run_flags, s.run_state, s.run_alias, s.rid, s.run_f, s.runs64, s.drun,
                                         s.defer2, s.defer2_n,
                                         s.keys[0], s.defer1, s.defer1_n, o.stats, s.stripes, s.errb, s.errs, restore,
                                         s.fast_blk, s.uniq, list_on ? s.uniq_n : nullptr, kt_acc ? s.kt_blk : nullptr,
                                         early ? errb_prev : nullptr);
    if (ev) (void)hipEventRecord(ev[4], st);
    if (!restore && P.lc_en)
      k_fast_over<<<g, 256, 0, st>>>(s.sorted_n, rs, s.segsum, s.rid, s.run_flags, s.run_state, s.run_f, s.errb);
#ifndef RL_EXP_NO_LATE
    const uint32_t gl = restore ? 0u : !late_full ? LATE_SCAN_BLOCKS
                                     : (RL_LATE_FAST_BLOCKS && g > RL_LATE_FAST_BLOCKS ? RL_LATE_FAST_BLOCKS : g);
    k_late<<<RUNS_GENERAL_LATE_BLOCKS + gl, 256, lds, st>>>(
        b, t, P, rs, s.keys[1], s.vals[0], s.res, s.run_start, s.run_end, s.defer, s.defer_n, s.defer2, s.defer2_n,
        s.grp, s.lead, s.gmask,
        s.keys[0], s.defer1, s.defer1_n, s.segsum, s.rid, s.run_flags, s.run_state, s.run_alias, s.run_f, o.stats,
        s.stripes, s.errb,
        s.errs, restore, s.fast_blk, s.sorted_n, late_hint, late_full ? 0 : 1);
#endif
    if (table_done) (void)hipEventRecord(table_done, st);
    if (!restore) {
      const uint32_t nf = b.n_rules <= LDS_RULES ? b.n_rules : 0u;
      const uint32_t gf = cdiv(nf * RL_NUM_STATS > b.n ? nf * RL_NUM_STATS : b.n, 256);
      k_finish<<<gf, 256, 0, st>>>(s.res, b.n, o, s.stripes, nf, s.errb, P.lc_en ? s.counters + 5 : nullptr,
                                   kt_acc ? s.kt_blk : nullptr, g_runs + g, kt_acc, b.own);
    }
  } else {
    if (ev) {
      (void)hipEventRecord(ev[3], st);
      (void)hipEventRecord(ev[4], st);
    }
    if (table_done) (void)hipEventRecord(table_done, st);
  }
  if (ev) (void)hipEventRecord(ev[5], st);
}


void launch_sweep(const TableDev& t, uint64_t nslots, uint32_t now, unsigned long long* evicted, hipStream_t st) {
  k_sweep<<<2048, 256, 0, st>>>(t, nslots, now, evicted);
}

void launch_arena_compact(Slot* slots, uint64_t nslots, const uint8_t* from, uint8_t* to, unsigned long long* used16,
                          hipStream_t st) {
  k_arena_compact<<<2048, 256, 0, st>>>(slots, nslots, from, to, used16);
}

void launch_reclaim(const TableDev& t, const HashKey& hk, uint64_t nslots, uint32_t* need, unsigned long long* ctr,
                    hipStream_t st) {
  k_reclaim_mark<<<2048, 256, 0, st>>>(t, hk, nslots, need, ctr);
  k_reclaim_free<<<2048, 256, 0, st>>>(t.slots, nslots, need, ctr, ctr + 1);
}

void launch_lc_count(const TableDev& t, uint64_t nslots, uint32_t now, unsigned long long* out, hipStream_t st) {
  k_lc_count<<<2048, 256, 0, st>>>(t, nslots, now, out);
}

void launch_table_info(const Slot* slots, uint64_t nslots, unsigned long long* out, hipStream_t st) {
  k_table_info<<<2048, 256, 0, st>>>(slots, nslots, out);
}

void launch_resize_place(const TableDev& t, const HashKey& hk, uint64_t nslots, Slot* to, uint64_t to_nslots,
                         uint32_t* map, unsigned long long* ctr, hipStream_t st) {
  const uint32_t probe = (uint32_t)(to_nslots < (1u << 16) ? to_nslots : (1u << 16));
  k_resize_place<<<(uint32_t)((nslots + 255) / 256 < 2048 ? (nslots + 255) / 256 : 2048), 256, 0, st>>>(
      t, hk, nslots, to, to_nslots - 1, 64u - (uint32_t)__builtin_ctzll(to_nslots), probe, map, ctr);
}

void launch_resize_relink(const TableDev& t, uint64_t nslots, const uint32_t* map, unsigned long long* ctr,
                          hipStream_t st) {
  k_resize_relink<<<(uint32_t)((nslots + 255) / 256 < 2048 ? (nslots + 255) / 256 : 2048), 256, 0, st>>>(t, nslots, map,
                                                                                                        ctr);
}

void launch_export_count(const TableDev& t, uint64_t s0, uint64_t s1, uint32_t* cnt, unsigned long long* tot,
                         hipStream_t st) {
  if (s1 > s0)
    k_export_count<<<(uint32_t)((s1 - s0 + 255) / 256 < 2048 ? (s1 - s0 + 255) / 256 : 2048), 256, 0, st>>>(t, s0, s1, cnt,
                                                                                                          tot);
}

void launch_export_write(const TableDev& t, uint64_t s0, uint64_t s1, const uint32_t* cnt, unsigned long long* cursor,
                         const ExportDev& o, hipStream_t st) {
  if (s1 > s0)
    k_export_write<<<(uint32_t)((s1 - s0 + EXPORT_WRITE_THREADS - 1) / EXPORT_WRITE_THREADS), EXPORT_WRITE_THREADS, 0,
                     st>>>(t, s0, s1, cnt, cursor, o);
}

void launch_import(const TableDev& t, const HashKey& hk, const uint8_t* stem, uint32_t stem_total, const ImportRec* rec,
                   const uint32_t* gstart, const unsigned long long* ghash, uint32_t ng, unsigned long long* epoch,
                   uint32_t* err, hipStream_t st) {
  if (!ng) return;
  k_log_epoch<<<1, 256, 0, st>>>(t.log_ctr, epoch);
  TableDev tv = t;
  tv.log_epoch = epoch;
  BatchDev b{};
  b.hk = hk;
  b.stem = stem;
  b.stem_cap = b.stem_total = stem_total;
  k_import<<<cdiv(ng, 256), 256, 0, st>>>(tv, b, rec, gstart, ghash, ng, err);
}

void launch_lookup(const TableDev& t, const HashKey& hk, const Params& P, const int64_t* time_floor,
                   const uint8_t* stem, uint32_t stem_total, const LookupDev& q, hipStream_t st) {
  if (!q.n) return;
  BatchDev b{};
  b.hk = hk;
  b.stem = stem;
  b.stem_cap = b.stem_total = stem_total;
  k_lookup<<<cdiv(q.n, 256), 256, 0, st>>>(t, b, P, time_floor, q);
}

bool log_tear_hook() { return RL_LOG_TEAR != 0; }

void launch_debug_keys(const BatchDev& b, uint8_t* out, uint32_t* klen, hipStream_t st) {
  if (b.n) k_debug_keys<<<cdiv(b.n, 256), 256, 0, st>>>(b, out, klen);
}

void launch_debug_decide(uint32_t n, const uint32_t* before, const uint32_t* after, const uint8_t* lc_hit,
                         const uint32_t* hits, const uint32_t* limit, const uint8_t* unit, const uint8_t* flags,
                         const int64_t* now, float ratio, int lc_en, uint8_t* code, uint32_t* rem, uint32_t* reset,
                         unsigned long long* deltas, uint8_t* lc_set, hipStream_t st) {
  if (n)
    k_debug_decide<<<cdiv(n, 256), 256, 0, st>>>(n, before, after, lc_hit, hits, limit, unit, flags, now, ratio,
                                                 lc_en, code, rem, reset, deltas, lc_set);
}

}
```

Baseline: 6.232 billion.

## Pack partition tile records into 8 bytes and widen k_part to 8 waves

```diff
diff --git a/ratelimit_amd/build.py b/ratelimit_amd/build.py
--- a/ratelimit_amd/build.py
+++ b/ratelimit_amd/build.py
@@ -11,7 +11,7 @@
            "rl_comm.hip",
            "rl_api.hip",
            "rl_pack.cpp"]
-HEADERS = ["rl_device.h", "rl_kernels.h", "rl_slot_img.h", "rl_hot_select.h", "rl_match.h", "rl_wire_parse.h", "rl_resp_emit.h", "rl_engine.h",
+HEADERS = ["rl_device.h", "rl_kernels.h", "rl_tile.h", "rl_slot_img.h", "rl_hot_select.h", "rl_match.h", "rl_wire_parse.h", "rl_resp_emit.h", "rl_engine.h",
            "rl_comm.h", "rl_transport.h",
            os.path.join("..", "..", "include", "ratelimit_hip.h")]
 HIPCC = os.environ.get("HIPCC", "/opt/rocm/bin/hipcc")
diff --git a/ratelimit_amd/csrc/rl_engine.hip b/ratelimit_amd/csrc/rl_engine.hip
--- a/ratelimit_amd/csrc/rl_engine.hip
+++ b/ratelimit_amd/csrc/rl_engine.hip
@@ -287,6 +287,7 @@
 }
 
 bool alloc_buffer(Scratch& s, uint32_t n) {
+  static_assert(sizeof(*s.tile) == 8, "Scratch::tile: one 8-byte record per descriptor");
   const size_t items = (size_t)n / (64 * 4 * 8) + 1 + PART_DIGITS;
   bool ok = dalloc(&s.big_meta, PART_DIGITS) == hipSuccess && dalloc(&s.big_n, 1) == hipSuccess &&
             dalloc(&s.big_work, items) == hipSuccess && dalloc(&s.work_n, 1) == hipSuccess &&
diff --git a/ratelimit_amd/csrc/rl_kernels.h b/ratelimit_amd/csrc/rl_kernels.h
--- a/ratelimit_amd/csrc/rl_kernels.h
+++ b/ratelimit_amd/csrc/rl_kernels.h
@@ -5,6 +5,7 @@
 
 #include "rl_device.h"
 #include "rl_hot_select.h"
+#include "rl_tile.h"
 
 namespace rl {
 
@@ -12,6 +13,9 @@
 #define RL_PART_ITEMS 16
 #endif
 constexpr uint32_t PART_ITEMS = RL_PART_ITEMS, PART_TILE = 256 * PART_ITEMS;
+constexpr uint32_t PART_WAVES = 8, PART_THREADS = 64 * PART_WAVES;
+constexpr uint32_t PART_WITEMS = PART_TILE / PART_THREADS;
+static_assert(PART_TILE % PART_THREADS == 0, "k_part: whole items per lane");
 constexpr uint32_t PART_BITS = 10, PART_DIGITS = 1u << PART_BITS;
 #ifndef RL_BIG_BLOCKS
 #define RL_BIG_BLOCKS 64
@@ -25,6 +29,8 @@
   uint32_t heavy[BIG_HEAVY];
 };
 constexpr uint32_t MAX_PART_TILES = 2048 * 16 / PART_ITEMS;
+static_assert((uint64_t)MAX_PART_TILES * PART_TILE <= (1ull << TILE_IDX_BITS),
+              "a tile record's index bits hold every descriptor index of the largest batch");
 constexpr uint32_t LONG_RUN = 32;
 constexpr uint32_t RUN_SLOW = 1, RUN_FAST = 2, RUN_MULTI = 4;
 constexpr uint32_t RUN_NOWVAR = 8;
@@ -185,7 +191,7 @@
   unsigned long long* stripes;
   uint32_t* hits_s;
   uint32_t* hit_a;
-  uint4* tile;
+  TileRec* tile;
   uint32_t* hit_t;
   uint32_t* segsum;
   uint32_t* rid;
diff --git a/ratelimit_amd/csrc/rl_kernels.hip b/ratelimit_amd/csrc/rl_kernels.hip
--- a/ratelimit_amd/csrc/rl_kernels.hip
+++ b/ratelimit_amd/csrc/rl_kernels.hip
@@ -1308,11 +1308,22 @@
 
 #ifdef RL_BK_PROF
 __device__ unsigned long long g_bk_prof[PART_DIGITS * 16];
+__device__ unsigned long long g_part_prof[MAX_PART_TILES * 8];
 __device__ uint32_t g_bk_peel[PART_DIGITS * 16];
-#define BK_STAMP(d, k) \
-  if (threadIdx.x == 0) g_bk_prof[(d) * 16 + (k)] = wall_clock64()
+#define PROF_WAIT() asm volatile("s_waitcnt vmcnt(0) lgkmcnt(0)" ::: "memory")
+#define BK_STAMP(d, k)                                        \
+  do {                                                        \
+    PROF_WAIT();                                              \
+    if (threadIdx.x == 0) g_bk_prof[(d) * 16 + (k)] = wall_clock64(); \
+  } while (0)
+#define PART_STAMP(t, k)                                      \
+  do {                                                        \
+    PROF_WAIT();                                              \
+    if (threadIdx.x == 0) g_part_prof[(t) * 8 + (k)] = wall_clock64(); \
+  } while (0)
 #else
 #define BK_STAMP(d, k)
+#define PART_STAMP(t, k)
 #endif
 
 template <uint32_t IT, uint32_t BITS>
@@ -1344,7 +1355,8 @@
   for (uint32_t i = 0; i < IT; i++) pos[i] = __shfl(pos[i] & 0xFFFFu, leader[i]) + (pos[i] >> 16);
 }
 
-__device__ inline uint32_t scan256(uint32_t v, uint32_t* wsum4, uint32_t* total) {
+template <uint32_t W>
+__device__ inline uint32_t scan_waves(uint32_t v, uint32_t* wsum, uint32_t* total) {
   const uint32_t lane = threadIdx.x & 63, wave = threadIdx.x >> 6;
   uint32_t inc = v;
 #pragma unroll
@@ -1352,45 +1364,60 @@
     const uint32_t y = __shfl_up(inc, off, 64);
     if (lane >= off) inc += y;
   }
-  if (wave < 4 && lane == 63) wsum4[wave] = inc;
+  if (wave < W && lane == 63) wsum[wave] = inc;
   __syncthreads();
-  uint32_t pre = 0;
-#pragma unroll
-  for (uint32_t w = 0; w < 4; w++) pre += w < wave ? wsum4[w] : 0u;
-  if (total) *total = wsum4[0] + wsum4[1] + wsum4[2] + wsum4[3];
+  uint32_t pre = 0, all = 0;
+#pragma unroll
+  for (uint32_t w = 0; w < W; w++) {
+    pre += w < wave ? wsum[w] : 0u;
+    all += wsum[w];
+  }
+  if (total) *total = all;
   __syncthreads();
   return pre + inc - v;
 }
-
-__global__ __launch_bounds__(256) void k_part(const uint32_t* __restrict__ kin, const uint32_t* __restrict__ hin,
-                                              uint4* __restrict__ out, uint32_t n, uint32_t ntiles,
-                                              uint32_t* __restrict__ info, const uint32_t* err) {
-  constexpr uint32_t DPT = PART_DIGITS / 256;
-  __shared__ uint32_t wcnt[4][PART_DIGITS];
-  __shared__ uint32_t wsum[4];
-  __shared__ uint32_t sk[PART_TILE], sv[PART_TILE], sh[PART_TILE];
+__device__ inline uint32_t scan256(uint32_t v, uint32_t* wsum4, uint32_t* total) {
+  return scan_waves<4>(v, wsum4, total);
+}
+
+constexpr uint32_t PART_LDS_WORDS =
+    PART_WAVES * PART_DIGITS > 2 * PART_TILE ? PART_WAVES * PART_DIGITS : 2 * PART_TILE;
+static_assert(PART_DIGITS % PART_THREADS == 0, "k_part: whole digits per thread");
+static_assert(PART_TILE < (1u << 16), "part_info packs a tile offset and a count into 16 bits each");
+
+__global__ __launch_bounds__(PART_THREADS) void k_part(const uint32_t* __restrict__ kin,
+                                                       const uint32_t* __restrict__ hin, TileRec* __restrict__ out,
+                                                       uint32_t n, uint32_t ntiles, uint32_t* __restrict__ info,
+                                                       const uint32_t* err) {
+  constexpr uint32_t DPT = PART_DIGITS / PART_THREADS;
+  __shared__ uint32_t lds[PART_LDS_WORDS];
+  __shared__ uint32_t wsum[PART_WAVES];
+  uint32_t(*wcnt)[PART_DIGITS] = reinterpret_cast<uint32_t(*)[PART_DIGITS]>(lds);
+  uint32_t *sk = lds, *sp = lds + PART_TILE;
   if (*err) return;
   const uint32_t tid = threadIdx.x, lane = tid & 63, wave = tid >> 6, tile = blockIdx.x;
-  for (uint32_t j = tid; j < 4 * PART_DIGITS; j += 256) (&wcnt[0][0])[j] = 0;
+  PART_STAMP(tile, 0);
+  for (uint32_t j = tid; j < PART_WAVES * PART_DIGITS; j += PART_THREADS) lds[j] = 0;
   __syncthreads();
-  const uint32_t wbase = tile * PART_TILE + wave * 64 * PART_ITEMS;
-  uint32_t kk[PART_ITEMS], vv[PART_ITEMS], hh[PART_ITEMS], pos[PART_ITEMS];
-#pragma unroll
-  for (uint32_t i = 0; i < PART_ITEMS; i++) {
+  const uint32_t wbase = tile * PART_TILE + wave * 64 * PART_WITEMS;
+  uint32_t kk[PART_WITEMS], pv[PART_WITEMS], pos[PART_WITEMS];
+#pragma unroll
+  for (uint32_t i = 0; i < PART_WITEMS; i++) {
     const uint32_t j = min(wbase + i * 64 + lane, n - 1);
     kk[i] = kin[j];
-    vv[i] = j;
-    hh[i] = hin[j];
-  }
-  wave_multisplit<PART_ITEMS, PART_BITS>(kk, wbase, n, 32 - PART_BITS, wcnt[wave], pos);
+    pv[i] = tile_pack(0u, j, hin[j]).iv;
+  }
+  PART_STAMP(tile, 1);
+  wave_multisplit<PART_WITEMS, PART_BITS>(kk, wbase, n, 32 - PART_BITS, wcnt[wave], pos);
   __syncthreads();
+  PART_STAMP(tile, 2);
   uint32_t c[DPT], tsum = 0;
 #pragma unroll
   for (uint32_t j = 0; j < DPT; j++) {
     const uint32_t d = tid * DPT + j;
     uint32_t acc = 0;
 #pragma unroll
-    for (uint32_t w = 0; w < 4; w++) {
+    for (uint32_t w = 0; w < PART_WAVES; w++) {
       const uint32_t t = wcnt[w][d];
       wcnt[w][d] = acc;
       acc += t;
@@ -1398,34 +1425,37 @@
     c[j] = acc;
     tsum += acc;
   }
-  uint32_t excl = scan256(tsum, wsum, nullptr);
+  uint32_t excl = scan_waves<PART_WAVES>(tsum, wsum, nullptr);
 #pragma unroll
   for (uint32_t j = 0; j < DPT; j++) {
     const uint32_t d = tid * DPT + j;
     info[(size_t)d * ntiles + tile] = (excl << 16) | c[j];
 #pragma unroll
-    for (uint32_t w = 0; w < 4; w++) wcnt[w][d] += excl;
+    for (uint32_t w = 0; w < PART_WAVES; w++) wcnt[w][d] += excl;
     excl += c[j];
   }
   __syncthreads();
 #pragma unroll
-  for (uint32_t i = 0; i < PART_ITEMS; i++) {
+  for (uint32_t i = 0; i < PART_WITEMS; i++) pos[i] += wcnt[wave][kk[i] >> (32 - PART_BITS)];
+  __syncthreads();
+  PART_STAMP(tile, 3);
+#pragma unroll
+  for (uint32_t i = 0; i < PART_WITEMS; i++) {
     if (wbase + i * 64 + lane < n) {
-      const uint32_t d = kk[i] >> (32 - PART_BITS);
-      const uint32_t q = wcnt[wave][d] + pos[i];
-      sk[q] = kk[i];
-      sv[q] = vv[i];
-      sh[q] = hh[i];
+      sk[pos[i]] = kk[i];
+      sp[pos[i]] = pv[i];
     }
   }
   __syncthreads();
+  PART_STAMP(tile, 4);
   const uint32_t cnt = min(PART_TILE, n - tile * PART_TILE);
-  uint4* o = out + (size_t)tile * PART_TILE;
-#pragma unroll
-  for (uint32_t i = 0; i < PART_ITEMS; i++) {
-    const uint32_t q = i * 256 + tid;
-    if (q < cnt) o[q] = make_uint4(sk[q], sv[q], sh[q], 0u);
-  }
+  TileRec* o = out + (size_t)tile * PART_TILE;
+#pragma unroll
+  for (uint32_t i = 0; i < PART_WITEMS; i++) {
+    const uint32_t q = i * PART_THREADS + tid;
+    if (q < cnt) o[q] = TileRec{sk[q], sp[q]};
+  }
+  PART_STAMP(tile, 5);
 }
 
 template <typename B>
@@ -1475,6 +1505,17 @@
   for (uint32_t i = 0; i < IT; i++) j[i] = src[lo[i]] + p[i];
 }
 
+template <uint32_t IT>
+__device__ inline void tile_gather(const TileRec* __restrict__ pt, const uint32_t* __restrict__ hin,
+                                   const uint32_t (&jj)[IT], uint32_t (&kk)[IT], uint32_t (&vv)[IT],
+                                   uint32_t (&hh)[IT]) {
+  TileRec e[IT];
+#pragma unroll
+  for (uint32_t i = 0; i < IT; i++) e[i] = pt[jj[i]];
+#pragma unroll
+  for (uint32_t i = 0; i < IT; i++) tile_unpack(e[i], hin, kk[i], vv[i], hh[i]);
+}
+
 template <typename B>
 __device__ inline uint32_t block_sum(BucketLds<B>& L, uint32_t v) {
   const uint32_t lane = threadIdx.x & 63, wave = threadIdx.x >> 6;
@@ -1736,7 +1777,7 @@
 
 constexpr uint32_t BK_SAMPLES_PER_LANE = 4;
 template <typename B>
-__device__ inline void sample_heavy(BucketLds<B>& L, uint32_t S, uint32_t ntiles, const uint4* __restrict__ pt) {
+__device__ inline void sample_heavy(BucketLds<B>& L, uint32_t S, uint32_t ntiles, const TileRec* __restrict__ pt) {
   constexpr uint32_t R = BK_SAMPLES_PER_LANE, NS = 64 * R;
   const uint32_t lane = threadIdx.x & 63;
   if ((threadIdx.x >> 6) == 0) {
@@ -1747,7 +1788,7 @@
     bucket_src(ntiles, p, j);
 #pragma unroll
     for (uint32_t i = 0; i < R; i++) {
-      ks[i] = pt[j[i]].x;
+      ks[i] = pt[j[i]].key;
       cnt[i] = 0;
       first[i] = true;
     }
@@ -1783,22 +1824,23 @@
   __syncthreads();
 }
 
+constexpr uint32_t BK_GRID = 512;
+static_assert(BK_GRID < PART_DIGITS, "k_bucket<LIST, true> walks several buckets");
 #ifndef RL_BK_EARLY
 #define RL_BK_EARLY 1
 #endif
 template <bool LIST>
-__global__ __launch_bounds__(BkSmall::THREADS, 4) void k_bucket(
-    const uint4* __restrict__ pt,
+__device__ __attribute__((always_inline)) inline void bucket_one(
+    BucketLds<BkSmall>& L, const uint32_t d,
+    const TileRec* __restrict__ pt, const uint32_t* __restrict__ hin,
     const uint32_t* __restrict__ info, uint32_t ntiles, uint32_t* __restrict__ sk, uint32_t* __restrict__ sv,
     uint32_t* __restrict__ sh, uint32_t* __restrict__ segsum, uint32_t* __restrict__ rid,
     uint32_t* __restrict__ run_start, uint32_t* __restrict__ run_end, unsigned long long* num_runs,
     uint32_t* __restrict__ drun, BigMeta* __restrict__ meta, uint32_t* big_n, uint32_t* __restrict__ work,
-    uint32_t* work_n, uint32_t* sorted_n, uint2* __restrict__ uniq, uint32_t* uniq_n, const uint32_t* err,
+    uint32_t* work_n, uint32_t* sorted_n, uint2* __restrict__ uniq, uint32_t* uniq_n,
     uint32_t* big_hint) {
   using B = BkSmall;
-  __shared__ BucketLds<B> L;
-  if (*err) return;
-  const uint32_t tid = threadIdx.x, lane = tid & 63, wave = tid >> 6, d = blockIdx.x;
+  const uint32_t tid = threadIdx.x, lane = tid & 63, wave = tid >> 6;
   BK_STAMP(d, 0);
   bucket_setup(L, info, ntiles, d);
   const uint32_t S = L.S;
@@ -1836,13 +1878,7 @@
 #pragma unroll
   for (uint32_t i = 0; i < B::ITEMS; i++) pp[i] = min(strip0 + i * 64 + lane, S - 1);
   bucket_src(ntiles, pp, jj);
-#pragma unroll
-  for (uint32_t i = 0; i < B::ITEMS; i++) {
-    const uint4 e = pt[jj[i]];
-    kk[i] = e.x;
-    vv[i] = e.y;
-    hh[i] = e.z;
-  }
+  tile_gather(pt, hin, jj, kk, vv, hh);
   BK_STAMP(d, 2);
   uint32_t* ht = L.v;
   uint8_t* df = reinterpret_cast<uint8_t*>(&L.wcnt[0][0]);
@@ -1878,6 +1914,7 @@
     }
   }
   __syncthreads();
+  BK_STAMP(d, 6);
   const uint64_t lt = (1ull << lane) - 1;
   uint32_t cidx[B::ITEMS], sidx[LIST ? B::ITEMS : 1], wc = 0, ws = 0, wr = 0, dmask = 0, smask = 0;
 #pragma unroll
@@ -1935,6 +1972,7 @@
     for (uint32_t i = 0; i < B::ITEMS; i++)
       if ((smask >> i) & 1u) uniq[ub + sidx[i]] = make_uint2(vv[i], kk[i]);
   }
+  BK_STAMP(d, 8);
   if (!M) return;
   if (M <= 64) {
     if (wave == 0) {
@@ -1985,9 +2023,32 @@
   BK_STAMP(d, 5);
 }
 
+template <bool LIST, bool WALK>
+__global__ __launch_bounds__(BkSmall::THREADS, 4) void k_bucket(
+    const TileRec* __restrict__ pt, const uint32_t* __restrict__ hin,
+    const uint32_t* __restrict__ info, uint32_t ntiles, uint32_t* __restrict__ sk, uint32_t* __restrict__ sv,
+    uint32_t* __restrict__ sh, uint32_t* __restrict__ segsum, uint32_t* __restrict__ rid,
+    uint32_t* __restrict__ run_start, uint32_t* __restrict__ run_end, unsigned long long* num_runs,
+    uint32_t* __restrict__ drun, BigMeta* __restrict__ meta, uint32_t* big_n, uint32_t* __restrict__ work,
+    uint32_t* work_n, uint32_t* sorted_n, uint2* __restrict__ uniq, uint32_t* uniq_n, const uint32_t* err,
+    uint32_t* big_hint) {
+  __shared__ BucketLds<BkSmall> L;
+  if (*err) return;
+  if constexpr (WALK) {
+    for (uint32_t d = blockIdx.x; d < PART_DIGITS; d += gridDim.x) {
+      bucket_one<LIST>(L, d, pt, hin, info, ntiles, sk, sv, sh, segsum, rid, run_start, run_end, num_runs, drun, meta,
+                       big_n, work, work_n, sorted_n, uniq, uniq_n, big_hint);
+      __syncthreads();
+    }
+  } else {
+    bucket_one<LIST>(L, blockIdx.x, pt, hin, info, ntiles, sk, sv, sh, segsum, rid, run_start, run_end, num_runs, drun,
+                     meta, big_n, work, work_n, sorted_n, uniq, uniq_n, big_hint);
+  }
+}
+
 template <typename B>
 __device__ inline bool bucket_peel(BucketLds<B>& L, uint32_t d, uint32_t S, uint32_t base, uint32_t ntiles,
-                                   const uint4* __restrict__ pt,
+                                   const TileRec* __restrict__ pt, const uint32_t* __restrict__ hin,
                                    uint32_t* __restrict__ sk,
                                    uint32_t* __restrict__ sv, uint32_t* __restrict__ sh) {
   constexpr uint32_t IT = B::ITEMS;
@@ -1996,7 +2057,7 @@
   if (wave == 0) {
     uint32_t p[1] = {(uint32_t)(((uint64_t)(2 * lane + 1) * S) >> 7)}, j[1];
     bucket_src(ntiles, p, j);
-    const uint32_t ks = pt[j[0]].x;
+    const uint32_t ks = pt[j[0]].key;
     uint32_t cnt = 0;
     bool first = true;
     for (uint32_t q = 0; q < 64; q++) {
@@ -2030,13 +2091,7 @@
 #pragma unroll
     for (uint32_t i = 0; i < IT; i++) pp[i] = min(strip0 + i * 64 + lane, S - 1);
     bucket_src(ntiles, pp, jj);
-#pragma unroll
-    for (uint32_t i = 0; i < IT; i++) {
-      const uint4 e = pt[jj[i]];
-      kk[i] = e.x;
-      vv[i] = e.y;
-      hh[i] = e.z;
-    }
+    tile_gather(pt, hin, jj, kk, vv, hh);
     uint32_t wl = 0, lr[IT];
     uint32_t wc[BK_HEAVY];
 #pragma unroll
@@ -2141,13 +2196,7 @@
 #pragma unroll
     for (uint32_t i = 0; i < IT; i++) pp[i] = min(s0 + i * 64 + lane, S - 1);
     bucket_src(ntiles, pp, jj);
-#pragma unroll
-    for (uint32_t i = 0; i < IT; i++) {
-      const uint4 e = pt[jj[i]];
-      kk[i] = e.x;
-      vv[i] = e.y;
-      hh[i] = e.z;
-    }
+    tile_gather(pt, hin, jj, kk, vv, hh);
     uint32_t hr[IT], wc[BK_HEAVY];
 #pragma unroll
     for (uint32_t c = 0; c < BK_HEAVY; c++) wc[c] = 0;
@@ -2199,7 +2248,7 @@
 
 template <typename B>
 __device__ inline void bucket_lsd(BucketLds<B>& L, uint32_t S, uint32_t base, uint32_t ntiles,
-                                  const uint4* __restrict__ pt,
+                                  const TileRec* __restrict__ pt, const uint32_t* __restrict__ hin,
                                   uint32_t* __restrict__ sk,
                                   uint32_t* __restrict__ sv, uint32_t* __restrict__ sh, uint32_t* __restrict__ ht,
                                   uint32_t* __restrict__ segsum, uint32_t* __restrict__ rid) {
@@ -2214,7 +2263,7 @@
     for (uint32_t i = 0; i < IT; i++) pp[i] = min(c0 + i * B::THREADS + tid, S - 1);
     bucket_src(ntiles, pp, jj);
 #pragma unroll
-    for (uint32_t i = 0; i < IT; i++) kk[i] = pt[jj[i]].x;
+    for (uint32_t i = 0; i < IT; i++) kk[i] = pt[jj[i]].key;
 #pragma unroll
     for (uint32_t i = 0; i < IT; i++) {
       if (c0 + i * B::THREADS + tid < S) {
@@ -2250,13 +2299,7 @@
         for (uint32_t i = 0; i < IT; i++) jj[i] = pp[i];
       }
       if (pass == 0) {
-#pragma unroll
-        for (uint32_t i = 0; i < IT; i++) {
-          const uint4 e = pt[jj[i]];
-          kk[i] = e.x;
-          vv[i] = e.y;
-          hh[i] = e.z;
-        }
+        tile_gather(pt, hin, jj, kk, vv, hh);
       } else {
 #pragma unroll
         for (uint32_t i = 0; i < IT; i++) {
@@ -2314,22 +2357,17 @@
   return x;
 }
 
-__device__ inline void big_chunk_load(const BigMeta& M, uint32_t j, uint32_t ntiles, const uint4* __restrict__ pt,
-                                      uint32_t (&kk)[BkSmall::ITEMS], uint32_t (&vv)[BkSmall::ITEMS],
-                                      uint32_t (&hh)[BkSmall::ITEMS], uint32_t (&cls)[BkSmall::ITEMS], bool values) {
+__device__ inline void big_chunk_load(const BigMeta& M, uint32_t j, uint32_t ntiles, const TileRec* __restrict__ pt,
+                                      const uint32_t* __restrict__ hin, uint32_t (&kk)[BkSmall::ITEMS],
+                                      uint32_t (&vv)[BkSmall::ITEMS], uint32_t (&hh)[BkSmall::ITEMS],
+                                      uint32_t (&cls)[BkSmall::ITEMS]) {
   using B = BkSmall;
   const uint32_t lane = threadIdx.x & 63, s0 = j * BIG_CHUNK + (threadIdx.x >> 6) * B::STRIP;
   uint32_t pp[B::ITEMS], jj[B::ITEMS];
 #pragma unroll
   for (uint32_t i = 0; i < B::ITEMS; i++) pp[i] = min(s0 + i * 64 + lane, M.S - 1);
   bucket_src(ntiles, pp, jj);
-#pragma unroll
-  for (uint32_t i = 0; i < B::ITEMS; i++) {
-    const uint4 e = pt[jj[i]];
-    kk[i] = e.x;
-    hh[i] = e.z;
-    vv[i] = values ? e.y : 0u;
-  }
+  tile_gather(pt, hin, jj, kk, vv, hh);
 #pragma unroll
   for (uint32_t i = 0; i < B::ITEMS; i++) {
     cls[i] = s0 + i * 64 + lane < M.S ? M.r : 0xFFu;
@@ -2339,7 +2377,8 @@
   }
 }
 
-__global__ __launch_bounds__(BkSmall::THREADS) void k_big_count(const uint4* __restrict__ pt,
+__global__ __launch_bounds__(BkSmall::THREADS) void k_big_count(const TileRec* __restrict__ pt,
+                                                                const uint32_t* __restrict__ hin,
                                                                 const uint32_t* __restrict__ info, uint32_t ntiles,
                                                                 const BigMeta* __restrict__ meta,
                                                                 const uint32_t* __restrict__ work,
@@ -2354,7 +2393,7 @@
     const BigMeta M = meta[w >> 16];
     bucket_setup(L, info, ntiles, M.d);
     uint32_t kk[B::ITEMS], vv[B::ITEMS], hh[B::ITEMS], cls[B::ITEMS];
-    big_chunk_load(M, w & 0xFFFFu, ntiles, pt, kk, vv, hh, cls, false);
+    big_chunk_load(M, w & 0xFFFFu, ntiles, pt, hin, kk, vv, hh, cls);
     uint32_t nl = 0, nc[BK_HEAVY], hs[BK_HEAVY];
 #pragma unroll
     for (uint32_t c = 0; c < BK_HEAVY; c++) nc[c] = hs[c] = 0;
@@ -2394,7 +2433,7 @@
 }
 
 __global__ __launch_bounds__(BkSmall::THREADS) void k_big_place(
-    const uint4* __restrict__ pt,
+    const TileRec* __restrict__ pt, const uint32_t* __restrict__ hin,
     const uint32_t* __restrict__ info, uint32_t ntiles, const BigMeta* __restrict__ meta,
     const uint32_t* __restrict__ work, const uint32_t* work_n, const uint32_t* __restrict__ cnt,
     uint32_t* __restrict__ sk, uint32_t* __restrict__ sv, uint32_t* __restrict__ sh, uint32_t* __restrict__ segsum,
@@ -2440,7 +2479,7 @@
       drun[M.db_heavy + tid] = M.rb_heavy + tid;
     }
     uint32_t kk[B::ITEMS], vv[B::ITEMS], hh[B::ITEMS], cls[B::ITEMS];
-    big_chunk_load(M, j, ntiles, pt, kk, vv, hh, cls, true);
+    big_chunk_load(M, j, ntiles, pt, hin, kk, vv, hh, cls);
     uint32_t rk[B::ITEMS], hp[B::ITEMS], wl = 0, wc[BK_HEAVY], wh[BK_HEAVY];
 #pragma unroll
     for (uint32_t c = 0; c < BK_HEAVY; c++) wc[c] = wh[c] = 0;
@@ -2517,7 +2556,7 @@
 }
 
 __global__ __launch_bounds__(BkBig::THREADS) void k_bucket_big(
-    const uint4* __restrict__ pt,
+    const TileRec* __restrict__ pt, const uint32_t* __restrict__ hin,
     const uint32_t* __restrict__ info, uint32_t ntiles, uint32_t* __restrict__ sk, uint32_t* __restrict__ sv,
     uint32_t* __restrict__ sh, uint32_t* __restrict__ ht, uint32_t* __restrict__ segsum, uint32_t* __restrict__ rid,
     uint32_t* __restrict__ run_start, uint32_t* __restrict__ run_end, unsigned long long* num_runs,
@@ -2564,8 +2603,8 @@
       if (tid < M.r) run_start[M.rb_heavy + tid] = run_end[M.rb_heavy + tid] = 0;
       bucket_setup(L, info, ntiles, d);
       BK_STAMP(d, 1);
-      if (!bucket_peel(L, d, S, base, ntiles, pt, sk, sv, sh))
-        bucket_lsd(L, S, base, ntiles, pt, sk, sv, sh, ht, segsum, rid);
+      if (!bucket_peel(L, d, S, base, ntiles, pt, hin, sk, sv, sh))
+        bucket_lsd(L, S, base, ntiles, pt, hin, sk, sv, sh, ht, segsum, rid);
       bucket_segment<B, false>(L, d, S, base, sk, sh, segsum, rid, run_start, run_end, num_runs, drun);
     }
     BK_STAMP(d, 7);
@@ -4971,6 +5010,14 @@
   lc_set[i] = r.set_lc;
 }
 
+#ifdef RL_BK_PROF
+extern "C" __attribute__((visibility("default"))) int rl_debug_stage_a_prof(unsigned long long* bk,
+                                                                            unsigned long long* part) {
+  if (hipDeviceSynchronize() != hipSuccess) return 1;
+  if (hipMemcpyFromSymbol(bk, HIP_SYMBOL(g_bk_prof), sizeof(g_bk_prof)) != hipSuccess) return 1;
+  return hipMemcpyFromSymbol(part, HIP_SYMBOL(g_part_prof), sizeof(g_part_prof)) != hipSuccess;
+}
+#endif
 static inline uint32_t cdiv(uint64_t a, uint64_t b) { return (uint32_t)((a + b - 1) / b); }
 
 void launch_stage_a(const BatchDev& b, const Scratch& s, int isolate, int per_second, hipStream_t st,
@@ -4983,23 +5030,25 @@
                                   s.work_n, s.run_flags, s.runs64, s.hit_a, s.res, s.sorted_n, s.uniq_n);
   if (ev) (void)hipEventRecord(ev[1], st);
   const uint32_t ptiles = cdiv(b.n, PART_TILE);
+  const uint32_t* hin = b.wire ? s.hit_a : b.hits;
   if (b.n)
-    k_part<<<ptiles, 256, 0, st>>>(s.keys[0], b.wire ? s.hit_a : b.hits, s.tile, b.n, ptiles, s.part_info, s.err);
+    k_part<<<ptiles, PART_THREADS, 0, st>>>(s.keys[0], hin, s.tile, b.n, ptiles, s.part_info, s.err);
   if (ev) (void)hipEventRecord(ev[2], st);
   if (b.n) {
     const size_t seg_lds = (2ull * ptiles + 1) * 4;
-    (list_on ? k_bucket<true> : k_bucket<false>)<<<PART_DIGITS, BkSmall::THREADS, seg_lds, st>>>(
-        s.tile, s.part_info, ptiles, s.keys[1], s.vals[0], s.hits_s, s.segsum, s.rid, s.run_start, s.run_end,
+    (list_on ? k_bucket<true, false> : k_bucket<false, true>)
+        <<<list_on ? PART_DIGITS : BK_GRID, BkSmall::THREADS, seg_lds, st>>>(
+        s.tile, hin, s.part_info, ptiles, s.keys[1], s.vals[0], s.hits_s, s.segsum, s.rid, s.run_start, s.run_end,
         s.runs64, s.drun, s.big_meta, s.big_n, s.big_work, s.work_n, s.sorted_n, s.uniq, s.uniq_n, s.err, big_hint);
 #ifndef RL_EXP_NO_BIG
     const uint32_t gi = big_full ? BIG_ITEM_BLOCKS : 1u, gb = big_full ? BIG_BLOCKS : 1u;
-    k_big_count<<<gi, BkSmall::THREADS, seg_lds, st>>>(s.tile, s.part_info, ptiles,
+    k_big_count<<<gi, BkSmall::THREADS, seg_lds, st>>>(s.tile, hin, s.part_info, ptiles,
                                                                     s.big_meta, s.big_work, s.work_n, s.big_cnt,
                                                                     s.err);
     k_big_place<<<gi, BkSmall::THREADS, seg_lds, st>>>(
-        s.tile, s.part_info, ptiles, s.big_meta, s.big_work, s.work_n, s.big_cnt, s.keys[1],
+        s.tile, hin, s.part_info, ptiles, s.big_meta, s.big_work, s.work_n, s.big_cnt, s.keys[1],
         s.vals[0], s.hits_s, s.segsum, s.rid, s.run_start, s.run_end, s.drun, s.err);
-    k_bucket_big<<<gb, BkBig::THREADS, seg_lds, st>>>(s.tile, s.part_info, ptiles,
+    k_bucket_big<<<gb, BkBig::THREADS, seg_lds, st>>>(s.tile, hin, s.part_info, ptiles,
                                                               s.keys[1], s.vals[0], s.hits_s, s.hit_t, s.segsum,
                                                               s.rid, s.run_start, s.run_end, s.runs64, s.drun, s.big_meta,
                                                               s.big_n, s.big_cnt, s.err);
diff --git a/ratelimit_amd/csrc/rl_tile.h b/ratelimit_amd/csrc/rl_tile.h
--- /dev/null
+++ b/ratelimit_amd/csrc/rl_tile.h
@@ -0,0 +1,39 @@
+#pragma once
+
+#include <stdint.h>
+
+#if defined(__HIPCC__)
+#define RL_TILE_HD __host__ __device__
+#else
+#define RL_TILE_HD
+#endif
+
+namespace rl {
+
+constexpr uint32_t TILE_IDX_BITS = 23;
+constexpr uint32_t TILE_IDX_MASK = (1u << TILE_IDX_BITS) - 1u;
+constexpr uint32_t TILE_HITS_ESC = (1u << (32 - TILE_IDX_BITS)) - 1u;
+
+struct __attribute__((aligned(8))) TileRec {
+  uint32_t key;
+  uint32_t iv;
+};
+static_assert(sizeof(TileRec) == 8, "one dwordx2 per record");
+
+RL_TILE_HD inline TileRec tile_pack(uint32_t key, uint32_t index, uint32_t hits) {
+  const uint32_t h9 = hits < TILE_HITS_ESC ? hits : TILE_HITS_ESC;
+  return TileRec{key, (index & TILE_IDX_MASK) | (h9 << TILE_IDX_BITS)};
+}
+RL_TILE_HD inline uint32_t tile_index(uint32_t iv) { return iv & TILE_IDX_MASK; }
+RL_TILE_HD inline bool tile_escaped(uint32_t iv) { return (iv >> TILE_IDX_BITS) == TILE_HITS_ESC; }
+RL_TILE_HD inline uint32_t tile_hits(uint32_t iv, const uint32_t* hits) {
+  return tile_escaped(iv) ? hits[iv & TILE_IDX_MASK] : iv >> TILE_IDX_BITS;
+}
+RL_TILE_HD inline void tile_unpack(const TileRec& e, const uint32_t* hits, uint32_t& key, uint32_t& index,
+                                   uint32_t& h) {
+  key = e.key;
+  index = tile_index(e.iv);
+  h = tile_hits(e.iv, hits);
+}
+
+}
```

Result: faster. 6.396 billion (median of 6 runs) (+2.6%).
